# sfu-rsl/FastTrack

Hardware: AMD Instinct MI355X
Metric: frames/sec extract+match (higher is better)
Workload: dtype u8

## Files before the change

### fasttrack_amd/_capi.py

```python
from __future__ import annotations

import ctypes as C
import os
import re

import numpy as np

_PKG = os.path.dirname(os.path.abspath(__file__))
LIB_PATH = os.environ.get("FT_LIB") or os.path.join(_PKG, "libfasttrack_amd.so")
HEADER_PATH = os.path.join(os.path.dirname(_PKG), "include", "fasttrack_amd.h")

FT_OK, FT_ERR_INVALID, FT_ERR_NO_DEVICE, FT_ERR_HIP, FT_ERR_CAPACITY, FT_ERR_EMPTY = 0, -1, -2, -3, -4, -5

KP_DTYPE = np.dtype([("x", "<f4"), ("y", "<f4"), ("size", "<f4"), ("angle", "<f4"), ("response", "<f4"),
                     ("octave", "<i4"), ("class_id", "<i4")])
assert KP_DTYPE.itemsize == 28


class FastTrackError(RuntimeError):
    def __init__(self, status: int, message: str):
        super().__init__(f"fasttrack_amd status {status}: {message}")
        self.status = status


# ... 75 lines not shown
    _fields_ = [("M", C.c_int), ("skip", C.c_void_p), ("world_pos", C.c_void_p), ("normal", C.c_void_p),
                ("max_distance", C.c_void_p), ("min_distance", C.c_void_p), ("descriptors", C.c_void_p),
                ("observations", C.c_void_p)]


class FrustumResult(C.Structure):
    _fields_ = [(k, C.c_void_p) for k in ("in_view", "in_view_r", "level", "level_r", "view_cos", "view_cos_r",
                                          "proj_x", "proj_y", "proj_xr", "proj_yr", "depth", "depth_r")]


def declared_symbols() -> list[str]:
    text = open(HEADER_PATH).read()
    return sorted(set(re.findall(r"FT_API[^;(]*?\b(ft_[a-z0-9_]+)\s*\(", text)))


_lib = None


def _hip_runtime_mapped() -> bool:
    try:
        with open("/proc/self/maps") as f:
            mapped = {ln.split()[-1] for ln in f if "libamdhip64" in ln}
    except OSError:
        return False
    ours = {os.path.realpath(os.path.join(os.environ.get("ROCM_PATH", "/opt/rocm"), "lib", n))
            for n in ("libamdhip64.so", "libamdhip64.so.7")}
    return any(os.path.realpath(m) in ours for m in mapped)


def lib() -> C.CDLL:
    global _lib
    if _lib is not None:
        return _lib
    if not os.path.exists(LIB_PATH):
        raise ImportError(
            f"{LIB_PATH} is missing: build it with `python -c 'import __graft_entry__ as g; g.build()'` "
            f"(or `make -C fasttrack_amd/csrc`).  fasttrack_amd has no CPU fallback.")
    if "GPU_MAX_HW_QUEUES" not in os.environ:
        if _hip_runtime_mapped():
            import warnings
            warnings.warn("fasttrack_amd: a HIP runtime was loaded before the library and GPU_MAX_HW_QUEUES is unset - contexts "
                          "will use private streams (about 10 % below the lane table on wide batches); export "
                          "GPU_MAX_HW_QUEUES=10 before the first HIP call of the process", RuntimeWarning, stacklevel=2)
        else:
            os.environ["GPU_MAX_HW_QUEUES"] = "10"
    mode = os.RTLD_LOCAL | os.RTLD_NOW | getattr(os, "RTLD_DEEPBIND", 0)
    L = C.CDLL(LIB_PATH, mode=mode)
    vp, i, f = C.c_void_p, C.c_int, C.c_float
    ip = C.POINTER(C.c_int)
    L.ft_version.restype = C.c_char_p
    L.ft_last_error.restype = C.c_char_p
    L.ft_device_count.restype = i
    L.ft_device_pci_bus_id.argtypes = [i, C.c_char_p, i]
    L.ft_context_create.argtypes = [i, i, C.POINTER(vp)]
    L.ft_context_destroy.argtypes = [vp]
    L.ft_context_synchronize.argtypes = [vp]
    L.ft_context_device_name.argtypes = [vp, C.c_char_p, i]
    L.ft_context_host_threads.argtypes = [vp]
    L.ft_context_hw_queues.argtypes = [vp]
    L.ft_context_set_lane_map.argtypes = [vp, vp, i]
    L.ft_context_set_option.argtypes = [vp, C.c_char_p, i]
    L.ft_context_get_option.argtypes = [vp, C.c_char_p, ip]
    L.ft_option_describe.argtypes = [i, C.POINTER(C.c_char_p), C.POINTER(C.c_char_p), ip, C.POINTER(C.c_char_p)]
    L.ft_option_range.argtypes = [C.c_char_p, ip, ip]
    L.ft_context_save_stats.argtypes = [vp, C.c_char_p]
    L.ft_context_set_kernel_timing.argtypes = [vp, i]
    L.ft_context_get_stat.argtypes = [vp, C.c_char_p, C.POINTER(C.c_double), C.POINTER(C.c_long)]
    L.ft_context_reset_stats.argtypes = [vp]
    L.ft_device_malloc.argtypes = [vp, C.c_size_t, C.POINTER(vp)]
    L.ft_device_free.argtypes = [vp, vp]
    L.ft_host_malloc.argtypes = [vp, C.c_size_t, C.POINTER(vp)]
    L.ft_host_free.argtypes = [vp, vp]
    L.ft_memcpy_h2d.argtypes = [vp, vp, vp, C.c_size_t]
    L.ft_memcpy_d2h.argtypes = [vp, vp, vp, C.c_size_t]
    L.ft_extractor_create.argtypes = [vp, i, f, i, i, i, i, i, i, C.POINTER(vp)]
    L.ft_extractor_destroy.argtypes = [vp]
    L.ft_extractor_levels.argtypes = [vp]
    L.ft_extractor_max_batch.argtypes = [vp]
    L.ft_extractor_max_keypoints.argtypes = [vp]
    L.ft_extractor_scale_factors.argtypes = [vp, vp, vp, vp, vp]
    L.ft_extractor_features_per_level.argtypes = [vp, vp]
    L.ft_extractor_level_size.argtypes = [vp, i, ip, ip]
    L.ft_extract.argtypes = [vp, vp, i, i, i, i, i, vp, vp, i, ip, ip]
    L.ft_extract_batch.argtypes = [vp, vp, i, i, i, i, i, i, i, vp, vp, i, vp, vp]
    L.ft_extractor_download_level.argtypes = [vp, i, i, vp, i]
    L.ft_extractor_device_level.argtypes = [vp, i, i, C.POINTER(vp), ip]
    L.ft_extractor_download_candidates.argtypes = [vp, i, i, vp, i, ip]
    L.ft_extractor_octree_on_device.argtypes = [vp, i, vp, i, i, vp, i, ip, ip]
    L.ft_stereo_match.argtypes = [vp, vp, i, vp, i, vp, i, vp, vp, f, f, i, vp, vp, vp, ip]
    L.ft_stereo_frontend_create.argtypes = [vp, i, f, i, i, i, i, i, i, f, f, C.POINTER(vp)]
    L.ft_stereo_frontend_destroy.argtypes = [vp]
    L.ft_stereo_frontend_left.argtypes = [vp]
    L.ft_stereo_frontend_left.restype = vp
    L.ft_stereo_frontend_right.argtypes = [vp]
    L.ft_stereo_frontend_right.restype = vp
    L.ft_stereo_frontend_process.argtypes = [vp, vp, vp, i, i, i, i, i, vp, vp, vp, vp, vp, vp, i, vp, vp, vp]
    L.ft_stereo_frontend_submit.argtypes = [vp, vp, vp, i, i, i, i, i, vp, vp, vp, vp, vp, vp, i, vp, vp, vp]
    L.ft_stereo_frontend_wait.argtypes = [vp]
    L.ft_fisheye_match.argtypes = [vp, vp, i, vp, i, vp, vp, vp]
    L.ft_search_local_points.argtypes = [vp, C.POINTER(FrameView), C.POINTER(LocalPoints), f, f, vp, ip] + [vp] * 10
    L.ft_search_last_frame.argtypes = [vp, C.POINTER(FrameView), C.POINTER(LastPoints), vp, f, i, i, i, vp, ip] + [vp] * 4
    L.ft_features_in_area.argtypes = [vp, C.POINTER(FrameView), i, vp, vp, vp, vp, vp, vp, vp, i, vp]
    L.ft_fisheye_stereo.argtypes = [vp, C.POINTER(FisheyeRig), vp, vp, i, vp, vp, i, vp, i, vp, vp, vp, ip]
    L.ft_is_in_frustum.argtypes = [vp, C.POINTER(FrameView), C.POINTER(FramePose), C.POINTER(MapPoints), f, f,
                                   C.POINTER(FrustumResult), ip]
    L.ft_tracked_frame_create.argtypes = [vp, i, i, C.POINTER(vp)]
    L.ft_tracked_frame_destroy.argtypes = [vp]
    L.ft_tracked_frame_upload.argtypes = [vp, C.POINTER(FrameView)]
    L.ft_tracked_frame_bind_stereo.argtypes = [vp, vp, i, C.POINTER(FrameView)]
    L.ft_tracked_frame_search_last_frame.argtypes = [vp, C.POINTER(LastPoints), vp, f, i, i, i, vp, ip]
    L.ft_tracked_frame_search_last_frame_se3.argtypes = [vp, C.POINTER(LastPoints), C.POINTER(SE3), C.POINTER(SE3), f, i, i, i, vp, ip]
    L.ft_search_last_frame_se3.argtypes = [vp, C.POINTER(FrameView), C.POINTER(LastPoints), C.POINTER(SE3), C.POINTER(SE3), f, i, i,
                                           i, vp, ip] + [vp] * 4
    L.ft_tracked_frame_track_local_map.argtypes = [vp, C.POINTER(FramePose), C.POINTER(MapPoints), f, f, f, f, i, f,
                                                   C.POINTER(FrustumResult), ip, vp, ip]
    L.ft_tracked_frame_holder_obs.argtypes = [vp, vp]
    L.ft_search_for_initialization.argtypes = [vp, C.POINTER(FrameView), C.POINTER(FrameView), vp, i, f, i, vp, ip, vp]
    L.ft_tracked_frame_search_for_initialization.argtypes = [vp, vp, vp, i, f, i, vp, ip]
    L.ft_search_keyframe_projection.argtypes = [vp, C.POINTER(FrameView), C.POINTER(KeyFramePoints), C.POINTER(SE3), f, f, i, i, vp, ip, vp, vp]
    L.ft_tracked_frame_search_keyframe_projection.argtypes = [vp, C.POINTER(KeyFramePoints), C.POINTER(SE3), f, f, i, i, vp, ip]
    L.ft_tracked_batch_create.argtypes = [vp, i, i, i, C.POINTER(vp)]
    L.ft_tracked_batch_destroy.argtypes = [vp]
    L.ft_tracked_batch_upload.argtypes = [vp, i, C.POINTER(FrameView)]
    L.ft_tracked_batch_search_last_frame.argtypes = [vp, i, C.POINTER(LastPoints), vp, f, vp, vp, i, C.POINTER(vp), vp]
    L.ft_tracked_batch_search_last_frame_se3.argtypes = [vp, i, C.POINTER(LastPoints), C.POINTER(SE3), C.POINTER(SE3), f, vp, vp, i,
                                                         C.POINTER(vp), vp]
    L.ft_tracked_batch_track_local_map.argtypes = [vp, i, C.POINTER(FramePose), C.POINTER(MapPoints), f, f, f, f, i, f,
                                                   C.POINTER(FrustumResult), vp, C.POINTER(vp), vp]
    L.ft_tracked_batch_submit_search_last_frame.argtypes = L.ft_tracked_batch_search_last_frame.argtypes
    L.ft_tracked_batch_submit_search_last_frame_se3.argtypes = L.ft_tracked_batch_search_last_frame_se3.argtypes
    L.ft_tracked_batch_submit_track_local_map.argtypes = L.ft_tracked_batch_track_local_map.argtypes
    L.ft_tracked_batch_wait.argtypes = [vp]
    L.ft_tracked_batch_holder_obs.argtypes = [vp, i, vp]
    L.ft_tracked_batch_bind_fisheye.argtypes = [vp, vp, vp, i, i, i, i, i, i, C.POINTER(FrameView), C.POINTER(FisheyeRig), vp, C.POINTER(vp),
                                                C.POINTER(vp), C.POINTER(vp), C.POINTER(vp), vp]
    L.ft_tracked_batch_bind_fisheye_slots.argtypes = [vp, vp, vp, i, i, i, i, i, i, i, C.POINTER(FrameView), C.POINTER(FisheyeRig), vp,
                                                      C.POINTER(vp), C.POINTER(vp), C.POINTER(vp), C.POINTER(vp), vp]
    L.ft_descriptor_distance.argtypes = [vp, vp, vp, i, vp]
    L.ft_stereo_frontend_device_descriptors.argtypes = [vp, i, i, C.POINTER(vp), ip]
    L.ft_vocabulary_create.argtypes = [vp, i, i, i, i, i, vp, vp, vp, vp, C.POINTER(vp)]
    L.ft_vocabulary_load_text.argtypes = [vp, C.c_char_p, C.POINTER(vp)]
    L.ft_vocabulary_destroy.argtypes = [vp]
    L.ft_vocabulary_info.argtypes = [vp, ip, ip, ip, ip]
    L.ft_bow_transform.argtypes = [vp, vp, i, i, i, vp, vp, vp, vp, vp, i, ip, vp, vp, vp, i, ip]
    L.ft_search_by_bow.argtypes = [vp, C.POINTER(BowSide), vp, C.POINTER(BowSide), i, f, i, vp, ip]
    L.ft_search_for_triangulation.argtypes = [vp, C.POINTER(TriangKeyFrame), i, C.POINTER(TriangKeyFrame), C.POINTER(TriangPair), i, i, i, vp, vp, vp]
    L.ft_fuse_search.argtypes = [vp, C.POINTER(FusePoints), i, C.POINTER(FuseTarget), vp, vp, vp, vp]
    L.ft_search_keyframe_sim3.argtypes = [vp, C.POINTER(FrameView), i, C.POINTER(Sim3Job)]
    L.ft_selftest_libm.argtypes = [vp, i, C.c_uint32, C.c_uint32, C.c_uint32, C.POINTER(C.c_ulonglong),
                                   C.POINTER(C.c_ulonglong), C.POINTER(C.c_uint32)]
    L.ft_octree_distribute.argtypes = [vp, i, i, i, i, i, i, vp, i, ip]
    L.ft_level_geometry.argtypes = [i, i, i, f, i, vp, vp, vp, vp, vp, vp, vp]
    L.ft_pyramid_band_plan.argtypes = [i, i, f, i, i, vp, vp]
    _lib = L
    return L


def check(status: int) -> None:
    if status != FT_OK:
        raise FastTrackError(status, lib().ft_last_error().decode(errors="replace"))


def ptr(a):
    return None if a is None else a.ctypes.data_as(C.c_void_p)
```

### fasttrack_amd/csrc/extractor.cpp

```cpp
#include <algorithm>
#include <map>
#include <memory>
#include <cmath>
#include <cstdio>
#include <cstdlib>
#include <cstring>

#include "ft_host.h"

namespace {

inline int cvRoundF(float v) { return (int)lrintf(v); }
inline short satShort(int v) { return (short)(v < -32768 ? -32768 : (v > 32767 ? 32767 : v)); }

void buildTaps(int ssize, int dsize, bool clampIndex, FtTap *out) {
    const double inv_scale = (double)dsize / ssize;
    const double scale = 1. / inv_scale;
    for (int d = 0; d < dsize; d++) {
        float f = (float)((d + 0.5) * scale - 0.5);
        int s = (int)std::floor(f);
        f -= s;
        if (clampIndex) {
            if (s < 0) { f = 0; s = 0; }
            if (s >= ssize - 1) { f = 0; s = ssize - 1; }
// ... 162 lines not shown
int ft_pipeline_depth(const ft_tuning &t, int batch, bool deviceOctree) {
    const int envDepth = t.pipeline_depth > 0 ? std::min(FT_PIPE_MAX, t.pipeline_depth) : 0;
    if (envDepth) return std::max(1, std::min(envDepth, batch));
    if (deviceOctree) return batch >= 256 ? 2 : 1;
    return std::max(1, std::min(FT_PIPE_MAX, batch / 16));
}

int ft_extract_foreign_wait(ft_extractor *ex) {
    if (!ex->foreignReader) return FT_OK;
    hipEvent_t ev = ex->foreignReader;
    ex->foreignReader = nullptr;
    FT_HIP(hipStreamWaitEvent(ex->stream, ev, 0));
    return FT_OK;
}

int ft_extract_prepare(ft_extractor *ex, const uint8_t *const *images, int batch, int on_device, int width,
                       int height, int stride) {
    FT_REQUIRE(ex && images, "extract: null handle or image list");
    FT_REQUIRE(batch >= 1 && batch <= ex->maxBatch, "extract: batch outside [1, max_batch]");
    FT_REQUIRE(width == ex->width && height == ex->height, "extract: image size differs from the extractor's");
    FT_REQUIRE(stride >= width, "extract: stride smaller than width");
    int rc = ft_set_device(ex->ctx);
    if (rc != FT_OK) return rc;
    const FtGeom &g = ex->geom;
    const bool uploadKernel = ex->tune.upload_kernel != 0;
    if (!on_device && ex->stageHost && uploadKernel) {
        for (int b = 0; b < batch; b++) {
            if (!images[b]) {
                ft_set_error("extract: empty image");
                return FT_ERR_EMPTY;
            }
            ex->h_l0[b] = ex->d_pyr + (size_t)b * g.pyrPerSlot + g.lv[0].off;
        }
        ft_extract_restage(ex, images, batch, width, height, stride);
        ex->l0Aligned = true;
        ex->l0pitch = g.lv[0].pitch;
        ex->lastBatch = batch;
        return ft_launch_upload(ex->stream, batch, ex->h_srcTab, width, height, ex->d_pyr + g.lv[0].off, g.lv[0].pitch,
                                g.pyrPerSlot, ex->d_l0);
    }
    hipStream_t us = ex->stream;
    if (!on_device && !ex->stageHost) {
        rc = ft_context_upload_stream(ex->ctx, &us);
        if (rc != FT_OK) return rc;
    }
    bool oneCopy = false;
    if (!on_device && !ex->stageHost && batch >= 4 && stride == width && g.lv[0].pitch == width) {
        oneCopy = images[0] != nullptr;
        const ptrdiff_t delta = oneCopy && images[1] ? images[1] - images[0] : 0;
        if (delta < (ptrdiff_t)width * height) oneCopy = false;
        for (int b = 1; b < batch && oneCopy; b++)
            if (!images[b] || images[b] - images[b - 1] != delta) oneCopy = false;
        if (oneCopy && ex->ctx->maxPitch > 0 && (size_t)delta > ex->ctx->maxPitch) oneCopy = false;
        if (oneCopy) {
            const hipError_t ce = hipMemcpy2DAsync(ex->d_pyr + g.lv[0].off, g.pyrPerSlot, images[0], (size_t)delta, (size_t)width * height,
                                                   batch, hipMemcpyHostToDevice, us);
            if (ce != hipSuccess) {
                (void)hipGetLastError();
                oneCopy = false;
            }
        }
    }
    for (int b = 0; b < batch; b++) {
        if (!images[b]) {
            ft_set_error("extract: empty image");
            return FT_ERR_EMPTY;
        }
        uint8_t *slot0 = ex->d_pyr + (size_t)b * g.pyrPerSlot + g.lv[0].off;
        if (oneCopy) {
            ex->h_l0[b] = slot0;
        } else if (on_device) {
            ex->h_l0[b] = images[b];
        } else if (ex->stageHost) {
            ex->h_l0[b] = slot0;
            uint8_t *stg = ex->h_stage + (size_t)b * width * height;
            for (int y = 0; y < height; y++) memcpy(stg + (size_t)y * width, images[b] + (size_t)y * stride, width);
            FT_HIP(hipMemcpy2DAsync(slot0, g.lv[0].pitch, stg, width, width, height, hipMemcpyHostToDevice, ex->stream));
        } else {
            ex->h_l0[b] = slot0;
            FT_HIP(hipMemcpy2DAsync(slot0, g.lv[0].pitch, images[b], stride, width, height, hipMemcpyHostToDevice, us));
        }
    }
    if (us != ex->stream) {
        FT_HIP(hipEventRecord(ex->evUp, us));
        FT_HIP(hipStreamWaitEvent(ex->stream, ex->evUp, 0));
    }
    ex->l0Aligned = !on_device || ft_frames_aligned(images, batch, stride);
    ex->l0pitch = on_device ? stride : g.lv[0].pitch;
    ex->lastBatch = batch;
    FT_HIP(hipMemcpyAsync((void *)ex->d_l0, (const void *)ex->h_l0, sizeof(uint8_t *) * batch, hipMemcpyHostToDevice,
                          ex->stream));
    return FT_OK;
}

int ft_extract_ensure_stage(ft_extractor *ex) {
    if (!ex->h_srcTab) FT_CHECK(ex->own.pinAlloc(&ex->h_srcTab, 16));
    if (!ex->h_stage) FT_CHECK(ex->own.pinAlloc(&ex->h_stage, (size_t)std::min(ex->maxBatch, 16) * ex->width * ex->height));
    return FT_OK;
}
bool ft_frames_aligned(const uint8_t *const *images, int batch, int stride) {
    bool aligned = (stride & 3) == 0;
    for (int b = 0; b < batch; b++)
        if ((uintptr_t)images[b] & 3) aligned = false;
    return aligned;
}
void ft_extract_rebind(ft_extractor *ex, const uint8_t *const *images, int batch, int on_device, int width, int height, int stride) {
    if (on_device)
        for (int b = 0; b < batch; b++) ex->h_l0[b] = images[b];
    else
        ft_extract_restage(ex, images, batch, width, height, stride);
    ex->lastBatch = batch;
}
bool ft_graph_capture(hipStream_t st, hipGraphExec_t *exec, const std::function<int()> &enqueue) {
    if (*exec) hipGraphExecDestroy(*exec);
    *exec = nullptr;
    hipGraph_t graph = nullptr;
    int rc = FT_OK;
    hipError_t ce = hipStreamBeginCapture(st, hipStreamCaptureModeThreadLocal);
    if (ce == hipSuccess) {
        rc = enqueue();
        ce = hipStreamEndCapture(st, &graph);
        if (rc == FT_OK && ce == hipSuccess && graph) ce = hipGraphInstantiate(exec, graph, nullptr, nullptr, 0);
        if (graph) hipGraphDestroy(graph);
    }
    if (rc == FT_OK && ce == hipSuccess && *exec) return true;
    (void)hipGetLastError();
    *exec = nullptr;
    return false;
}
void ft_extract_restage(ft_extractor *ex, const uint8_t *const *images, int batch, int width, int height, int stride) {
    const bool uploadKernel = ex->tune.upload_kernel != 0;
    for (int b = 0; b < batch; b++) {
        if (uploadKernel && ft_is_pinned_host_range(images[b], (size_t)(height - 1) * stride + width)) {
            ex->h_srcTab[b].ptr = images[b];
            ex->h_srcTab[b].stride = stride;
            continue;
        }
        uint8_t *stg = ex->h_stage + (size_t)b * width * height;
        for (int y = 0; y < height; y++) memcpy(stg + (size_t)y * width, images[b] + (size_t)y * stride, width);
        ex->h_srcTab[b].ptr = stg;
        ex->h_srcTab[b].stride = width;
    }
}

int ft_extract_ensure_host_cand(ft_extractor *ex) {
    if (ex->h_cand) return FT_OK;
    FT_CHECK(ex->own.pinAlloc(&ex->h_cand, (size_t)ex->maxBatch * ex->geom.candPerSlot, hipHostMallocMapped | hipHostMallocCoherent));
    void *dp = nullptr;
    FT_HIP(hipHostGetDevicePointer(&dp, ex->h_cand, 0));
    ex->d_cand = (uint32_t *)dp;
    return FT_OK;
}

int ft_extract_launch_a(ft_extractor *ex, int b0, int nb, hipEvent_t done) {
    const FtGeom &g = ex->geom;
    if (!ex->deviceOctree) {
        const int rce = ft_extract_ensure_host_cand(ex);
        if (rce != FT_OK) return rce;
    }
    const bool tm = ex->ctx->kernelTiming;
    const int al = ex->l0Aligned ? 1 : 0;
    const uint8_t *const *l0 = ex->d_l0 + b0;
    uint8_t *pyr = ex->d_pyr + (size_t)b0 * g.pyrPerSlot;
    int *cellCount = ex->d_cellCount + (size_t)b0 * g.totalCells;
    uint32_t *stage = ex->d_stage + (size_t)b0 * g.stagePerSlot;
    hipStreamCaptureStatus cap = hipStreamCaptureStatusNone;
    FT_HIP(hipStreamIsCapturing(ex->stream, &cap));
    ex->evt.begin(tm, "kernel.pyr_down(all levels)", ex->stream);
    int rc = ft_launch_pyramid(ex->stream, g, nb, l0, ex->l0pitch, pyr, ex->d_taps, al, ex->tune.pyr_rows,
                               cap == hipStreamCaptureStatusNone ? &ex->pyrBands : nullptr);
    ex->evt.end(tm, ex->stream);
    if (rc != FT_OK) return rc;
    ex->evt.begin(tm, "kernel.fast_cells", ex->stream);
    rc = ft_launch_fast_cells(ex->stream, g, nb, l0, ex->l0pitch, pyr, ex->iniTh, ex->minTh, al, cellCount, stage,
                              ex->deviceOctree ? 0 : 1, ex->d_cellTab);
    ex->evt.end(tm, ex->stream);
    if (rc != FT_OK) return rc;
    ex->evt.begin(tm, "kernel.compact", ex->stream);
    uint32_t *candDst = ex->deviceOctree ? ex->d_candDev : ex->d_cand;
    int *cntDst = ex->deviceOctree ? ex->d_candCountDev : ex->d_candCount;
    rc = ft_launch_compact(ex->stream, g, nb, cellCount, stage, candDst + (size_t)b0 * g.candPerSlot,
                           cntDst + (size_t)b0 * g.nlevels);
    ex->evt.end(tm, ex->stream);
    if (rc != FT_OK) return rc;
    if (done) FT_HIP(hipEventRecord(done, ex->stream));
    return FT_OK;
}

int ft_extract_launch_octree(ft_extractor *ex, int sub, int b0, int nb, hipEvent_t done) {
    const FtGeom &g = ex->geom;
    hipStream_t so = ex->streamO[sub % FT_OCT_STREAMS];
    FT_HIP(hipEventRecord(ex->evO[sub], ex->stream));
    FT_HIP(hipStreamWaitEvent(so, ex->evO[sub], 0));
    FtOctArgs a = ex->octLayout;
    a.cand = ex->d_candDev + (size_t)b0 * g.candPerSlot;
    a.candCount = ex->d_candCountDev + (size_t)b0 * g.nlevels;
    a.sel = ex->d_sel + (size_t)b0 * g.maxKp;
    a.selCount = ex->d_selCount + (size_t)b0 * g.nlevels;
    a.overflow = ex->d_overflow;
    a.ovSlot = ex->d_ovSlot + b0;
    a.low = ex->d_octLow ? ex->d_octLow + (size_t)b0 * g.nlevels * FT_OCT_MAXN : nullptr;
    const bool large = nb > 16 || ex->lastBatch > 16;
    const bool histNow = ex->histEnabled && (large ? ex->histGrid > 0 : ex->histOn);
    a.histCap = histNow ? nb * g.nlevels : 0;
    a.histGrid = large ? std::min(ex->histGrid, nb * g.nlevels) : nb * g.nlevels;
    a.histWanted = ex->histEnabled && !histNow ? 1 : 0;
    a.histFirst = ex->histEnabled && (ex->histFirstMode == 2 || (ex->histFirstMode == 1 && !large)) ? 1 : 0;
    if (a.histFirst) a.histCap = a.histGrid = a.histWanted = 0;
    a.sortCap = a.bigN ? std::min(ex->bigGrid, nb * g.nlevels) : 0;
    a.bigCount = ex->d_bigCount + 4 * (sub % FT_OCT_STREAMS);
    a.bigList = ex->d_bigList + (size_t)(sub % FT_OCT_STREAMS) * ex->maxBatch * g.nlevels;
    a.sortList = ex->d_sortList + (size_t)(sub % FT_OCT_STREAMS) * ex->maxBatch * g.nlevels;
    const bool tm = ex->ctx->kernelTiming;
    ex->evt.begin(tm, "kernel.octree", so);
    int rc = ft_launch_octree(so, g, nb, a);
    ex->evt.end(tm, so);
    if (rc != FT_OK) return rc;
    if (done) FT_HIP(hipEventRecord(done, so));
    return FT_OK;
}

static void hostOctreeLevel(ft_extractor *ex, int slot, int level, const uint32_t *cand, int n) {
    static thread_local ft::OctreeWorkspace ws;
    static thread_local std::vector<int> keep;
    const FtLevelGeom &v = ex->geom.lv[level];
    keep.clear();
    const int minB = FT_EDGE_THRESHOLD - 3;
    int k = ft::distribute_octree(cand, n, minB, v.maxBX, minB, v.maxBY, ex->quota[level], ws, keep);
    k = std::min(k, ex->levelMax[level]);
    FtSelKp *dst = ex->h_sel + (size_t)slot * ex->geom.maxKp + ex->levelOff[level];
    for (int i = 0; i < k; i++) {
        const uint32_t c = cand[keep[i]];
        dst[i].x = (short)((c & 0xfffu) + minB);
        dst[i].y = (short)(((c >> 12) & 0xfffu) + minB);
        dst[i].level = (short)level;
        dst[i].response = (short)(c >> 24);
    }
    ex->h_selCount[(size_t)slot * ex->nlevels + level] = k;
}
static void sumSelCounts(ft_extractor *ex, int slot) {
    int n = 0;
    for (int l = 0; l < ex->nlevels; l++) n += ex->h_selCount[(size_t)slot * ex->nlevels + l];
    ex->h_nSel[slot] = n;
}
static void sortEmissionOrder(const FtLevelGeom &v, uint32_t *cand, int n) {
    auto rank = [&](uint32_t q) -> uint64_t {
        const int x = (int)(q & 0xfffu) - 3, y = (int)((q >> 12) & 0xfffu) - 3;
        const int cj = std::min(x / std::max(v.wCell, 1), std::max(v.nCols - 1, 0));
        const int ci = std::min(y / std::max(v.hCell, 1), std::max(v.nRows - 1, 0));
        return ((uint64_t)ci << 48) | ((uint64_t)cj << 32) | ((uint64_t)y << 16) | (uint64_t)x;
    };
    std::sort(cand, cand + n, [&](uint32_t a, uint32_t b) { return rank(a) < rank(b); });
}

int ft_extract_octree_multi(ft_extractor *const *exs, int nex, int b0, int nb) {
    ft_extractor *e0 = exs[0];
    const FtGeom &g = e0->geom;
    const int L = g.nlevels;
    const int perEx = nb * L;
    auto task = [&](int t, int) {
        ft_extractor *ex = exs[t / perEx];
        const int r = t % perEx;
        const int level = r / nb, rel = r - level * nb, slot = b0 + rel;
        hostOctreeLevel(ex, slot, level, ex->h_cand + (size_t)slot * g.candPerSlot + g.lv[level].candBase,
                        ex->h_candCount[slot * L + level]);
    };
    e0->ctx->pool->parallel_for(nex * perEx, task);
    for (int e = 0; e < nex; e++)
        for (int slot = b0; slot < b0 + nb; slot++) sumSelCounts(exs[e], slot);
    return FT_OK;
}

int ft_extract_octree(ft_extractor *ex, int b0, int nb) { return ft_extract_octree_multi(&ex, 1, b0, nb); }

void ft_extract_update_big_grid(ft_extractor *ex) {
    if (!ex->octLayout.bigN && !ex->histEnabled) return;
    if (ex->lastBatch <= 16) {
        if (ex->h_overflow[0]) {
            if (ex->histEnabled && ex->histFirstMode == 0 && !ex->histOn) ex->histOn = true;
            else if (ex->octLayout.bigN && ex->bigGrid == 0) ex->bigGrid = ex->maxBatch * ex->nlevels;
        }
        return;
    }
    int want = 0, wantHist = 0;
    for (int k = 0; k < FT_OCT_STREAMS; k++) {
        want = std::max(want, ex->h_bigStat[k]);
        wantHist = std::max(wantHist, ex->h_histStat[k]);
        ex->h_bigStat[k] = ex->h_histStat[k] = 0;
    }
    if (wantHist > 0) {
        ex->histIdle = 0;
        ex->histGrid = std::max(std::max(ex->histGrid, FT_OCT_HISTMIN), std::min(FT_OCT_HISTMAX, ((wantHist + 63) / 64) * 64));
    } else if (ex->histGrid > 0 && ++ex->histIdle >= FT_OCT_HIST_RETIRE) {
        ex->histGrid = 0;
    }
    if (!ex->octLayout.bigN) return;
    if (want > 0) {
        ex->bigIdle = 0;
        const int need = std::max(FT_OCT_BIGMIN, ((want + want / 4 + 63) / 64) * 64);
        if (need > ex->bigGrid) ex->bigGrid = std::min(need, ex->maxBatch * ex->nlevels);
    } else if (ex->bigGrid > 0 && ++ex->bigIdle >= 16) {
        ex->bigGrid = 0;
    }
}

int ft_extract_overflow_slots(ft_extractor *ex, int batch, std::vector<int> &slots) {
    std::vector<int> f(batch, 0);
    FT_HIP(hipMemcpy(f.data(), ex->d_ovSlot, sizeof(int) * batch, hipMemcpyDeviceToHost));
    for (int b = 0; b < batch; b++)
        if (f[b]) slots.push_back(b);
    FT_HIP(hipMemset(ex->d_ovSlot, 0, sizeof(int) * batch));
    FT_HIP(hipMemset(ex->d_overflow, 0, sizeof(int)));
    ex->h_overflow[0] = 0;
    return FT_OK;
}

int ft_extract_repair_prepare(const std::vector<std::pair<ft_extractor *, int>> &jobs) {
    if (jobs.empty()) return FT_OK;
    ft_extractor *e0 = jobs[0].first;
    const FtGeom &g = e0->geom;
    const int L = g.nlevels;
    std::vector<int> jobIdx(jobs.size());
    {
        std::map<ft_extractor *, int> perEx;
        for (size_t j = 0; j < jobs.size(); j++) jobIdx[j] = perEx[jobs[j].first]++;
        for (auto &kv : perEx) {
            ft_extractor *ex = kv.first;
            if (kv.second > ex->repCap) {
                ex->own.giveBack(ex->h_repCand);
                ex->repCap = 0;
                const int want = std::min(ex->maxBatch, std::max(kv.second + kv.second / 2, 4));
                FT_CHECK(ex->own.pinAlloc(&ex->h_repCand, (size_t)want * g.candPerSlot));
                ex->repCap = want;
            }
        }
    }
    std::vector<int> counts(jobs.size() * L, 0);
    for (size_t j = 0; j < jobs.size(); j++) {
        ft_extractor *ex = jobs[j].first;
        const int slot = jobs[j].second;
        FT_HIP(hipMemcpy(counts.data() + j * L, ex->d_candCountDev + (size_t)slot * L, sizeof(int) * L, hipMemcpyDeviceToHost));
        for (int l = 0; l < L; l++) {
            const FtLevelGeom &v = g.lv[l];
            int &n = counts[j * L + l];
            n = std::max(0, std::min(n, v.candCap));
            if (n > 0)
                FT_HIP(hipMemcpyAsync(ex->h_repCand + (size_t)jobIdx[j] * g.candPerSlot + v.candBase,
                                      ex->d_candDev + (size_t)slot * g.candPerSlot + v.candBase, sizeof(uint32_t) * n,
                                      hipMemcpyDeviceToHost, ex->streamB));
        }
    }
    for (auto &j : jobs) FT_HIP(hipStreamSynchronize(j.first->streamB));
    auto task = [&](int t, int) {
        const int j = t / L, level = t % L;
        ft_extractor *ex = jobs[j].first;
        const int n = counts[(size_t)j * L + level];
        uint32_t *cand = ex->h_repCand + (size_t)jobIdx[j] * g.candPerSlot + g.lv[level].candBase;
        sortEmissionOrder(g.lv[level], cand, n);
        hostOctreeLevel(ex, jobs[j].second, level, cand, n);
    };
    e0->ctx->pool->parallel_for((int)jobs.size() * L, task);
    for (auto &j : jobs) {
        sumSelCounts(j.first, j.second);
        j.first->ctx->addStat("extract.host_octree_repairs", 0);
    }
    return FT_OK;
}

int ft_extract_repair_launch(ft_extractor *ex, int slot, hipStream_t st) {
    const bool dev = ex->deviceOctree;
    ex->deviceOctree = false;
    const int rc = ft_extract_launch_b(ex, slot, 1, st);
    ex->deviceOctree = dev;
    return rc;
}

static int rangeMaxN(const ft_extractor *ex, int b0, int nb) {
    if (ex->deviceOctree) return ex->geom.maxKp;
    int maxN = 0;
    for (int b = b0; b < b0 + nb; b++) maxN = std::max(maxN, ex->h_nSel[b]);
    return maxN;
}

int ft_extract_launch_b(ft_extractor *ex, int b0, int nb, hipStream_t st) {
    const FtGeom &g = ex->geom;
    if (!ex->deviceOctree) {
        FT_HIP(hipMemcpyAsync(ex->d_selCount + (size_t)b0 * g.nlevels, ex->h_selCount + (size_t)b0 * g.nlevels,
                              sizeof(int) * nb * g.nlevels, hipMemcpyHostToDevice, st));
        FT_HIP(hipMemcpyAsync(ex->d_sel + (size_t)b0 * g.maxKp, ex->h_sel + (size_t)b0 * g.maxKp,
                              sizeof(FtSelKp) * (size_t)nb * g.maxKp, hipMemcpyHostToDevice, st));
    }
    const bool tm = ex->ctx->kernelTiming;
    ex->evt.begin(tm, "kernel.orient_desc", st);
    int rc = ft_launch_orient_desc(st, g, nb, ex->d_l0 + b0, ex->l0pitch, ex->d_pyr + (size_t)b0 * g.pyrPerSlot,
                                   ex->l0Aligned ? 1 : 0, ex->d_sel + (size_t)b0 * g.maxKp,
                                   ex->d_selCount + (size_t)b0 * g.nlevels, ex->octLayout, ex->d_nSel + b0,
                                   ex->d_keys + (size_t)b0 * g.maxKp, ex->d_desc + (size_t)b0 * g.maxKp * 32);
    ex->evt.end(tm, st);
    return rc;
}

int ft_extract_finish_counts(ft_extractor *ex, int batch, hipStream_t st) {
    if (!ex->deviceOctree) return FT_OK;
    FtCountsArgs a;
    a.nSel = ex->d_nSel;
    a.oNSel = ex->h_nSel;
    a.overflow = ex->d_overflow;
    a.oOverflow = ex->h_overflow;
    a.bigCount = (ex->octLayout.bigN || ex->histEnabled) ? ex->d_bigCount : nullptr;
    a.oHist = ex->h_histStat;
    a.oBig = ex->h_bigStat;
    a.batch = batch;
    a.nStreams = FT_OCT_STREAMS;
    return ft_launch_finish_counts(st, a);
}

FtDeliverArgs ft_deliver_args(const ft_extractor *ex) {
    FtDeliverArgs d{};
    d.keysL = ex->d_keys;
    d.descL = ex->d_desc;
    d.nL = ex->d_nSel;
    d.overflowL = ex->d_overflow;
    d.oKeysL = ex->h_keys;
    d.oDescL = ex->h_desc;
    d.oNL = ex->h_nSel;
    d.oOverflowL = ex->h_overflow;
    d.srcStride = d.dstStride = ex->geom.maxKp;
    return d;
}

int ft_extract_download(ft_extractor *ex, int b0, int nb, hipStream_t st) {
    const FtGeom &g = ex->geom;
    const int maxN = rangeMaxN(ex, b0, nb);
    if (maxN == 0) return FT_OK;
    const size_t o = (size_t)b0 * g.maxKp;
    FT_HIP(hipMemcpy2DAsync(ex->h_keys + o, sizeof(ft_keypoint) * g.maxKp, ex->d_keys + o, sizeof(ft_keypoint) * g.maxKp,
                            sizeof(ft_keypoint) * maxN, nb, hipMemcpyDeviceToHost, st));
    FT_HIP(hipMemcpy2DAsync(ex->h_desc + o * 32, (size_t)32 * g.maxKp, ex->d_desc + o * 32, (size_t)32 * g.maxKp,
                            (size_t)32 * maxN, nb, hipMemcpyDeviceToHost, st));
    return FT_OK;
}

static int assembleOutputs(ft_extractor *ex, int batch, int lap0, int lap1, ft_keypoint *keypoints,
                           uint8_t *descriptors, int capacity, int *n_keypoints, int *n_mono) {
    const FtGeom &g = ex->geom;
    for (int b = 0; b < batch; b++)
        if (ex->h_nSel[b] > capacity) {
            ft_set_error("extract: output capacity too small (use ft_extractor_max_keypoints)");
            return FT_ERR_CAPACITY;
        }
    const std::function<void(int, int)> one = [&](int b, int) {
        const int n = ex->h_nSel[b];
        const ft_keypoint *src = ex->h_keys + (size_t)b * g.maxKp;
        const uint8_t *sd = ex->h_desc + (size_t)b * g.maxKp * 32;
        ft_keypoint *dk = keypoints ? keypoints + (size_t)b * capacity : nullptr;
        uint8_t *dd = descriptors ? descriptors + (size_t)b * capacity * 32 : nullptr;
        int monoIndex = 0, stereoIndex = n - 1;
        for (int i = 0; i < n; i++) {
            const ft_keypoint &kp = src[i];
            int dst;
            if (kp.x >= lap0 && kp.x <= lap1) dst = stereoIndex--;
            else dst = monoIndex++;
            if (dk) dk[dst] = kp;
            if (dd) memcpy(dd + (size_t)dst * 32, sd + (size_t)i * 32, 32);
        }
        if (n_keypoints) n_keypoints[b] = n;
        if (n_mono) n_mono[b] = monoIndex;
    };
    if (batch >= 16) ex->ctx->pool->parallel_for(batch, one);
    else
        for (int b = 0; b < batch; b++) one(b, 0);
    return FT_OK;
}

extern "C" {

int ft_extractor_create(ft_context *ctx, int nfeatures, float scale_factor, int nlevels, int ini_th_fast,
                        int min_th_fast, int image_width, int image_height, int max_batch, ft_extractor **out) {
    FT_REQUIRE(ctx && out, "ft_extractor_create: null argument");
    *out = nullptr;
    FT_REQUIRE(nfeatures > 0, "nfeatures must be positive");
    FT_REQUIRE(nlevels >= 1 && nlevels <= FT_MAX_LEVELS, "nlevels outside [1, 12]");
    FT_REQUIRE(scale_factor > 1.0f, "scaleFactor must exceed 1");
    FT_REQUIRE(min_th_fast >= 1 && ini_th_fast >= min_th_fast && ini_th_fast < 255,
               "FAST thresholds must satisfy 1 <= minThFAST <= iniThFAST < 255");
    FT_REQUIRE(image_width >= 2 * FT_EDGE_THRESHOLD + 8 && image_height >= 2 * FT_EDGE_THRESHOLD + 8,
               "image smaller than the 19-px border allows");
    FT_REQUIRE(max_batch >= 1 && max_batch <= 4096, "max_batch outside [1, 4096]");
    FT_CHECK(ft_set_device(ctx));
    ft_extractor *ex = new ft_extractor();
    std::unique_ptr<ft_extractor, void (*)(ft_extractor *)> guard(ex, destroyExtractor);
    ex->ctx = ctx;
    ex->nfeatures = nfeatures;
    ex->scaleFactor = scale_factor;
    ex->nlevels = nlevels;
    ex->iniTh = ini_th_fast;
    ex->minTh = min_th_fast;
    ex->width = image_width;
    ex->height = image_height;
    ex->maxBatch = max_batch;
    ex->tune = ctx->tuning;
    std::vector<FtTap> taps;
    FT_CHECK(buildGeometry(ex, taps));
    const FtGeom &g = ex->geom;
    const size_t B = max_batch;
    {
        int first[FT_MAX_LEVELS * PC_BANDS], end[FT_MAX_LEVELS * PC_BANDS];
        ft_pyr_bands_of(g, PC_BANDS, first, end);
        ex->pyrBands.K = PC_BANDS;
        for (int l = 1; l < g.nlevels; l++)
            for (int k = 0; k < PC_BANDS; k++) ex->pyrBands.rows[l][k] = (unsigned)first[l * PC_BANDS + k] | ((unsigned)end[l * PC_BANDS + k] << 16);
    }
    {
        hipStream_t lanes[FT_LANE_STREAMS];
        FT_CHECK(ft_context_take_lanes(ctx, max_batch <= 16, image_width, image_height, lanes, &ex->ownStreams));
        ex->stream = lanes[0];
        ex->streamB = lanes[1];
        for (int i = 0; i < FT_OCT_STREAMS; i++) ex->streamO[i] = lanes[2 + i];
    }
    FtOwned &own = ex->own;
    for (int i = 0; i < FT_PIPE_MAX; i++) {
        FT_CHECK(own.event(&ex->evA[i]));
        FT_CHECK(own.event(&ex->evB[i]));
        FT_CHECK(own.event(&ex->evO[i]));
    }
    FT_CHECK(own.event(&ex->evJoin));
    FT_CHECK(own.event(&ex->evUp));
    FT_CHECK(own.devAlloc(&ex->d_pyr, B * g.pyrPerSlot));
    FT_CHECK(own.devAlloc(&ex->d_taps, taps.size()));
    FT_CHECK(own.devAlloc(&ex->d_cellTab, (size_t)std::max(g.totalCells, 1)));
    FT_CHECK(own.devAlloc(&ex->d_cellCount, B * g.totalCells));
    FT_CHECK(own.devAlloc(&ex->d_stage, B * g.stagePerSlot));
    FT_CHECK(own.devAlloc(&ex->d_l0, B));
    FT_CHECK(own.devAlloc(&ex->d_sel, B * g.maxKp));
    FT_CHECK(own.devAlloc(&ex->d_nSel, B));
    FT_CHECK(own.devAlloc(&ex->d_selCount, B * g.nlevels + FT_MAX_LEVELS));
    FT_CHECK(own.devAlloc(&ex->d_overflow, 1));
    FT_CHECK(own.devAlloc(&ex->d_ovSlot, B));
    FT_CHECK(own.devAlloc(&ex->d_bigCount, 4 * FT_OCT_STREAMS));
    FT_CHECK(own.pinAlloc(&ex->h_bigStat, FT_OCT_STREAMS));
    FT_CHECK(own.pinAlloc(&ex->h_histStat, FT_OCT_STREAMS));
    for (int k = 0; k < FT_OCT_STREAMS; k++) ex->h_bigStat[k] = ex->h_histStat[k] = 0;
    FT_CHECK(own.devAlloc(&ex->d_bigList, (size_t)FT_OCT_STREAMS * B * g.nlevels));
    FT_CHECK(own.devAlloc(&ex->d_sortList, (size_t)FT_OCT_STREAMS * B * g.nlevels));
    FT_CHECK(own.pinAlloc(&ex->h_selCount, B * g.nlevels));
    FT_CHECK(own.pinAlloc(&ex->h_overflow, 1));
    FT_CHECK(own.devAlloc(&ex->d_keys, B * g.maxKp));
    FT_CHECK(own.devAlloc(&ex->d_desc, B * g.maxKp * 32));
    FT_CHECK(own.pinAlloc(&ex->h_l0, B));
    FT_CHECK(own.pinAlloc(&ex->h_candCount, B * g.nlevels, hipHostMallocMapped | hipHostMallocCoherent));
    FT_CHECK(own.pinAlloc(&ex->h_sel, B * g.maxKp));
    FT_CHECK(own.pinAlloc(&ex->h_nSel, B));
    FT_CHECK(own.pinAlloc(&ex->h_nMono, B));
    FT_CHECK(own.pinAlloc(&ex->h_keys, B * g.maxKp));
    FT_CHECK(own.pinAlloc(&ex->h_desc, B * g.maxKp * 32));
    FT_HIP(hipHostGetDevicePointer((void **)&ex->d_candCount, ex->h_candCount, 0));
    {
        std::vector<FtCellRec> cellTab(std::max(g.totalCells, 1), FtCellRec{0, 0, 0, 0});
        for (int l = 0; l < nlevels; l++) {
            const FtLevelGeom &v = g.lv[l];
            for (int ci = 0; ci < v.nRows; ci++)
                for (int cj = 0; cj < v.nCols; cj++) {
                    const int iniX = 16 + cj * v.wCell, iniY = 16 + ci * v.hCell;
                    const int maxX = std::min(iniX + v.wCell + 6, v.maxBX), maxY = std::min(iniY + v.hCell + 6, v.maxBY);
                    int tw = maxX - iniX, th = maxY - iniY;
                    if (iniX >= v.maxBX - 6 || iniY >= v.maxBY - 3 || tw < 7 || th < 7) tw = th = 0;
                    const int c = ci * v.nCols + cj;
                    FtCellRec &r = cellTab[v.cellBase + c];
                    r.origin = (uint32_t)iniX | ((uint32_t)iniY << 16);
                    r.shape = (uint32_t)tw | ((uint32_t)th << 8) | ((uint32_t)l << 16);
                    r.srcOff = (uint32_t)(v.off + iniY * v.pitch + iniX);
                    r.outOff = (uint32_t)(v.stageBase + c * v.cellCap);
                }
        }
        FT_HIP(hipMemcpy(ex->d_cellTab, cellTab.data(), cellTab.size() * sizeof(FtCellRec), hipMemcpyHostToDevice));
        FT_HIP(hipMemcpy(ex->d_taps, taps.data(), taps.size() * sizeof(FtTap), hipMemcpyHostToDevice));
        FT_HIP(hipMemset(ex->d_nSel, 0, sizeof(int) * B));
    }
    memset(ex->h_nSel, 0, sizeof(int) * B);
    ex->levelOff.assign(nlevels + 1, 0);
    for (int l = 0; l < nlevels; l++) ex->levelOff[l + 1] = ex->levelOff[l] + ex->levelMax[l];
    memset(ex->h_selCount, 0, sizeof(int) * B * nlevels);
    ex->h_overflow[0] = 0;
    {
        FtOctArgs &o = ex->octLayout;
        memset(&o, 0, sizeof o);
        int maxQ = 0, need = 0;
        for (int l = 0; l < nlevels; l++) {
            o.quota[l] = ex->quota[l];
            o.levelMax[l] = ex->levelMax[l];
            o.selOff[l] = ex->levelOff[l];
            maxQ = std::max(maxQ, ex->quota[l]);
            const int minB = FT_EDGE_THRESHOLD - 3;
            int nIni = (int)std::round(static_cast<float>(g.lv[l].maxBX - minB) / (g.lv[l].maxBY - minB));
            if (nIni < 1) nIni = 1;
            need = std::max(need, ex->quota[l] + 4 * nIni);
        }
        o.poolCap = need + 16;
        (void)maxQ;
        ex->deviceOctree = ex->tune.device_octree != 0 && o.poolCap < 30000 && ft_octree_smem_bytes(o.poolCap) <= 160 * 1024;
        o.histCap = o.sortCap = o.histGrid = o.histWanted = o.histFirst = 0;
        ex->histEnabled = ex->deviceOctree && ex->tune.oct_hist != 0 &&
                          ft_octree_hist_smem_bytes(o.poolCap) <= 160 * 1024;
        ex->histFirstMode = ex->tune.oct_hist_first;
        o.bigN = ex->deviceOctree && ex->tune.oct_big != 0 ? ft_octree_big_keys(o.poolCap) : 0;
        o.bigCount = ex->d_bigCount;
        o.bigList = ex->d_bigList;
        o.sortList = ex->d_sortList;
        o.low = nullptr;
        if (ex->deviceOctree) {
            if (ft_debug_env("FT_DEBUG_OCT_PROFILE")) {
                FT_CHECK(own.devAlloc(&o.prof, (size_t)FT_MAX_LEVELS * 8));
                hipMemset(o.prof, 0, sizeof(unsigned long long) * FT_MAX_LEVELS * 8);
            }
            FT_CHECK(own.devAlloc(&ex->d_candDev, B * g.candPerSlot));
            FT_CHECK(own.devAlloc(&ex->d_candCountDev, B * g.nlevels));
            if (ft_octree_smem_bytes(o.poolCap, true) < ft_octree_smem_bytes(o.poolCap, false))
                FT_CHECK(own.devAlloc(&ex->d_octLow, B * g.nlevels * (size_t)FT_OCT_MAXN));
            FT_HIP(hipMemset(ex->d_overflow, 0, sizeof(int)));
            FT_HIP(hipMemset(ex->d_ovSlot, 0, sizeof(int) * B));
            FT_HIP(hipMemset(ex->d_bigCount, 0, 4 * FT_OCT_STREAMS * sizeof(int)));
        }
    }
    ctx->liveObjects++;
    *out = guard.release();
    return FT_OK;
}

int ft_octree_distribute(const int *xys, int n, int minX, int maxX, int minY, int maxY, int N, int *out_idx,
                         int capacity, int *n_out) {
    FT_REQUIRE(n >= 0 && (n == 0 || xys) && n_out, "ft_octree_distribute: bad argument");
    FT_REQUIRE(maxX > minX && maxY > minY && N >= 0, "ft_octree_distribute: empty region");
    std::vector<uint32_t> packed(n);
    for (int i = 0; i < n; i++) {
        FT_REQUIRE(xys[3 * i] >= 0 && xys[3 * i] < 4096 && xys[3 * i + 1] >= 0 && xys[3 * i + 1] < 4096 &&
                       xys[3 * i + 2] >= 0 && xys[3 * i + 2] < 256,
                   "ft_octree_distribute: candidate out of range");
        packed[i] = ft_pack_cand(xys[3 * i], xys[3 * i + 1], xys[3 * i + 2]);
    }
    ft::OctreeWorkspace ws;
    std::vector<int> keep;
    auto dbgInt = [](const char *name, int def) {
        const char *e = ft_debug_env(name);
        return e && *e ? atoi(e) : def;
    };
    const int usePaths = dbgInt("FT_DEBUG_OCTREE_PATHS", 0);
    int k;
    if (usePaths == 3 && n < 65535) {
        const int bins = dbgInt("FT_DEBUG_OCTREE_HIST_BINS", FT_OCT_HIST_BINS);
        k = ft::distribute_octree_hist(packed.data(), n, minX, maxX, minY, maxY, N, bins, keep);
        if (k == -2 && !dbgInt("FT_DEBUG_OCTREE_HIST_STRICT", 0)) {
            keep.clear();
            k = ft::distribute_octree_rounds(packed.data(), n, minX, maxX, minY, maxY, N, keep);
        }
    } else if (usePaths == 2 && n < 65535) k = ft::distribute_octree_rounds(packed.data(), n, minX, maxX, minY, maxY, N, keep);
    else if (usePaths == 1 && n < 65535) k = ft::distribute_octree_paths(packed.data(), n, minX, maxX, minY, maxY, N, keep);
    else k = ft::distribute_octree(packed.data(), n, minX, maxX, minY, maxY, N, ws, keep);
    if (k < 0) {
        ft_set_error("ft_octree_distribute: path-code workspace overflow");
        return FT_ERR_CAPACITY;
    }
    *n_out = k;
    if (k > capacity) {
        ft_set_error("ft_octree_distribute: capacity too small");
        return FT_ERR_CAPACITY;
    }
    for (int i = 0; i < k; i++) out_idx[i] = keep[i];
    return FT_OK;
}

int ft_level_geometry(int width, int height, int nfeatures, float scale_factor, int nlevels, int *level_w,
                      int *level_h, int *quota, int *n_cols, int *n_rows, int *w_cell, int *h_cell) {
    FT_REQUIRE(nlevels >= 1 && nlevels <= FT_MAX_LEVELS && scale_factor > 1.0f && nfeatures > 0, "bad parameters");
    ft_extractor ex;
    ex.nfeatures = nfeatures;
    ex.scaleFactor = scale_factor;
    ex.nlevels = nlevels;
    ex.width = width;
    ex.height = height;
    std::vector<FtTap> taps;
    int rc = buildGeometry(&ex, taps);
    if (rc != FT_OK) return rc;
    for (int l = 0; l < nlevels; l++) {
        const FtLevelGeom &v = ex.geom.lv[l];
        if (level_w) level_w[l] = v.w;
        if (level_h) level_h[l] = v.h;
        if (quota) quota[l] = ex.quota[l];
        if (n_cols) n_cols[l] = v.nCols;
        if (n_rows) n_rows[l] = v.nRows;
        if (w_cell) w_cell[l] = v.wCell;
        if (h_cell) h_cell[l] = v.hCell;
    }
    return FT_OK;
}

int ft_pyramid_band_plan(int width, int height, float scale_factor, int nlevels, int bands, int *first_row, int *end_row) {
    FT_REQUIRE(nlevels >= 1 && nlevels <= FT_MAX_LEVELS && scale_factor > 1.0f && bands >= 1 && first_row && end_row, "bad parameters");
    ft_extractor ex;
    ex.nfeatures = 1000;
    ex.scaleFactor = scale_factor;
    ex.nlevels = nlevels;
    ex.width = width;
    ex.height = height;
    std::vector<FtTap> taps;
    int rc = buildGeometry(&ex, taps);
    if (rc != FT_OK) return rc;
    ft_pyr_bands_of(ex.geom, bands, first_row, end_row);
    return FT_OK;
}

int ft_extractor_destroy(ft_extractor *ex) {
    if (!ex) return FT_OK;
    freeAll(ex);
    ex->ctx->liveObjects--;
    delete ex;
    return FT_OK;
}

int ft_extractor_levels(const ft_extractor *ex) { return ex ? ex->nlevels : 0; }
int ft_extractor_max_batch(const ft_extractor *ex) { return ex ? ex->maxBatch : 0; }
int ft_extractor_max_keypoints(const ft_extractor *ex) { return ex ? ex->geom.maxKp : 0; }

int ft_extractor_scale_factors(const ft_extractor *ex, float *scale, float *inv_scale, float *sigma2,
                               float *inv_sigma2) {
    FT_REQUIRE(ex, "null extractor");
    for (int i = 0; i < ex->nlevels; i++) {
        if (scale) scale[i] = ex->sf[i];
        if (inv_scale) inv_scale[i] = ex->invsf[i];
        if (sigma2) sigma2[i] = ex->sigma2[i];
        if (inv_sigma2) inv_sigma2[i] = ex->invsigma2[i];
    }
    return FT_OK;
}

int ft_extractor_features_per_level(const ft_extractor *ex, int *quota) {
    FT_REQUIRE(ex && quota, "null argument");
    for (int i = 0; i < ex->nlevels; i++) quota[i] = ex->quota[i];
    return FT_OK;
}

int ft_extractor_level_size(const ft_extractor *ex, int level, int *width, int *height) {
    FT_REQUIRE(ex && level >= 0 && level < ex->nlevels, "level out of range");
    if (width) *width = ex->geom.lv[level].w;
    if (height) *height = ex->geom.lv[level].h;
    return FT_OK;
}

int ft_extract_batch(ft_extractor *ex, const uint8_t *const *images, int batch, int on_device, int width,
                     int height, int stride, int lap0, int lap1, ft_keypoint *keypoints, uint8_t *descriptors,
                     int capacity, int *n_keypoints, int *n_mono) {
    FT_REQUIRE(ex, "null extractor");
    if (!images || width <= 0 || height <= 0) {
        ft_set_error("extract: empty image");
        return FT_ERR_EMPTY;
    }
    FtTimer tAll;
    int rc = ft_set_device(ex->ctx);
    if (rc != FT_OK) return rc;
    rc = ft_extract_foreign_wait(ex);
    if (rc != FT_OK) return rc;
    const int S = ft_pipeline_depth(ex->tune, batch, ex->deviceOctree);
    const int sb = (batch + S - 1) / S;
    const bool deliver = batch <= 8;
    static const bool stagedOnly = ft_debug_env("FT_DEBUG_STAGED_OUTPUTS") != nullptr;
    const bool direct = !stagedOnly && !deliver && ex->deviceOctree && capacity > 0 && (keypoints || descriptors) &&
                        (!keypoints || ft_host_block_contains(ex->ctx, keypoints, sizeof(ft_keypoint) * (size_t)batch * capacity)) &&
                        (!descriptors || ft_host_block_contains(ex->ctx, descriptors, (size_t)32 * batch * capacity));
    bool deliveredDirect = false;
    auto deliverOrdered = [&](int b0, int nb) -> int {
        deliveredDirect = true;
        FtOrderedArgs a;
        a.keys = ex->d_keys;
        a.desc = ex->d_desc;
        a.nSel = ex->d_nSel;
        a.oKeys = keypoints;
        a.oDesc = descriptors;
        a.oMono = ex->h_nMono;
        a.srcStride = ex->geom.maxKp;
        a.capacity = capacity;
        a.b0 = b0;
        a.lap0 = (float)lap0;
        a.lap1 = (float)lap1;
        return ft_launch_deliver_ordered(ex->streamB, nb, a);
    };
    auto repairOverflow = [&]() -> int {
        std::vector<int> slots;
        FT_CHECK(ft_extract_overflow_slots(ex, batch, slots));
        std::vector<std::pair<ft_extractor *, int>> jobs;
        for (int b : slots) jobs.emplace_back(ex, b);
        FT_CHECK(ft_extract_repair_prepare(jobs));
        for (int b : slots) {
            ex->ctx->addStat("extract.device_octree_fallbacks", 1);
            FT_CHECK(ft_extract_repair_launch(ex, b, ex->streamB));
            FT_CHECK(deliveredDirect ? deliverOrdered(b, 1) : ft_extract_download(ex, b, 1, ex->streamB));
        }
        FT_HIP(hipStreamSynchronize(ex->streamB));
        return FT_OK;
    };
    const bool dev = ex->deviceOctree;
    double tOct = 0;
    auto enqueue = [&](bool capture) -> int {
        FT_CHECK(ft_extract_prepare(ex, images, batch, on_device, width, height, stride));
        for (int s = 0, b0 = 0; b0 < batch; s++, b0 += sb) {
            const int nb = std::min(sb, batch - b0);
            FT_CHECK(ft_extract_launch_a(ex, b0, nb, dev ? nullptr : ex->evA[s]));
            if (dev) FT_CHECK(ft_extract_launch_octree(ex, s, b0, nb, ex->evA[s]));
        }
        for (int s = 0, b0 = 0; b0 < batch; s++, b0 += sb) {
            const int nb = std::min(sb, batch - b0);
            if (dev) {
                FT_HIP(hipStreamWaitEvent(ex->streamB, ex->evA[s], 0));
            } else {
                FT_HIP(hipEventSynchronize(ex->evA[s]));
                FtTimer tO;
                FT_CHECK(ft_extract_octree(ex, b0, nb));
                tOct += tO.ms();
            }
            FT_CHECK(ft_extract_launch_b(ex, b0, nb, ex->streamB));
            if (!capture) FT_CHECK((direct && dev) ? deliverOrdered(b0, nb) : ft_extract_download(ex, b0, nb, ex->streamB));
        }
        if (!capture) return ft_extract_finish_counts(ex, batch, ex->streamB);
        FT_CHECK(ft_launch_deliver(ex->streamB, batch, ft_deliver_args(ex)));
        FT_HIP(hipEventRecord(ex->evJoin, ex->streamB));
        FT_HIP(hipStreamWaitEvent(ex->stream, ex->evJoin, 0));
        return FT_OK;
    };
    bool launched = false, graphable = ex->tune.graph != 0 && !ex->graphDisabled && ex->ownStreams && dev && !ex->ctx->kernelTiming &&
                                       deliver && batch >= 1 && batch <= ex->maxBatch && width == ex->width && height == ex->height && stride >= width;
    for (int b = 0; b < batch && graphable; b++)
        if (!images[b]) graphable = false;
    if (graphable && !on_device && ft_extract_ensure_stage(ex) != FT_OK) {
        (void)hipGetLastError();
        graphable = false;
    }
    if (graphable) {
        ft_extractor::GraphKey key;
        key.batch = batch; key.onDevice = on_device; key.width = width; key.height = height; key.stride = stride;
        key.aligned = !on_device || ft_frames_aligned(images, batch, stride);
        key.bigGrid = ex->bigGrid + (ex->histOn ? (1 << 24) : 0);
        if (ex->graphExec && key == ex->graphKey) {
            ft_extract_rebind(ex, images, batch, on_device, width, height, stride);
            launched = true;
        } else {
            ex->stageHost = !on_device;
            launched = ft_graph_capture(ex->stream, &ex->graphExec, [&] { return enqueue(true); });
            ex->stageHost = false;
            ex->graphDisabled = !launched;
            if (launched) ex->graphKey = key;
            ex->ctx->addStat(launched ? "extract.graph_captures" : "extract.graph_capture_failed", 0);
        }
    }
    if (launched) FT_HIP(hipGraphLaunch(ex->graphExec, ex->stream));
    else FT_CHECK(enqueue(false));
    if (dev) ex->ctx->addStat("extract.device_octree_batches", 0);
    if (launched) {
        FT_HIP(hipStreamSynchronize(ex->stream));
    } else {
        FT_HIP(hipStreamSynchronize(ex->streamB));
        FT_HIP(hipStreamSynchronize(ex->stream));
        ex->evt.resolve(ex->ctx);
        if (!dev) ex->ctx->addStat("extract.octree(host)", tOct);
    }
    if (dev) {
        ft_extract_update_big_grid(ex);
        if (ex->h_overflow[0]) FT_CHECK(repairOverflow());
    }
    if (deliveredDirect) {
        for (int b = 0; b < batch; b++)
            if (ex->h_nSel[b] > capacity) {
                ft_set_error("extract: output capacity too small (use ft_extractor_max_keypoints)");
                return FT_ERR_CAPACITY;
            }
        for (int b = 0; b < batch; b++) {
            if (n_keypoints) n_keypoints[b] = ex->h_nSel[b];
            if (n_mono) n_mono[b] = ex->h_nMono[b];
        }
        ex->ctx->addStat("extract.delivered_in_order_on_device", batch);
        rc = FT_OK;
    } else {
        rc = assembleOutputs(ex, batch, lap0, lap1, keypoints, descriptors, capacity, n_keypoints, n_mono);
    }
    ex->ctx->addStat("extract.total", tAll.ms());
    return rc;
}

int ft_extract(ft_extractor *ex, const uint8_t *image, int width, int height, int stride, int lap0, int lap1,
               ft_keypoint *keypoints, uint8_t *descriptors, int capacity, int *n_keypoints, int *n_mono) {
    if (!image || width <= 0 || height <= 0) {
        ft_set_error("extract: empty image");
        return FT_ERR_EMPTY;
    }
    const uint8_t *imgs[1] = {image};
    return ft_extract_batch(ex, imgs, 1, 0, width, height, stride, lap0, lap1, keypoints, descriptors, capacity,
                            n_keypoints, n_mono);
}

int ft_extractor_device_level(ft_extractor *ex, int slot, int level, const uint8_t **dptr, int *pitch) {
    FT_REQUIRE(ex && dptr && pitch, "null argument");
    FT_REQUIRE(slot >= 0 && slot < ex->lastBatch, "slot holds no image");
    FT_REQUIRE(level >= 0 && level < ex->nlevels, "level out of range");
    const FtGeom &g = ex->geom;
    if (level == 0) {
        *dptr = ex->h_l0[slot];
        *pitch = ex->l0pitch;
    } else {
        *dptr = ex->d_pyr + (size_t)slot * g.pyrPerSlot + g.lv[level].off;
        *pitch = g.lv[level].pitch;
    }
    return FT_OK;
}

int ft_extractor_download_level(ft_extractor *ex, int slot, int level, uint8_t *dst, int dst_stride) {
    FT_REQUIRE(dst, "null destination");
    const uint8_t *src = nullptr;
    int pitch = 0;
    int rc = ft_extractor_device_level(ex, slot, level, &src, &pitch);
    if (rc != FT_OK) return rc;
    rc = ft_set_device(ex->ctx);
    if (rc != FT_OK) return rc;
    const FtLevelGeom &v = ex->geom.lv[level];
    FT_REQUIRE(dst_stride >= v.w, "destination stride smaller than the level width");
    FT_HIP(hipStreamSynchronize(ex->stream));
    FT_HIP(hipStreamSynchronize(ex->streamB));
    FT_HIP(hipMemcpy2D(dst, dst_stride, src, pitch, v.w, v.h, hipMemcpyDeviceToHost));
    return FT_OK;
}

int ft_extractor_download_blurred_level(ft_extractor *ex, int slot, int level, uint8_t *dst, int dst_stride) {
    FT_REQUIRE(dst, "null destination");
    const uint8_t *src = nullptr;
    int pitch = 0;
    int rc = ft_extractor_device_level(ex, slot, level, &src, &pitch);
    if (rc != FT_OK) return rc;
    rc = ft_set_device(ex->ctx);
    if (rc != FT_OK) return rc;
    const FtLevelGeom &v = ex->geom.lv[level];
    FT_REQUIRE(dst_stride >= v.w, "destination stride smaller than the level width");
    FT_HIP(hipStreamSynchronize(ex->stream));
    FT_HIP(hipStreamSynchronize(ex->streamB));
    uint8_t *tmp = nullptr;
    FT_HIP(hipMalloc((void **)&tmp, (size_t)v.w * v.h));
    rc = ft_launch_blur_level(ex->stream, src, pitch, v.w, v.h, tmp, v.w);
    hipError_t e = rc == FT_OK ? hipStreamSynchronize(ex->stream) : hipSuccess;
    if (rc == FT_OK && e == hipSuccess) e = hipMemcpy2D(dst, dst_stride, tmp, v.w, v.w, v.h, hipMemcpyDeviceToHost);
    hipFree(tmp);
    if (rc != FT_OK) return rc;
    FT_HIP(e);
    return FT_OK;
}

int ft_extractor_download_candidates(ft_extractor *ex, int slot, int level, int *xys, int capacity, int *n) {
    FT_REQUIRE(ex && n, "null argument");
    FT_REQUIRE(slot >= 0 && slot < ex->lastBatch, "slot holds no image");
    FT_REQUIRE(level >= 0 && level < ex->nlevels, "level out of range");
    int rc = ft_set_device(ex->ctx);
    if (rc != FT_OK) return rc;
    FT_HIP(hipStreamSynchronize(ex->stream));
    const FtGeom &g = ex->geom;
// ... 94 lines not shown
```

### fasttrack_amd/csrc/ft_host.h

```cpp
#pragma once

#include <algorithm>
#include <atomic>
#include <chrono>
#include <functional>
#include <map>
#include <mutex>
#include <string>
#include <vector>

#include "ft_internal.h"
#include "octree.h"
#include "thread_pool.h"

#define FT_REQUIRE(cond, msg)               \
    do {                                    \
        if (!(cond)) {                      \
            ft_set_error(std::string(msg)); \
            return FT_ERR_INVALID;          \
        }                                   \
    } while (0)
#define FT_CHECK(call)                \
    do {                              \
        const int _rc = (call);       \
// ... 20 lines not shown
    X(search_cache, "FT_SEARCH_CACHE", 2, 0, 3, "projection searches: 1 = later claim passes walk the cached candidate keys, 2 = and a batch of 24+ frames resolves its claims in one launch, 3 = every batch does") \
    X(search_grid, "FT_SEARCH_GRID", 1, 0, 1, "projection searches: CSR grid of the frame built on the device") \
    X(blocking_sync, "FT_BLOCKING_SYNC", 2, 0, 2, "host waits for the device: 0 = the runtime's default (it spins), 1 = sleeping (hipDeviceScheduleBlockingSync), 2 = sleeping when the process may use fewer than 8 CPUs")

struct ft_tuning {
#define FT_X(field, env, def, lo, hi, doc) int field = def;
    FT_TUNING_OPTIONS(FT_X)
#undef FT_X
};
bool ft_tuning_from_env(ft_tuning &t, std::string &err);
int *ft_tuning_field(ft_tuning &t, const char *name);
const char *ft_debug_env(const char *name);
const char *ft_read_env(const char *name);

struct ft_context {
    int device = 0;
    std::string deviceName;
    ft::ThreadPool *pool = nullptr;
    hipStream_t stream = nullptr;
    std::mutex laneMutex;
    std::vector<hipStream_t> lanes;
    hipStream_t uploadStream = nullptr;
    std::vector<int> laneMap;
    std::vector<int> laneMapSmall;
    bool userLaneMap = false;
    int nextLaneSet = 0;
    size_t maxPitch = 0;
    int hwQueues = 4;
    std::atomic<int> liveObjects{0};
    std::mutex matchMutex;
    void *scratchDev = nullptr, *scratchPin = nullptr;
    size_t scratchDevBytes = 0, scratchPinBytes = 0;
    std::mutex hostAllocMutex;
    std::vector<hipEvent_t> retiredEvents;
    std::map<uintptr_t, size_t> hostBlocks;
    std::vector<void *> hostAllocs;
    bool kernelTiming = false;
    ft_tuning tuning;
    std::mutex statsMutex;
    std::map<std::string, std::pair<double, long>> stats;
    void addStat(const char *name, double ms) {
        std::lock_guard<std::mutex> lk(statsMutex);
        auto &s = stats[name];
        s.first += ms;
        s.second += 1;
    }
};

struct FtEventTimer {
    struct Rec {
        const char *name;
        hipEvent_t a, b;
    };
    std::vector<hipEvent_t> pool;
    size_t used = 0;
    std::vector<Rec> recs;
    hipEvent_t get() {
        if (used == pool.size()) {
            hipEvent_t e = nullptr;
            if (hipEventCreate(&e) != hipSuccess) return nullptr;
            pool.push_back(e);
        }
        return pool[used++];
    }
    void begin(bool enabled, const char *name, hipStream_t st) {
        if (!enabled) return;
        Rec r{name, get(), get()};
        if (!r.a || !r.b) return;
        hipEventRecord(r.a, st);
        recs.push_back(r);
    }
    void end(bool enabled, hipStream_t st) {
        if (!enabled || recs.empty()) return;
        hipEventRecord(recs.back().b, st);
    }
    void resolve(ft_context *ctx) {
        for (auto &r : recs) {
            float ms = 0;
            if (hipEventElapsedTime(&ms, r.a, r.b) == hipSuccess) ctx->addStat(r.name, ms);
        }
        recs.clear();
        used = 0;
    }
    void destroy() {
        for (auto e : pool) hipEventDestroy(e);
        pool.clear();
    }
};

struct FtOwned {
    std::vector<void *> dev, pin;
    std::vector<hipEvent_t> events;
    FtOwned() = default;
    FtOwned(const FtOwned &) = delete;
    FtOwned &operator=(const FtOwned &) = delete;
    ~FtOwned() { release(); }
    template <typename T>
    int devAlloc(T **p, size_t n) {
        FT_HIP(hipMalloc((void **)p, std::max<size_t>(n, 1) * sizeof(T)));
        dev.push_back((void *)*p);
        return FT_OK;
    }
    template <typename T>
    int pinAlloc(T **p, size_t n, unsigned flags = hipHostMallocDefault) {
        FT_HIP(hipHostMalloc((void **)p, std::max<size_t>(n, 1) * sizeof(T), flags));
        pin.push_back((void *)*p);
        return FT_OK;
    }
    int event(hipEvent_t *e) {
        FT_HIP(hipEventCreateWithFlags(e, hipEventDisableTiming));
        events.push_back(*e);
        return FT_OK;
    }
    template <typename T>
    void giveBack(T *&p) {
        auto drop = [&](std::vector<void *> &v) {
            auto it = std::find(v.begin(), v.end(), (void *)p);
            if (it == v.end()) return false;
            v.erase(it);
            return true;
        };
        if (p && drop(dev)) hipFree((void *)p);
        else if (p && drop(pin)) hipHostFree((void *)p);
        p = nullptr;
    }
    void release() {
        for (auto e : events) hipEventDestroy(e);
        for (auto p : dev) hipFree(p);
        for (auto p : pin) hipHostFree(p);
        events.clear();
        dev.clear();
        pin.clear();
    }
};

struct FtTimer {
    std::chrono::steady_clock::time_point t0 = std::chrono::steady_clock::now();
    double ms() const {
        return std::chrono::duration<double, std::milli>(std::chrono::steady_clock::now() - t0).count();
    }
};

struct ft_extractor {
    ft_context *ctx = nullptr;
    ft_tuning tune;
    int nfeatures = 0, nlevels = 0, iniTh = 0, minTh = 0, width = 0, height = 0, maxBatch = 0;
    float scaleFactor = 1.2f;
    std::vector<float> sf, invsf, sigma2, invsigma2;
    std::vector<int> quota;
    std::vector<int> levelMax;
    std::vector<int> levelOff;
    FtGeom geom{};
    FtPyrBands pyrBands{};
    hipStream_t stream = nullptr;
    hipStream_t streamB = nullptr;
    hipEvent_t evA[FT_PIPE_MAX] = {}, evB[FT_PIPE_MAX] = {};
    hipStream_t streamO[FT_OCT_STREAMS] = {};
    bool ownStreams = false;
    FtOwned own;
    hipEvent_t evO[FT_PIPE_MAX] = {};
    struct GraphKey {
        int batch = 0, onDevice = 0, width = 0, height = 0, stride = 0, aligned = 0, bigGrid = 0;
        bool operator==(const GraphKey &o) const {
            return batch == o.batch && onDevice == o.onDevice && width == o.width && height == o.height && stride == o.stride &&
                   aligned == o.aligned && bigGrid == o.bigGrid;
        }
    } graphKey;
    hipGraphExec_t graphExec = nullptr;
    bool graphDisabled = false;
    hipEvent_t evJoin = nullptr;
    hipEvent_t evUp = nullptr;
    hipEvent_t foreignReader = nullptr;
    uint8_t *d_pyr = nullptr;
    FtTap *d_taps = nullptr;
    FtCellRec *d_cellTab = nullptr;
    int *d_cellCount = nullptr;
    uint32_t *d_stage = nullptr;
    const uint8_t **d_l0 = nullptr;
    const uint8_t **h_l0 = nullptr;
    uint8_t *h_stage = nullptr;
    FtSrcEntry *h_srcTab = nullptr;
    bool stageHost = false;
    uint32_t *h_cand = nullptr, *d_cand = nullptr;
    int *h_candCount = nullptr, *d_candCount = nullptr;
    bool deviceOctree = false;
    uint32_t *d_candDev = nullptr;
    int *d_candCountDev = nullptr;
    int *d_selCount = nullptr, *h_selCount = nullptr;
    int *d_overflow = nullptr, *h_overflow = nullptr;
    int *d_ovSlot = nullptr;
    int *d_bigCount = nullptr;
    int *h_bigStat = nullptr;
    unsigned *d_bigList = nullptr;
    unsigned *d_sortList = nullptr;
    uint32_t *d_octLow = nullptr;
    uint32_t *h_repCand = nullptr;
    int repCap = 0;
    bool histEnabled = false;
    int histFirstMode = 1;
    bool histOn = false;
    int histGrid = FT_OCT_HISTMIN;
    int histIdle = 0;
    int *h_histStat = nullptr;
    int bigGrid = 0, bigIdle = 0;
    FtOctArgs octLayout{};
    FtSelKp *h_sel = nullptr, *d_sel = nullptr;
    int *h_nSel = nullptr, *d_nSel = nullptr;
    int *h_nMono = nullptr;
    ft_keypoint *d_keys = nullptr, *h_keys = nullptr;
    uint8_t *d_desc = nullptr, *h_desc = nullptr;
    uint8_t *d_stScratch = nullptr;
    int stCap = 0;
    FtEventTimer evt;
    int lastBatch = 0;
    int l0pitch = 0;
    bool l0Aligned = true;
};

struct ft_stereo_frontend {
    ft_context *ctx = nullptr;
    ft_extractor *exL = nullptr, *exR = nullptr;
    float mbf = 0, mb = 0;
    int capacity = 0;
    FtOwned own;
    float *d_uright = nullptr, *d_depth = nullptr, *h_uright = nullptr, *h_depth = nullptr;
    int *d_sad = nullptr, *d_nMatches = nullptr, *h_nMatches = nullptr;
    int maxBatch = 0;
    bool pairedCapable = false, lastPaired = false;
    FtSortedR *d_sorted = nullptr;
    int *d_rowStart = nullptr;
    int *d_leftOrder = nullptr;
    struct GraphKey {
        int batch = 0, onDevice = 0, width = 0, height = 0, stride = 0, capacity = 0, alignedL = 0, alignedR = 0, paired = 0;
        int bigGridL = 0, bigGridR = 0;
        const void *out[6] = {nullptr, nullptr, nullptr, nullptr, nullptr, nullptr};
        bool operator==(const GraphKey &o) const {
            if (batch != o.batch || onDevice != o.onDevice || width != o.width || height != o.height || stride != o.stride ||
                capacity != o.capacity || alignedL != o.alignedL || alignedR != o.alignedR || paired != o.paired ||
                bigGridL != o.bigGridL || bigGridR != o.bigGridR)
                return false;
            for (int i = 0; i < 6; i++)
                if (out[i] != o.out[i]) return false;
            return true;
        }
    } graphKey;
    hipGraphExec_t graphExec = nullptr;
    bool graphDisabled = false;
    hipEvent_t evFork = nullptr, evJoin = nullptr;
    hipEvent_t evDone[2] = {nullptr, nullptr};
    struct Pending {
        bool active = false, direct = false, graph = false;
        int batch = 0, capacity = 0;
        std::vector<const uint8_t *> imagesL, imagesR;
        int onDevice = 0, width = 0, height = 0, stride = 0;
        ft_keypoint *keysL = nullptr, *keysR = nullptr;
        uint8_t *descL = nullptr, *descR = nullptr;
        int *nL = nullptr, *nR = nullptr, *nMatches = nullptr;
        float *uright = nullptr, *depth = nullptr;
    } pending;
};

int ft_set_device(const ft_context *ctx);
int ft_context_take_lanes(ft_context *ctx, bool wantPrivate, int width, int height, hipStream_t *out, bool *owned);
int ft_context_upload_stream(ft_context *ctx, hipStream_t *out);
bool ft_is_pinned_host(const void *p);
bool ft_is_pinned_host_range(const void *p, size_t bytes);
bool ft_host_block_contains(ft_context *ctx, const void *p, size_t bytes);
int ft_extract_foreign_wait(ft_extractor *ex);
int ft_ensure_scratch(ft_context *ctx, size_t devBytes, size_t pinBytes);
int ft_usable_cpus();
int ft_hw_queues_hint();
bool ft_parse_lane_map(const char *text, std::vector<int> &map, std::string &err);
int ft_pipeline_depth(const ft_tuning &t, int batch, bool deviceOctree);
int ft_extract_prepare(ft_extractor *ex, const uint8_t *const *images, int batch, int on_device, int width, int height,
                       int stride);
int ft_extract_launch_a(ft_extractor *ex, int b0, int nb, hipEvent_t done);
int ft_extract_ensure_stage(ft_extractor *ex);
int ft_extract_ensure_host_cand(ft_extractor *ex);
void ft_extract_restage(ft_extractor *ex, const uint8_t *const *images, int batch, int width, int height, int stride);
bool ft_graph_capture(hipStream_t st, hipGraphExec_t *exec, const std::function<int()> &enqueue);
bool ft_frames_aligned(const uint8_t *const *images, int batch, int stride);
void ft_extract_rebind(ft_extractor *ex, const uint8_t *const *images, int batch, int on_device, int width, int height, int stride);
FtDeliverArgs ft_deliver_args(const ft_extractor *ex);
int ft_extract_octree(ft_extractor *ex, int b0, int nb);
int ft_extract_overflow_slots(ft_extractor *ex, int batch, std::vector<int> &slots);
void ft_extract_update_big_grid(ft_extractor *ex);
int ft_extract_repair_prepare(const std::vector<std::pair<ft_extractor *, int>> &jobs);
int ft_extract_repair_launch(ft_extractor *ex, int slot, hipStream_t st);
int ft_extract_octree_multi(ft_extractor *const *exs, int nex, int b0, int nb);
int ft_extract_launch_octree(ft_extractor *ex, int sub, int b0, int nb, hipEvent_t done);
int ft_extract_launch_b(ft_extractor *ex, int b0, int nb, hipStream_t st);
int ft_extract_finish_counts(ft_extractor *ex, int batch, hipStream_t st);
int ft_extract_download(ft_extractor *ex, int b0, int nb, hipStream_t st);
```

### fasttrack_amd/csrc/ft_internal.h

```cpp
#pragma once

#include <hip/hip_runtime.h>
#include <stdint.h>

#include <string>

#include "../../include/fasttrack_amd.h"

#define FT_MAX_LEVELS 12
#define FT_EDGE_THRESHOLD 19
#define FT_PATCH_SIZE 31
#define FT_HALF_PATCH 15
#define FT_TH_HIGH 100
#define FT_TH_LOW 50
#define FT_HISTO_LENGTH 30
#define FT_GRID_COLS 64
#define FT_GRID_ROWS 48

struct FtLevelGeom {
    int w, h, pitch;
    int off;
    int maxBX, maxBY;
    int nCols, nRows, wCell, hCell;
    int cellBase;
    int cellCap;
    int stageBase;
    int candBase;
    int candCap;
    int xtab, ytab;
    int area2x;
};

struct FtGeom {
    int nlevels;
    int totalCells;
    int stagePerSlot;
    int candPerSlot;
    int pyrPerSlot;
    int maxKp;
    float sf[FT_MAX_LEVELS];
    float invsf[FT_MAX_LEVELS];
    unsigned fastLv[FT_MAX_LEVELS];
    FtLevelGeom lv[FT_MAX_LEVELS];
};

struct FtCellRec {
    uint32_t origin;
    uint32_t shape;
    uint32_t srcOff;
    uint32_t outOff;
};

static inline __host__ __device__ uint32_t ft_pack_cand(int x, int y, int s) {
    return (uint32_t)x | ((uint32_t)y << 12) | ((uint32_t)s << 24);
}

struct FtSlotGrid {
    int blocksPerSlot, batch, xcdMap;
    unsigned magic;
};
static inline FtSlotGrid ft_slot_grid(int blocksPerSlot, int batch, dim3 &grid) {
    FtSlotGrid sg;
    sg.blocksPerSlot = blocksPerSlot;
    sg.batch = batch;
    sg.xcdMap = batch >= 8;
    sg.magic = blocksPerSlot > 1 ? 0xffffffffu / (unsigned)blocksPerSlot + 1u : 0u;
    grid = sg.xcdMap ? dim3((unsigned)blocksPerSlot * 8u * (unsigned)((batch + 7) / 8), 1, 1) : dim3(blocksPerSlot, batch, 1);
    return sg;
}
#if defined(__HIPCC__)
__device__ __forceinline__ bool ft_slot_block(const FtSlotGrid &sg, int &slot, int &blk) {
    if (!sg.xcdMap) {
        slot = blockIdx.y;
        blk = blockIdx.x;
        return true;
    }
    const int xcd = (int)(blockIdx.x & 7u), j = (int)(blockIdx.x >> 3);
    const int grp = sg.magic ? (int)__umulhi((unsigned)j, sg.magic) : j;
    blk = j - grp * sg.blocksPerSlot;
    slot = grp * 8 + xcd;
    return slot < sg.batch;
}
#endif

struct FtSelKp {
    short x, y;
    short level;
    short response;
};

struct FtTap {
    short s, a0, a1, pad;
};

#define FT_OCT_MAXN 4096
#define FT_OCT_HIST_BINS 8192
#define FT_OCT_HISTMIN 16
#define FT_OCT_HIST_RETIRE 2
#ifndef FT_OCT_HISTMAX
#define FT_OCT_HISTMAX 768
#endif
#define FT_OCT_BIGMIN 64
struct FtOctArgs {
    const uint32_t *cand;
    const int *candCount;
    FtSelKp *sel;
    int *selCount;
    int *overflow;
    int *ovSlot;
    int *bigCount;
    unsigned *bigList, *sortList;
    uint32_t *low;
    int histCap, histGrid, sortCap, bigN;
    int histWanted;
    int histFirst;
    int quota[FT_MAX_LEVELS], levelMax[FT_MAX_LEVELS], selOff[FT_MAX_LEVELS];
    int poolCap, keyBytes;
    unsigned long long *prof;
};

struct FtBowTree {
    const int *childStart;
    const unsigned *childList;
    const uint8_t *desc;
    const unsigned *wordId;
    const double *weight;
    int nNodes;
};
int ft_launch_bow_walk(hipStream_t st, const FtBowTree &t, const uint8_t *desc, int n, int nidLevel, unsigned *wordOut,
                       unsigned *nodeOut, double *weightOut);
struct FtBowSide {
    int n, nNodes;
    const unsigned *nodes;
    const int *offsets;
    const unsigned *features;
    const uint8_t *desc;
};
int ft_launch_search_by_bow(hipStream_t st, const FtBowSide &K, const uint8_t *kfHasPoint, const FtBowSide &F, int nleft,
                            float nnRatio, int *matches);

void ft_set_error(const std::string &msg);
int ft_debug_repeat(const char *name);
int ft_hip_fail(hipError_t e, const char *what, const char *file, int line);
const char *ft_debug_env(const char *name);

#define FT_HIP(call)                                                              \
    do {                                                                          \
        hipError_t _e = (call);                                                   \
        if (_e != hipSuccess) return ft_hip_fail(_e, #call, __FILE__, __LINE__);  \
    } while (0)

#ifndef PC_BANDS
#define PC_BANDS 2
#endif
#ifndef PC_WAVES
#define PC_WAVES 16
#endif
#define FT_PYR_BANDS_MAX 8
struct FtPyrBands {
    int K;
    unsigned rows[FT_MAX_LEVELS][FT_PYR_BANDS_MAX];
};
void ft_pyr_bands_of(const FtGeom &g, int K, int *first, int *end);
int ft_launch_pyramid(hipStream_t st, const FtGeom &g, int batch, const uint8_t *const *l0, int l0pitch,
                      uint8_t *pyr, const FtTap *taps, int alignedLoads, int rowsKernel, const FtPyrBands *bands);
struct FtCellRanges {
    int lo0, n0, lo1, n1;
};
int ft_launch_fast_cells(hipStream_t st, const FtGeom &g, int batch, const uint8_t *const *l0, int l0pitch,
                         const uint8_t *pyr, int iniTh, int minTh, int alignedLoads, int *cellCount,
                         uint32_t *stage, int ordered, const FtCellRec *cellTab);
int ft_launch_compact(hipStream_t st, const FtGeom &g, int batch, const int *cellCount, const uint32_t *stage,
                      uint32_t *cand, int *candCount);
int ft_launch_orient_desc(hipStream_t st, const FtGeom &g, int batch, const uint8_t *const *l0, int l0pitch,
                          const uint8_t *pyr, int alignedLoads, const FtSelKp *sel, const int *selCount,
                          const FtOctArgs &layout, int *nSel, ft_keypoint *keys, uint8_t *desc);
int ft_launch_octree(hipStream_t st, const FtGeom &g, int batch, const FtOctArgs &a);
int ft_launch_blur_level(hipStream_t st, const uint8_t *img, int pitch, int w, int h, uint8_t *dst, int dstPitch);
size_t ft_octree_smem_bytes(int poolCap, bool compact = false);
size_t ft_octree_hist_smem_bytes(int poolCap);
int ft_octree_big_keys(int poolCap);
size_t ft_fast_smem_bytes(const FtGeom &g);

struct __attribute__((aligned(16))) FtSortedR {
    float x, y;
    int octave, idx;
    unsigned long long desc[4];
};
struct FtStereoArgs {
    const ft_keypoint *keysL, *keysR;
    const uint8_t *descL, *descR;
    const int *nL, *nR;
    int capacity;
    float mbf, mb;
    float *uright, *depth;
    int *sad;
    int *hamIdx;
    int *nMatches;
    int applyMedianCut;
    int *rowStart;
    FtSortedR *sorted;
    int rowStride;
    int *leftOrder;
    int alignedLoads;
};
struct FtDeliverArgs {
    const ft_keypoint *keysL, *keysR;
    const uint8_t *descL, *descR;
    const float *uright, *depth;
    const int *nL, *nR, *nMatches;
    const int *overflowL, *overflowR;
    ft_keypoint *oKeysL, *oKeysR;
    uint8_t *oDescL, *oDescR;
    float *oUright, *oDepth;
    int *oNL, *oNR, *oNMatches, *oOverflowL, *oOverflowR;
    int srcStride, dstStride;
};
int ft_launch_deliver(hipStream_t st, int batch, const FtDeliverArgs &a);
struct FtOrderedArgs {
    const ft_keypoint *keys;
    const uint8_t *desc;
    const int *nSel;
    ft_keypoint *oKeys;
    uint8_t *oDesc;
    int *oMono;
    int srcStride, capacity, b0;
    float lap0, lap1;
};
int ft_launch_deliver_ordered(hipStream_t st, int nb, const FtOrderedArgs &a);
struct FtCountsArgs {
    const int *nSel;
    int *oNSel;
    const int *overflow;
    int *oOverflow;
    int *bigCount;
    int *oHist, *oBig;
    int batch, nStreams;
};
int ft_launch_finish_counts(hipStream_t st, const FtCountsArgs &a);
struct FtSrcEntry {
    const uint8_t *ptr;
    long long stride;
};
int ft_launch_upload(hipStream_t st, int batch, const FtSrcEntry *srcTab, int width, int height, uint8_t *slot0, int pitch,
                     size_t slotBytes, const uint8_t **l0Table);
struct FtFisheyeRig {
    float cam1[8], cam2[8], precision, Rlr[9], tlr[3];
    float sigma2[FT_MAX_LEVELS];
};
int ft_launch_fisheye_triangulate(hipStream_t st, const FtFisheyeRig &rig, const ft_keypoint *keysL, int nL,
                                  const ft_keypoint *keysR, int *matches, float *depth, float *p3d, int *nMatches);
int ft_launch_stereo_match(hipStream_t st, const FtGeom &g, int batch, const uint8_t *const *l0L,
                           const uint8_t *const *l0R, int l0pitchL, int l0pitchR, const uint8_t *pyrL,
                           const uint8_t *pyrR, const FtStereoArgs &a);
int ft_launch_stereo_median(hipStream_t st, int batch, const FtStereoArgs &a);
int ft_launch_stereo_rowsort(hipStream_t st, const FtGeom &g, int batch, const FtStereoArgs &a);
int ft_launch_fisheye(hipStream_t st, const uint8_t *descL, int nL, const uint8_t *descR, int nR, int *matches,
                      int *best, int *second);
int ft_launch_hamming_pairs(hipStream_t st, const uint8_t *a, const uint8_t *b, int n, int *dist);
```

### fasttrack_amd/csrc/kernels_extract.hip

```cpp
#include "ft_internal.h"
#include "libm_f32.h"
#include "wave_ops.h"

namespace {


struct FtMomentTab {
    unsigned W[17 * 8], M[17 * 8];
};
constexpr FtMomentTab ft_make_moment_tab() {
    constexpr int umax[16] = {15, 15, 15, 15, 14, 14, 14, 13, 13, 12, 11, 10, 9, 8, 6, 3};
    FtMomentTab t{};
    for (int av = 0; av < 16; av++)
        for (int j = 0; j < 8; j++)
            for (int k = 0; k < 4; k++) {
                const int u = -15 + 4 * j + k;
                const int au = u < 0 ? -u : u;
                if (u <= 15 && au <= umax[av]) {
                    t.W[av * 8 + j] |= (unsigned)(u + 16) << (8 * k);
                    t.M[av * 8 + j] |= 1u << (8 * k);
                }
            }
    return t;
}
// ... 718 lines not shown
        }
        flushB();
    } else if constexpr (TP > 0) {
        const bool act = lane < pw;
        const uint8_t *col = t0 + min(lane, pw - 1) + 3;
        unsigned pA = col[3 * TP], pB = col[4 * TP], pC = col[5 * TP];
        unsigned dA = __builtin_amdgcn_sad_u8(pA, (unsigned)col[0], 0u);
        unsigned dB = __builtin_amdgcn_sad_u8(pB, (unsigned)col[TP], 0u);
        unsigned dC = __builtin_amdgcn_sad_u8(pC, (unsigned)col[2 * TP], 0u);
        for (int y = 0; y < ph; y += FC_ROWS) {
            const uint8_t *r = col + y * TP;
            unsigned pv[FC_ROWS + 3], m01[FC_ROWS], dSv[FC_ROWS], mAny = 0;
            pv[0] = pA; pv[1] = pB; pv[2] = pC;
#pragma unroll
            for (int k = 0; k < FC_ROWS; k++) pv[k + 3] = r[(k + 6) * TP];
#pragma unroll
            for (int k = 0; k < FC_ROWS; k++) {
                const unsigned v = pv[k];
                const uint8_t *cpx = r + (k + 3) * TP;
                const unsigned dS = dSv[k] = __builtin_amdgcn_sad_u8(v, pv[k + 3], 0u);
                const unsigned dN = k == 0 ? dA : k == 1 ? dB : k == 2 ? dC : dSv[k >= 3 ? k - 3 : 0];
                const unsigned m1 = max(FT_AD(3, 0), FT_AD(-3, 0));
                m01[k] = (act && y + k < ph) ? min(max(dN, dS), m1) : 0u;
                mAny = max(mAny, m01[k]);
            }
            dA = dSv[FC_ROWS - 3]; dB = dSv[FC_ROWS - 2]; dC = dSv[FC_ROWS - 1];
            pA = pv[FC_ROWS]; pB = pv[FC_ROWS + 1]; pC = pv[FC_ROWS + 2];
            if (__any(mAny > (unsigned)minTh)) {
#pragma unroll
                for (int k = 0; k < FC_ROWS; k++) nc = pushRow(m01[k] > (unsigned)minTh, pixCode(y + k, lane), nc);
            }
            if (nc > FC_CAND - FC_ROWS * 64 || y + FC_ROWS >= ph) flushB();
        }
    } else {
        for (int base = 0; base < npx; base += 64 * FC_UNROLL) {
            unsigned m01[FC_UNROLL];
            const uint8_t *cp[FC_UNROLL];
            unsigned mAny = 0;
#pragma unroll
            for (int u = 0; u < FC_UNROLL; u++) {
                const int i = base + 64 * u + lane;
                const int ii = min(i, npx - 1);
                const int y = div_by(ii, pwMagic), x = ii - y * pw;
                const uint8_t *cpx = t0 + (y + 3) * tp + (x + 3);
                cp[u] = cpx;
                const unsigned v = cpx[0];
                const unsigned m0 = max(FT_AD(0, 3), FT_AD(0, -3));
                const unsigned m1 = max(FT_AD(3, 0), FT_AD(-3, 0));
                m01[u] = i < npx ? min(m0, m1) : 0u;
                mAny = max(mAny, m01[u]);
            }
            if (__any(mAny > (unsigned)minTh)) {
#pragma unroll
                for (int u = 0; u < FC_UNROLL; u++) {
                    const int i = base + 64 * u + lane;
                    const uint8_t *cpx = cp[u];
                    const unsigned v = cpx[0];
                    const unsigned m2 = max(FT_AD(2, 2), FT_AD(-2, -2));
                    const unsigned m3 = max(FT_AD(2, -2), FT_AD(-2, 2));
                    const bool pass = min(m01[u], min(m2, m3)) > (unsigned)minTh;
                    const unsigned long long b = __ballot(pass);
                    if (pass) cand[nc + __popcll(b & ((1ull << lane) - 1ull))] = (unsigned short)i;
                    nc += __popcll(b);
                }
            }
            if (nc > FC_CAND - 64 * FC_UNROLL || base + 64 * FC_UNROLL >= npx) flushB();
        }
    }
#undef FT_AD
    wave_lds_sync();
    if (dbg & 2) {
        if (lane == 0) *cnt = 0;
        return;
    }
    const bool useList = ncorn <= FC_CORN;
    const int nItems = useList ? ncorn : npx;
    auto nms = [&](int item, int &pix) -> int {
        int y, x;
        if (useList) {
            pix = (int)corn[item];
            y = pixY(pix), x = pixX(pix, y);
        } else {
            const unsigned mg = TP ? div_magic_of((unsigned)pw) : pwMagic;
            y = div_by(item, mg), x = item - y * pw;
            pix = pixCode(y, x);
        }
        const uint8_t *s = score + y * tp + x;
        const unsigned v = s[tp + 1];
        const unsigned m = max(max(max(max((unsigned)s[0], (unsigned)s[1]), (unsigned)s[2]),
                                   max(max((unsigned)s[tp], (unsigned)s[tp + 2]), (unsigned)s[2 * tp])),
                               max((unsigned)s[2 * tp + 1], (unsigned)s[2 * tp + 2]));
        return v > m ? (v >= (unsigned)iniTh ? 2 : 1) : 0;
    };
    uint32_t *out = stage + ((size_t)slot * g.stagePerSlot + rec.outOff);
    int run = 0;
    auto emit = [&](int fl, int pix, int need) {
        const bool f = fl >= need;
        const unsigned long long b = __builtin_amdgcn_ballot_w64(f);
        const int y = pixY(pix), x = pixX(pix, y);
        const int pos = (int)__builtin_amdgcn_mbcnt_hi((unsigned)(b >> 32), __builtin_amdgcn_mbcnt_lo((unsigned)b, (unsigned)run));
        const uint32_t packed = ft_pack_cand(x + (iniX - 13), y + (iniY - 13), score[(y + 1) * tp + (x + 1)]);
        if (f && pos < cellCap) out[pos] = packed;
        run += __popcll(b);
    };
    if (nItems <= 64 * FC_NMS_REG) {
        int fl[FC_NMS_REG], px[FC_NMS_REG], anyHi = 0;
#pragma unroll
        for (int q = 0; q < FC_NMS_REG; q++) {
            fl[q] = 0;
            px[q] = 0;
            if (q * 64 < nItems) {
                const int f = nms(min(q * 64 + lane, nItems - 1), px[q]);
                fl[q] = q * 64 + lane < nItems ? f : 0;
                anyHi |= __any(fl[q] == 2);
            }
        }
        const int need = anyHi ? 2 : 1;
#pragma unroll
        for (int q = 0; q < FC_NMS_REG; q++)
            if (q * 64 < nItems) emit(fl[q], px[q], need);
    } else {
        auto itemPix = [&](int it) -> int {
            if (useList) return (int)corn[it];
            const unsigned mg = TP ? div_magic_of((unsigned)pw) : pwMagic;
            const int y = div_by(it, mg);
            return pixCode(y, it - y * pw);
        };
        unsigned mx = 0;
        for (int base = 0; base < nItems; base += 64) {
            const int pix = itemPix(min(base + lane, nItems - 1));
            const int y = pixY(pix), x = pixX(pix, y);
            mx = max(mx, (unsigned)score[(y + 1) * tp + (x + 1)]);
        }
        int need = __any(mx >= (unsigned)iniTh) ? 2 : 1;
        for (;;) {
            int anyHi = 0;
            run = 0;
            for (int base = 0; base < nItems; base += 64) {
                const int it = base + lane;
                int pix = 0;
                const int f = nms(min(it, nItems - 1), pix);
                const int fl = it < nItems ? f : 0;
                anyHi |= __any(fl == 2);
                emit(fl, pix, need);
            }
            if (need == 1 || anyHi) break;
            need = 1;
        }
    }
    if (lane == 0) *cnt = min(run, cellCap);
}

__global__ __launch_bounds__(256) void k_compact(FtGeom g, const int *cellCount, const uint32_t *stage,
                                                 uint32_t *cand, int *candCount) {
    extern __shared__ __attribute__((aligned(16))) uint8_t smem[];
    int *offs = (int *)smem;
    __shared__ int wsum[4];
    const int tid = threadIdx.x, lane = tid & 63, wave = tid >> 6;
    const int level = blockIdx.x, slot = blockIdx.y;
    const FtLevelGeom &L = g.lv[level];
    const int nCells = L.nCols * L.nRows;
    const int *cnt = cellCount + (size_t)slot * g.totalCells + L.cellBase;
    const int per = (nCells + 255) / 256;
    const int c0 = tid * per, c1 = min(c0 + per, nCells);
    int local = 0;
    for (int c = c0; c < c1; c++) local += cnt[c];
    int incl = local;
#pragma unroll
    for (int o = 1; o < 64; o <<= 1) {
        int t = __shfl_up(incl, o);
        if (lane >= o) incl += t;
    }
    if (lane == 63) wsum[wave] = incl;
    __syncthreads();
    int wbase = 0, total = 0;
#pragma unroll
    for (int w = 0; w < 4; w++) {
        if (w < wave) wbase += wsum[w];
        total += wsum[w];
    }
    int run = wbase + incl - local;
    for (int c = c0; c < c1; c++) {
        offs[c] = run;
        run += cnt[c];
    }
    if (tid == 0) offs[nCells] = total;
    __syncthreads();
    total = min(total, L.candCap);
    const uint32_t *st = stage + (size_t)slot * g.stagePerSlot + L.stageBase;
    uint32_t *dst = cand + (size_t)slot * g.candPerSlot + L.candBase;
    for (int o = tid; o < total; o += 256) {
        int lo = 0, hi = nCells;
        while (hi - lo > 1) {
            int mid = (lo + hi) >> 1;
            if (offs[mid] <= o) lo = mid;
            else hi = mid;
        }
        dst[o] = st[(size_t)lo * L.cellCap + (o - offs[lo])];
    }
    if (tid == 0) candCount[slot * g.nlevels + level] = total;
}

#define OD_R 21
#define OD_P (2 * OD_R + 1)
#define OD_PP 48
#define OD_HP 40
#ifndef OD_LAYOUT
#define OD_LAYOUT 1
#endif
#ifndef OD_RP
#define OD_RP 44
#endif
#define OD_RAW_BYTES (OD_P * OD_PP)
#define OD_HB_BYTES (OD_LAYOUT ? OD_HP * OD_RP * 2 + 16 : OD_P * OD_HP * 2)
#define OD_WAVE_BYTES ((OD_RAW_BYTES + OD_HB_BYTES + 15) & ~15)
#define OD_WAVES 4
#ifndef OD_MFMA
#define OD_MFMA 0
#endif
#if OD_MFMA && !OD_LAYOUT
#error "OD_MFMA writes the column-major layout"
#endif
#define OD_BIAS (OD_MFMA ? 0x80808080u : 0u)
#ifndef OD_KPW_WIDE
#define OD_KPW_WIDE 2
#endif

__device__ __forceinline__ int reflect101(int i, int n) {
    if (i < 0) i = -i;
    if (i >= n) i = 2 * (n - 1) - i;
    return i;
}

__device__ __forceinline__ void od_hblur4(unsigned d0, unsigned d1, unsigned d2, unsigned &h0, unsigned &h1, unsigned &h2, unsigned &h3) {
#define FT_W4(a, b, c, d) ((unsigned)(a) | ((unsigned)(b) << 8) | ((unsigned)(c) << 16) | ((unsigned)(d) << 24))
    const unsigned W0a = FT_W4(18, 34, 48, 56), W0b = FT_W4(48, 34, 18, 0);
    const unsigned W1a = FT_W4(0, 18, 34, 48), W1b = FT_W4(56, 48, 34, 18);
    const unsigned W2a = FT_W4(0, 0, 18, 34), W2b = FT_W4(48, 56, 48, 34), W2c = FT_W4(18, 0, 0, 0);
    const unsigned W3a = FT_W4(0, 0, 0, 18), W3b = FT_W4(34, 48, 56, 48), W3c = FT_W4(34, 18, 0, 0);
#undef FT_W4
    h0 = __builtin_amdgcn_udot4(d1, W0b, __builtin_amdgcn_udot4(d0, W0a, 0u, false), false);
    h1 = __builtin_amdgcn_udot4(d1, W1b, __builtin_amdgcn_udot4(d0, W1a, 0u, false), false);
    h2 = __builtin_amdgcn_udot4(d2, W2c, __builtin_amdgcn_udot4(d1, W2b, __builtin_amdgcn_udot4(d0, W2a, 0u, false), false), false);
    h3 = __builtin_amdgcn_udot4(d2, W3c, __builtin_amdgcn_udot4(d1, W3b, __builtin_amdgcn_udot4(d0, W3a, 0u, false), false), false);
}
__device__ __forceinline__ unsigned od_vblur7(unsigned p0, unsigned p1, unsigned p2, unsigned p3, unsigned p4, unsigned p5, unsigned p6) {
    unsigned v;
    asm("v_mad_u32_u24 %0, %1, 18, %2" : "=v"(v) : "v"(p0 + p6), "s"(32768u));
    asm("v_mad_u32_u24 %0, %1, 34, %2" : "=v"(v) : "v"(p1 + p5), "v"(v));
    asm("v_mad_u32_u24 %0, %1, 48, %2" : "=v"(v) : "v"(p2 + p4), "v"(v));
    asm("v_mad_u32_u24 %0, %1, 56, %2" : "=v"(v) : "v"(p3), "v"(v));
    return v >> 16;
}

typedef unsigned short od_us2 __attribute__((ext_vector_type(2)));
typedef int od_v4i __attribute__((ext_vector_type(4)));
__device__ __forceinline__ unsigned od_dot2(unsigned a, unsigned w, unsigned acc) {
    return __builtin_amdgcn_udot2(__builtin_bit_cast(od_us2, a), __builtin_bit_cast(od_us2, w), acc, false);
}
__device__ __forceinline__ unsigned od_vblur7_pairs(unsigned e0, unsigned e1, unsigned e2, unsigned e3) {
    const unsigned W01 = 18u | (34u << 16), W23 = 48u | (56u << 16), W45 = 48u | (34u << 16), W6 = 18u;
    return od_dot2(e3, W6, od_dot2(e2, W45, od_dot2(e1, W23, od_dot2(e0, W01, 32768u)))) >> 16;
}
__device__ __forceinline__ unsigned od_vblur7_dwords(unsigned d0, unsigned d1, unsigned d2, unsigned d3, unsigned sh) {
    return od_vblur7_pairs(__builtin_amdgcn_alignbit(d1, d0, sh), __builtin_amdgcn_alignbit(d2, d1, sh),
                           __builtin_amdgcn_alignbit(d3, d2, sh), d3 >> (sh & 31u));
}

typedef short od_s2 __attribute__((ext_vector_type(2)));
__device__ __forceinline__ int od_sdot2(unsigned a, unsigned w, int acc) {
    return __builtin_amdgcn_sdot2(__builtin_bit_cast(od_s2, a), __builtin_bit_cast(od_s2, w), acc, false);
}
__device__ __forceinline__ unsigned od_vblur7_dwords_s(unsigned d0, unsigned d1, unsigned d2, unsigned d3, unsigned sh) {
    const unsigned W01 = 18u | (34u << 16), W23 = 48u | (56u << 16), W45 = 48u | (34u << 16), W6 = 18u;
    const unsigned e0 = __builtin_amdgcn_alignbit(d1, d0, sh), e1 = __builtin_amdgcn_alignbit(d2, d1, sh),
                   e2 = __builtin_amdgcn_alignbit(d3, d2, sh), e3 = d3 >> (sh & 31u);
    return (unsigned)od_sdot2(e3, W6, od_sdot2(e2, W45, od_sdot2(e1, W23, od_sdot2(e0, W01, 32768 + 256 * 32768)))) >> 16;
}

__global__ void k_blur_level(const uint8_t *img, int pitch, int w, int h, uint8_t *dst, int dstPitch) {
    const int gx = (blockIdx.x * blockDim.x + threadIdx.x) * 4, y = blockIdx.y;
    if (gx >= w || y >= h) return;
    unsigned hb[7][4];
    for (int s = 0; s < 7; s++) {
        const uint8_t *row = img + (size_t)reflect101(y + s - 3, h) * pitch;
        unsigned d[3] = {0u, 0u, 0u};
        for (int b = 0; b < 12; b++) d[b >> 2] |= (unsigned)row[reflect101(gx - 3 + b, w)] << (8 * (b & 3));
        od_hblur4(d[0], d[1], d[2], hb[s][0], hb[s][1], hb[s][2], hb[s][3]);
    }
    for (int j = 0; j < 4 && gx + j < w; j++) {
#if OD_LAYOUT
        const unsigned t[8] = {hb[0][j], hb[1][j], hb[2][j], hb[3][j], hb[4][j], hb[5][j], hb[6][j], 0u};
        unsigned v;
        if ((gx + j + y) & 1) v = od_vblur7_dwords(t[0] << 16, t[1] | (t[2] << 16), t[3] | (t[4] << 16), t[5] | (t[6] << 16), 16u);
        else v = od_vblur7_dwords(t[0] | (t[1] << 16), t[2] | (t[3] << 16), t[4] | (t[5] << 16), t[6], 0u);
        dst[(size_t)y * dstPitch + gx + j] = (uint8_t)v;
#else
        dst[(size_t)y * dstPitch + gx + j] = (uint8_t)od_vblur7(hb[0][j], hb[1][j], hb[2][j], hb[3][j], hb[4][j], hb[5][j], hb[6][j]);
#endif
    }
}

__device__ __forceinline__ float fast_atan2_deg(float y, float x) {
    const float p1 = 0.9997878412794807f * (float)(180 / 3.14159265358979323846);
    const float p3 = -0.3258083974640975f * (float)(180 / 3.14159265358979323846);
    const float p5 = 0.1555786518463281f * (float)(180 / 3.14159265358979323846);
    const float p7 = -0.04432655554792128f * (float)(180 / 3.14159265358979323846);
    const float eps = (float)2.2204460492503131e-16;
    const float ax = fabsf(x), ay = fabsf(y);
    float a, c, c2;
    if (ax >= ay) {
        c = __fdiv_rn(ay, __fadd_rn(ax, eps));
// ... 328 lines not shown
        mxSum = std::max(mxSum, t + sc);
    }
    return (TP ? mxTile + mxScore : mxSum) + fc_list_bytes();
}

static bool pyr_rows_fits(const FtGeom &g, int level) {
    const FtLevelGeom &D = g.lv[level], &P = g.lv[level - 1];
    return (double)P.w / (double)D.w < 2.5 && P.w >= 8;
}

int ft_launch_pyramid(hipStream_t st, const FtGeom &g, int batch, const uint8_t *const *l0, int l0pitch,
                      uint8_t *pyr, const FtTap *taps, int alignedLoads, int rowsKernel, const FtPyrBands *bands) {
    const bool rowsOn = rowsKernel != 0;
    bool cascade = rowsKernel == 2 && batch >= 8 && alignedLoads && bands && bands->K >= 1 && g.nlevels >= 2;
    for (int level = 1; cascade && level < g.nlevels; level++) cascade = pyr_rows_fits(g, level);
    if (cascade) {
        dim3 grid, block(64 * PC_WAVES, 1, 1);
        const FtSlotGrid sg = ft_slot_grid(bands->K, batch, grid);
        const int readableEnd = std::min((g.lv[0].w + 3) & ~3, l0pitch);
        for (int rep = ft_debug_repeat("pyr"); rep > 0; rep--)
            hipLaunchKernelGGL(k_pyr_cascade, grid, block, 0, st, g, l0, l0pitch, pyr, taps, sg, *bands, readableEnd);
        FT_HIP(hipGetLastError());
        return FT_OK;
    }
    for (int rep = ft_debug_repeat("pyr"); rep > 0; rep--)
    for (int level = 1; level < g.nlevels; level++) {
        const FtLevelGeom &D = g.lv[level], &P = g.lv[level - 1];
        if (rowsOn && batch >= 8 && alignedLoads && pyr_rows_fits(g, level)) {
            const int stripsX = (D.w + PR_COLS - 1) / PR_COLS, stripsY = (D.h + PR_RB - 1) / PR_RB;
            dim3 grid, block(64, 1, 1);
            const FtSlotGrid sg = ft_slot_grid(stripsX * stripsY, batch, grid);
            const int readableEnd = level == 1 ? std::min((P.w + 3) & ~3, l0pitch) : P.pitch;
            if (D.area2x)
                hipLaunchKernelGGL(k_pyr_rows<true>, grid, block, 0, st, g, level, l0, l0pitch, pyr, taps, sg, stripsX,
                                   div_magic_of((unsigned)stripsX), readableEnd);
            else
                hipLaunchKernelGGL(k_pyr_rows<false>, grid, block, 0, st, g, level, l0, l0pitch, pyr, taps, sg, stripsX,
                                   div_magic_of((unsigned)stripsX), readableEnd);
            continue;
        }
        const int cols = (int)((long long)PD_TW * P.w / D.w) + 8, rowsN = (int)((long long)PD_TH * P.h / D.h) + 8;
        const int ldsPitch = (cols + 3 + 3) & ~3;
        const unsigned sxQ16 = (unsigned)(((unsigned long long)P.w << 16) / (unsigned)D.w) + 1u;
        const unsigned syQ16 = (unsigned)(((unsigned long long)P.h << 16) / (unsigned)D.h) + 1u;
        const int tilesX = (D.w + PD_TW - 1) / PD_TW, tilesY = (D.h + PD_TH - 1) / PD_TH;
        dim3 grid, block(64, 1, 1);
        const FtSlotGrid sg = ft_slot_grid(tilesX * tilesY, batch, grid);
        hipLaunchKernelGGL(k_pyr_down, grid, block, (size_t)ldsPitch * rowsN + 4, st, g, level, l0, l0pitch, pyr, taps,
                           alignedLoads, ldsPitch, rowsN, sxQ16, syQ16, sg, tilesX, div_magic_of((unsigned)tilesX));
    }
    FT_HIP(hipGetLastError());
    return FT_OK;
}

static size_t fast_smem_of(const FtGeom &g, unsigned mask, int TP, int *tileBytes, int *scoreBytes) {
    size_t mxTile = 0, mxScore = 0, mxSum = 0;
    for (int l = 0; l < g.nlevels; l++) {
        const FtLevelGeom &L = g.lv[l];
        if (!((mask >> l) & 1u) || L.nCols * L.nRows <= 0) continue;
        const size_t t = (size_t)fc_tile_bytes(L.wCell, L.hCell, TP), sc = (size_t)fc_score_bytes(L.wCell, L.hCell, TP);
        mxTile = std::max(mxTile, t);
        mxScore = std::max(mxScore, sc);
        mxSum = std::max(mxSum, t + sc);
    }
    if (tileBytes) *tileBytes = (int)mxTile;
    if (scoreBytes) *scoreBytes = (int)mxScore;
    return (TP ? mxTile + mxScore : mxSum) + fc_list_bytes();
}

static bool fast_cell_ranges(const FtGeom &g, unsigned mask, FtCellRanges &cr) {
    int runs = 0, lo[2] = {0, 0}, n[2] = {0, 0};
    bool open = false;
    for (int l = 0; l < g.nlevels; l++) {
        const int cells = g.lv[l].nCols * g.lv[l].nRows;
        if (cells <= 0) continue;
        if ((mask >> l) & 1u) {
            if (!open) {
                if (runs == 2) return false;
                lo[runs] = g.lv[l].cellBase;
                n[runs] = 0;
                runs++;
                open = true;
            }
            n[runs - 1] += cells;
        } else {
            open = false;
        }
    }
    cr.lo0 = lo[0]; cr.n0 = n[0]; cr.lo1 = lo[1]; cr.n1 = n[1];
    return runs > 0;
}

int ft_launch_fast_cells(hipStream_t st, const FtGeom &g, int batch, const uint8_t *const *l0, int l0pitch,
                         const uint8_t *pyr, int iniTh, int minTh, int alignedLoads, int *cellCount,
                         uint32_t *stage, int ordered, const FtCellRec *cellTab) {
    if (g.totalCells == 0) return FT_OK;
    typedef void (*FastFn)(FtGeom, const uint8_t *const *, int, const uint8_t *, int, int, int, int *, uint32_t *, const FtCellRec *,
                           FtSlotGrid, int, int, int, FtCellRanges);
    static const int dbg = ft_debug_env("FT_DEBUG_FAST") ? atoi(ft_debug_env("FT_DEBUG_FAST")) : 0;
    static const bool occDbg = ft_debug_env("FT_DEBUG_OCC") != nullptr;
    static const bool noSplit = ft_debug_env("FT_DEBUG_FAST_NOSPLIT") != nullptr;
    const unsigned all = (1u << g.nlevels) - 1u;
    unsigned mask48 = 0, mask64 = 0, maskAny = 0;
    for (int l = 0; l < g.nlevels; l++) {
        if (g.lv[l].nCols * g.lv[l].nRows <= 0) continue;
        const int need = g.lv[l].wCell + 9;
        (need <= 48 ? mask48 : need <= 64 ? mask64 : maskAny) |= 1u << l;
    }
    struct Part { unsigned mask; int TP; };
    Part parts[3];
    int nParts = 0;
    FtCellRanges probe;
    const bool splittable = !noSplit && !maskAny && mask48 && mask64 && fast_cell_ranges(g, mask48, probe) && fast_cell_ranges(g, mask64, probe);
    if (splittable) {
        parts[nParts++] = {mask48, 48};
        parts[nParts++] = {mask64, 64};
    } else {
        parts[nParts++] = {all, fast_tile_pitch(g)};
    }
    const int runBlock = 8 * FC_XCD_RUN;
    for (int pi = 0; pi < nParts; pi++) {
        const int TP = parts[pi].TP;
        FtCellRanges cr;
        if (!fast_cell_ranges(g, parts[pi].mask, cr)) {
            cr.lo0 = 0; cr.n0 = g.totalCells; cr.lo1 = 0; cr.n1 = 0;
        }
        if (nParts == 1) { cr.lo0 = 0; cr.n0 = g.totalCells; cr.lo1 = 0; cr.n1 = 0; }
        const int nCells = cr.n0 + cr.n1;
        int tileBytes = 0, scoreBytes = 0;
        const size_t smem = fast_smem_of(g, parts[pi].mask, TP, &tileBytes, &scoreBytes);
        dim3 grid(((nCells + runBlock - 1) / runBlock) * runBlock, batch, 1), block(64, 1, 1);
        FtSlotGrid sg;
        sg.blocksPerSlot = 0; sg.batch = batch; sg.xcdMap = 0; sg.magic = 0;
        if (batch >= 8) sg = ft_slot_grid(nCells, batch, grid);
        const FastFn fn = TP == 48 ? (ordered ? k_fast_cells<48, true> : k_fast_cells<48, false>)
                          : TP == 64 ? (ordered ? k_fast_cells<64, true> : k_fast_cells<64, false>)
                                     : k_fast_cells<0, true>;
        if (smem > 64 * 1024)
            FT_HIP(hipFuncSetAttribute((const void *)fn, hipFuncAttributeMaxDynamicSharedMemorySize, (int)smem));
        if (occDbg) {
            int nb = 0;
            hipOccupancyMaxActiveBlocksPerMultiprocessor(&nb, (const void *)fn, 64, smem);
            fprintf(stderr, "[ft] k_fast_cells<%d,%d>: %d cells per image, %zu B of LDS per wave, %d waves per CU\n", TP, ordered, nCells, smem, nb);
        }
        for (int rep = ft_debug_repeat("fast"); rep > 0; rep--)
            hipLaunchKernelGGL(fn, grid, block, smem, st, g, l0, l0pitch, pyr, iniTh, minTh, alignedLoads, cellCount, stage, cellTab, sg, dbg,
                               tileBytes, scoreBytes, cr);
    }
    FT_HIP(hipGetLastError());
    return FT_OK;
}

int ft_launch_compact(hipStream_t st, const FtGeom &g, int batch, const int *cellCount, const uint32_t *stage,
                      uint32_t *cand, int *candCount) {
    int maxCells = 0;
    for (int l = 0; l < g.nlevels; l++) maxCells = std::max(maxCells, g.lv[l].nCols * g.lv[l].nRows);
    dim3 grid2(g.nlevels, batch, 1), block(256, 1, 1);
    for (int rep = ft_debug_repeat("compact"); rep > 0; rep--)
    hipLaunchKernelGGL(k_compact, grid2, block, (size_t)(maxCells + 1) * sizeof(int), st, g, cellCount, stage, cand,
                       candCount);
    FT_HIP(hipGetLastError());
    return FT_OK;
}

int ft_launch_blur_level(hipStream_t st, const uint8_t *img, int pitch, int w, int h, uint8_t *dst, int dstPitch) {
    dim3 grid(((w + 3) / 4 + 63) / 64, h, 1), block(64, 1, 1);
    hipLaunchKernelGGL(k_blur_level, grid, block, 0, st, img, pitch, w, h, dst, dstPitch);
    FT_HIP(hipGetLastError());
    return FT_OK;
}

int ft_launch_orient_desc(hipStream_t st, const FtGeom &g, int batch, const uint8_t *const *l0, int l0pitch,
                          const uint8_t *pyr, int alignedLoads, const FtSelKp *sel, const int *selCount,
                          const FtOctArgs &layout, int *nSel, ft_keypoint *keys, uint8_t *desc) {
    dim3 grid, block(64 * OD_WAVES, 1, 1);
    const int kpw = batch >= 8 ? OD_KPW_WIDE : 1;
    const FtSlotGrid sg = ft_slot_grid((g.maxKp + OD_WAVES * kpw - 1) / (OD_WAVES * kpw), batch, grid);
    const size_t smem = OD_WAVES * (size_t)OD_WAVE_BYTES;
    static const bool occDbg = ft_debug_env("FT_DEBUG_OCC") != nullptr;
    if (occDbg) {
        int nb = 0;
        hipOccupancyMaxActiveBlocksPerMultiprocessor(&nb, kpw == 1 ? (const void *)k_orient_desc<1> : (const void *)k_orient_desc<OD_KPW_WIDE>,
                                                     64 * OD_WAVES, smem);
        fprintf(stderr, "[ft] k_orient_desc<%d>: %zu B of LDS per workgroup, %d workgroups per CU\n", kpw, smem, nb);
    }
    static const int prof = ft_debug_env("FT_DEBUG_OD_PROFILE") ? 1 : 0;
    for (int rep = ft_debug_repeat("orient"); rep > 0; rep--) {
        if (kpw == 1)
            hipLaunchKernelGGL(k_orient_desc<1>, grid, block, smem, st, g, l0, l0pitch, pyr, alignedLoads, sel, selCount, layout,
                               nSel, keys, desc, sg, 0);
        else
            hipLaunchKernelGGL(k_orient_desc<OD_KPW_WIDE>, grid, block, smem, st, g, l0, l0pitch, pyr, alignedLoads, sel, selCount,
                               layout, nSel, keys, desc, sg, prof);
    }
    if (prof && kpw > 1) {
        static int launches = 0;
        if (++launches % 64 == 0) {
            unsigned long long h[16];
            if (hipMemcpyFromSymbol(h, HIP_SYMBOL(g_odProf), sizeof h) == hipSuccess && h[0]) {
                static const char *names[9] = {"loads (level, selection, patches)", "stage 0", "moments 0", "hblur 0", "stage 1 + moments 1",
                                               "angles", "samples 0 + stores", "hblur 1", "samples 1 + stores"};
                double tot = 0;
                for (int k = 0; k < 9; k++) tot += (double)h[1 + k];
                fprintf(stderr, "[ft] k_orient_desc<2> wave life, %llu sampled waves, %.2f us per wave:\n", h[0], tot / h[0] / 100.0);
                for (int k = 0; k < 9; k++) fprintf(stderr, "[ft]   %-36s %6.2f us  %5.1f %%\n", names[k], h[1 + k] / (double)h[0] / 100.0, 100.0 * h[1 + k] / tot);
            }
        }
    }
    FT_HIP(hipGetLastError());
    return FT_OK;
}
```

### fasttrack_amd/csrc/kernels_octree.hip

```cpp
#include "ft_internal.h"
#include "octree_paths.h"

namespace {

using ft::op::kMaxDepth;
using ft::op::Roots;
using ft::op::SortElem;
using ft::op::SortFrame;

__device__ __forceinline__ void wave_lds_sync() {
    __builtin_amdgcn_fence(__ATOMIC_ACQ_REL, "wavefront");
    __builtin_amdgcn_wave_barrier();
}

__device__ __forceinline__ int wave_excl_scan(int v, int lane, int &total) {
    (void)lane;
    int x = v;
    x += __builtin_amdgcn_update_dpp(0, x, 0x111, 0xF, 0xF, true);
    x += __builtin_amdgcn_update_dpp(0, x, 0x112, 0xF, 0xF, true);
    x += __builtin_amdgcn_update_dpp(0, x, 0x114, 0xF, 0xF, true);
    x += __builtin_amdgcn_update_dpp(0, x, 0x118, 0xF, 0xF, true);
    x += __builtin_amdgcn_update_dpp(0, x, 0x142, 0xA, 0xF, true);
    x += __builtin_amdgcn_update_dpp(0, x, 0x143, 0xC, 0xF, true);
    total = __builtin_amdgcn_readlane(x, 63);
// ... 113 lines not shown
            key = (unsigned)__shfl((int)key, partner);
            val = (unsigned)__shfl((int)val, partner);
            wave_lds_sync();
            if (sp < 64) {
                if (lane == sp) frames = (unsigned)(cut | (hi << 8) | (depth << 16));
                sp++;
            }
            hi = cut;
        }
    }
    if (lane < len) a[f + lane] = SortElem{key, val};
    wave_lds_sync();
}

__device__ __forceinline__ void wave_std_sort(SortElem *a, int n, SortFrame *stack, uint16_t *posA, uint16_t *posB, SortElem *tmp, int lane) {
    if (n <= 1) return;
    int lg = 0;
    for (int t = n; t > 1; t >>= 1) lg++;
    int sp = 0;
    if (lane == 0) stack[0] = SortFrame{0, (uint16_t)n, (uint16_t)(2 * lg), 0};
    sp = 1;
    wave_lds_sync();
    const unsigned long long below = (1ull << lane) - 1;
    while (sp > 0) {
        const SortFrame fr = stack[--sp];
        int f = fr.f, l = fr.l, depth = fr.depth;
        wave_lds_sync();
        while (l - f > 16) {
            if (l - f <= 64) {
                wave_sort_window(a, f, l, depth, (uint8_t *)posA, (uint8_t *)posB, lane);
                break;
            }
            if (depth == 0) {
                if (lane == 0) ft::op::ss_heap_sort(a + f, a + l);
                wave_lds_sync();
                break;
            }
            --depth;
            const int ia = f + 1, ib = f + (l - f) / 2, ic = l - 1;
            const uint32_t ka = a[ia].key, kb = a[ib].key, kc = a[ic].key;
            int pick;
            if (ka < kb) pick = (kb < kc) ? ib : (ka < kc) ? ic : ia;
            else pick = (ka < kc) ? ia : (kb < kc) ? ic : ib;
            const uint32_t pv = (pick == ia) ? ka : (pick == ib) ? kb : kc;
            if (lane == 0) {
                const SortElem t0 = a[f], t1 = a[pick];
                a[f] = t1;
                a[pick] = t0;
            }
            wave_lds_sync();
            int nA = 0, nB = 0;
            for (int i0 = f + 1; i0 < l; i0 += 64) {
                const int i = i0 + lane;
                const bool valid = i < l;
                const uint32_t x = valid ? a[i].key : 0u;
                const bool isA = valid && !(x < pv), isB = valid && !(pv < x);
                const unsigned long long bA = __ballot(isA), bB = __ballot(isB);
                if (isA) posA[nA + __popcll(bA & below)] = (uint16_t)i;
                if (isB) posB[nB + __popcll(bB & below)] = (uint16_t)i;
                nA += __popcll(bA);
                nB += __popcll(bB);
            }
            wave_lds_sync();
            int K = 0;
            const int nPair = min(nA, nB);
            for (int k0 = 0; k0 < nPair; k0 += 64) {
                const int k = k0 + lane;
                bool sw = false;
                int pa = 0, pb = 0;
                if (k < nPair) {
                    pa = posA[k];
                    pb = posB[nB - 1 - k];
                    sw = pa < pb;
                }
                const unsigned long long bs = __ballot(sw);
                if (sw) {
                    const SortElem t0 = a[pa], t1 = a[pb];
                    a[pa] = t1;
                    a[pb] = t0;
                }
                K += __popcll(bs);
                if (bs != ~0ull) break;
            }
            const int bK = K ? (int)posB[nB - K] : l;
            const int aK = K < nA ? (int)posA[K] : 0x7fffffff;
            const int cut = aK < bK ? aK : bK;
            wave_lds_sync();
            if (sp < 64) {
                if (lane == 0) stack[sp] = SortFrame{(uint16_t)cut, (uint16_t)l, (uint16_t)depth, 0};
                sp++;
            }
            l = cut;
        }
        wave_lds_sync();
    }
    for (int i = lane; i < n; i += 64) {
        const SortElem e = a[i];
        uint32_t kl[16], kr[16];
#pragma unroll
        for (int d = 0; d < 16; d++) {
            kl[d] = a[max(i - 1 - d, 0)].key;
            kr[d] = a[min(i + 1 + d, n - 1)].key;
        }
        int pos = i;
#pragma unroll
        for (int d = 0; d < 16; d++) {
            pos -= (i - 1 - d >= 0) && kl[d] > e.key;
            pos += (i + 1 + d <= n - 1) && kr[d] < e.key;
        }
        tmp[pos] = e;
    }
    wave_lds_sync();
    for (int i = lane; i < n; i += 64) a[i] = tmp[i];
    wave_lds_sync();
}

constexpr int OCT_THREADS = 512;
#ifndef OCT_SORT_STAGES
#define OCT_SORT_STAGES 2
#endif
static_assert(OCT_SORT_STAGES >= 1 && OCT_SORT_STAGES <= 4, "bitonic_pass is instantiated for 1 .. 4 stages");

template <int S>
__device__ __forceinline__ void bitonic_pass(unsigned long long *keys, int nPad, int k, int p, int tid) {
    constexpr int E = 1 << S;
    const int q = p - S + 1;
    for (int t = tid; t < (nPad >> S); t += OCT_THREADS) {
        const int i = ((t >> q) << (p + 1)) + (t & ((1 << q) - 1));
        unsigned long long e[E];
#pragma unroll
        for (int r = 0; r < E; r++) e[r] = keys[i + (r << q)];
        const bool up = (i & k) == 0;
#pragma unroll
        for (int d = E >> 1; d > 0; d >>= 1) {
#pragma unroll
            for (int r = 0; r < E; r++) {
                if (r & d) continue;
                const unsigned long long x = e[r], y = e[r | d];
                const unsigned long long lo = x < y ? x : y, hi = x < y ? y : x;
                e[r] = up ? lo : hi;
                e[r | d] = up ? hi : lo;
            }
        }
#pragma unroll
        for (int r = 0; r < E; r++) keys[i + (r << q)] = e[r];
    }
    __syncthreads();
}

enum { OM_START = 0, OM_M = 1, OM_CURB = 2, OM_GAVEUP = 3, OM_WAVESUM = 4  };

template <bool HIST>
__device__ __forceinline__ bool oct_level(const FtGeom &g, const FtOctArgs &a, const int slot, const int level, const int maxN,
                                          uint8_t *smem, uint32_t *lowG = nullptr) {
    const int tid = threadIdx.x;
    const int lane = tid & 63;
    const FtLevelGeom &L = g.lv[level];
    const int n = a.candCount[slot * g.nlevels + level];
    const int N = a.quota[level];
    int *cntOut = a.selCount + slot * g.nlevels + level;
    if (n <= 0) {
        if (tid == 0) *cntOut = 0;
        return true;
    }
    const unsigned wMagic = L.wCell > 1 ? 0xffffffffu / (unsigned)L.wCell + 1u : 0u;
    const unsigned hMagic = L.hCell > 1 ? 0xffffffffu / (unsigned)L.hCell + 1u : 0u;
    const int minB = FT_EDGE_THRESHOLD - 3;
    const Roots R = ft::op::make_roots(minB, L.maxBX, minB, L.maxBY);
    const bool keyFits = L.nCols <= 128 && L.nRows <= 128 && L.wCell <= 128 && L.hCell <= 128 && R.nIni <= 15;
    auto fail = [&]() {
        if (tid == 0) {
            *cntOut = 0;
            atomicOr(a.overflow, 1);
            a.ovSlot[slot] = 1;
        }
    };
    auto hand_on = [&](int *cnt, unsigned *list, int cap) -> bool {
        const int idx = atomicAdd(cnt, 1);
        atomicMax(cnt + 2, idx + 1);
        if (idx >= cap) return false;
        list[idx] = (unsigned)slot | ((unsigned)level << 16);
        return true;
    };
    if constexpr (!HIST) {
        if (n > maxN && keyFits && (a.histCap > 0 || a.histWanted || maxN < a.bigN)) {
            if (tid == 0) {
                bool ok;
                if ((a.histCap > 0 || a.histWanted) && n <= 65535) ok = hand_on(a.bigCount, a.bigList, a.histCap);
                else if (n <= a.bigN) ok = hand_on(a.bigCount + 1, a.sortList, a.sortCap);
                else ok = false;
                if (!ok) {
                    *cntOut = 0;
                    atomicOr(a.overflow, 1);
                    a.ovSlot[slot] = 1;
                }
            }
            return true;
        }
        if (n > maxN || !keyFits) {
            fail();
            return true;
        }
    } else {
        if (n > 65535 || !keyFits) {
            fail();
            return true;
        }
    }
    const uint32_t *cand = a.cand + (size_t)slot * g.candPerSlot + L.candBase;
    const int cap = a.poolCap;
    const OctLds o = oct_lds_layout(cap, HIST ? oct_hist_key_bytes() : maxN * 8, HIST, lowG != nullptr);
    const bool compact = !HIST && o.low != 0;
    unsigned long long *keys = (unsigned long long *)(smem + o.keys);
    const uint32_t *codes = (const uint32_t *)keys + (compact ? 0 : 1);
    const int codeShift = compact ? 0 : 1;
    uint32_t *bins32 = (uint32_t *)(smem + o.keys);
    uint16_t *bins = (uint16_t *)(smem + o.keys);
    int *misc = (int *)(smem + o.misc);
    auto lohiOf = [&](int b) -> uint32_t * { return (uint32_t *)(smem + (b ? o.lohi[1] : o.lohi[0])); };
    auto x01Of = [&](int b) -> uint32_t * { return (uint32_t *)(smem + (b ? o.x01[1] : o.x01[0])); };
    auto depOf = [&](int b) -> uint8_t * { return smem + (b ? o.dep[1] : o.dep[0]); };
    auto preOf = [&](int b) -> uint32_t * { return (uint32_t *)(smem + (b ? o.pre[1] : o.pre[0])); };
    SortElem *vSize = (SortElem *)(smem + o.vSize);
    SortElem *vPrev = (SortElem *)(smem + o.vPrev);
    uint16_t *ord = (uint16_t *)(smem + o.ord);
    uint16_t *bq = (uint16_t *)(smem + o.bq);
    uint32_t *pq = (uint32_t *)(smem + o.pq);
    uint8_t *mark = smem + o.mark;
    SortFrame *stack = (SortFrame *)(smem + o.stack);
    const int D = HIST ? ft::op::hist_depth(R.nIni, FT_OCT_HIST_BINS) : 0;
    const int nBins = HIST ? R.nIni << (2 * D) : 0;
    const int perThread = HIST ? (nBins + OCT_THREADS - 1) / OCT_THREADS : 0;

    const bool prof = a.prof && slot == 0;
    unsigned long long tPrev = prof ? wall_clock64() : 0;
    int profIdx = 0;
    auto tick = [&]() {
        if (!prof) return;
        const unsigned long long t = wall_clock64();
        if (tid == 0 && profIdx < 8) a.prof[level * 8 + profIdx] += t - tPrev;
        profIdx++;
        tPrev = t;
    };
    auto emission_key = [&](int x, int y) -> unsigned {
        const int cj = min(wMagic ? (int)__umulhi((unsigned)(x - 3), wMagic) : x - 3, L.nCols - 1);
        const int ci = min(hMagic ? (int)__umulhi((unsigned)(y - 3), hMagic) : y - 3, L.nRows - 1);
        return ((unsigned)ci << 21) | ((unsigned)cj << 14) | ((unsigned)(y - 3 - ci * L.hCell) << 7) | (unsigned)(x - 3 - cj * L.wCell);
    };
    if constexpr (!HIST) {
        int nPad = 64;
        while (nPad < n) nPad <<= 1;
        for (int i = tid; i < nPad; i += OCT_THREADS) {
            unsigned long long k = ~0ull;
            if (i < n) {
                const uint32_t c = cand[i];
                const int x = (int)(c & 0xfffu), y = (int)((c >> 12) & 0xfffu);
                k = ((unsigned long long)ft::op::path_code(R, x, y) << 36) | ((unsigned long long)(c >> 24) << 28) | emission_key(x, y);
            }
            keys[i] = k;
        }
        __syncthreads();
        tick();
        {
            int m = 1;
            for (int k = 2; k <= nPad; k <<= 1, m++) {
                int p = m - 1;
                const int first = m % OCT_SORT_STAGES;
                if (first == 1) bitonic_pass<1>(keys, nPad, k, p, tid);
                else if (first == 2) bitonic_pass<2>(keys, nPad, k, p, tid);
                else if (first == 3) bitonic_pass<3>(keys, nPad, k, p, tid);
                p -= first;
                for (; p >= OCT_SORT_STAGES - 1; p -= OCT_SORT_STAGES) bitonic_pass<OCT_SORT_STAGES>(keys, nPad, k, p, tid);
            }
        }
        tick();
        if (compact) {
            uint32_t *packed = (uint32_t *)keys;
            for (int base = 0; base < n; base += 8 * OCT_THREADS) {
                unsigned long long kk[8];
#pragma unroll
                for (int j = 0; j < 8; j++) {
                    const int i = base + j * OCT_THREADS + tid;
                    kk[j] = i < n ? keys[i] : 0ull;
                }
                __syncthreads();
#pragma unroll
                for (int j = 0; j < 8; j++) {
                    const int i = base + j * OCT_THREADS + tid;
                    if (i < n) {
                        packed[i] = (uint32_t)(kk[j] >> 32);
                        lowG[i] = (uint32_t)kk[j];
                    }
                }
                __syncthreads();
            }
        }
        if (tid >= 64) return true;
    } else {
        for (int i = tid; i <= (nBins >> 1); i += OCT_THREADS) bins32[i] = 0;
        if (tid == 0) misc[OM_GAVEUP] = 0;
        __syncthreads();
        for (int i = tid; i < n; i += OCT_THREADS) {
            const uint32_t c = cand[i];
            const unsigned b = ft::op::path_prefix(R, (int)(c & 0xfffu), (int)((c >> 12) & 0xfffu), D);
            atomicAdd(&bins32[b >> 1], 1u << ((b & 1u) * 16u));
        }
        __syncthreads();
        tick();
        {
            const int b0 = min(tid * perThread, nBins), b1 = min(b0 + perThread, nBins);
            int sum = 0;
            for (int b = b0; b < b1; b++) sum += bins[b];
            int tot;
            int ex = wave_excl_scan(sum, lane, tot);
            if (lane == 63) misc[OM_WAVESUM + (tid >> 6)] = tot;
            __syncthreads();
            for (int w = 0; w < (tid >> 6); w++) ex += misc[OM_WAVESUM + w];
            for (int b = b0; b < b1; b++) {
                const int c = bins[b];
                bins[b] = (uint16_t)ex;
                ex += c;
            }
            if (tid == OCT_THREADS - 1) bins[nBins] = (uint16_t)n;
            __syncthreads();
        }
        tick();
    }
    int curB = 0, start = cap, m = 0;
    bool gaveUp = false;
    if (tid < 64) {
    auto lower_bound = [&](int lo, int hi, uint32_t target) {
        while (lo < hi) {
            const int mid = (lo + hi) >> 1;
            if (codes[mid << codeShift] < (target << 4)) lo = mid + 1;
            else hi = mid;
        }
        return lo;
    };
    for (int s0 = 0; s0 < R.nIni; s0 += 64) {
        const int s = s0 + lane;
        int lo = 0, hi = 0;
        if (s < R.nIni) {
            if constexpr (HIST) {
                lo = bins[s << (2 * D)];
                hi = bins[(s + 1) << (2 * D)];
            } else {
                lo = lower_bound(0, n, (uint32_t)s << (2 * kMaxDepth));
                hi = lower_bound(lo, n, (uint32_t)(s + 1) << (2 * kMaxDepth));
            }
        }
        const bool has = hi > lo;
        const unsigned long long bal = __ballot(has);
        if (has) {
            const int pos = start + m + __popcll(bal & ((1ull << lane) - 1));
            int x0, x1;
            ft::op::root_bounds(R, s, x0, x1);
            lohiOf(0)[pos] = (uint32_t)lo | ((uint32_t)hi << 16);
            x01Of(0)[pos] = (uint32_t)x0 | ((uint32_t)x1 << 16);
            depOf(0)[pos] = 0;
            if constexpr (HIST) preOf(0)[pos] = (uint32_t)s;
        }
        m += __popcll(bal);
    }
// ... 149 lines not shown
            }
            wave_lds_sync();
        }
        split_round(nOrd, false);
        if (gaveUp) break;
        if (m >= N || m == prevSize) {
            finish = true;
        } else if (m + 3 * nV > N) {
            while (!finish) {
                prevSize = m;
                const int nPrev = nV;
                for (int k = lane; k < nPrev; k += 64) vPrev[k] = vSize[k];
                wave_lds_sync();
                const unsigned long long ts = prof ? wall_clock64() : 0;
                wave_std_sort(vPrev, nPrev, stack, bq, bq + cap, vSize, lane);
                if (prof && lane == 0) {
                    a.prof[level * 8 + 4] += wall_clock64() - ts;
                    a.prof[level * 8 + 5] += (unsigned long long)nPrev;
                    a.prof[level * 8 + 6] += 1;
                }
                for (int r = lane; r < nPrev; r += 64) ord[r] = (uint16_t)vPrev[nPrev - 1 - r].val;
                wave_lds_sync();
                split_round(nPrev, true);
                if (gaveUp) break;
                if (m >= N || m == prevSize) finish = true;
            }
            if (gaveUp) break;
        }
    }
    if constexpr (HIST) {
        if (lane == 0) {
            misc[OM_START] = start;
            misc[OM_M] = m;
            misc[OM_CURB] = curB;
            misc[OM_GAVEUP] = gaveUp ? 1 : 0;
        }
    }
    }
    tick();
    FtSelKp *out = a.sel + (size_t)slot * g.maxKp + a.selOff[level];
    const unsigned long long low = (1ull << 36) - 1, inv = (1ull << 28) - 1;
    auto write_out = [&](int t, unsigned long long best) {
        const unsigned ek = (unsigned)(~best) & (unsigned)inv;
        const int bx = (int)((ek >> 14) & 127u) * L.wCell + (int)(ek & 127u) + 3;
        const int by = (int)((ek >> 21) & 127u) * L.hCell + (int)((ek >> 7) & 127u) + 3;
        FtSelKp s;
        s.x = (short)(bx + minB);
        s.y = (short)(by + minB);
        s.level = (short)level;
        s.response = (short)(best >> 28);
        out[t] = s;
    };
    if constexpr (!HIST) {
        const int kept = min(m, a.levelMax[level]);
        const uint32_t *cl = lohiOf(curB);
        if (compact) {
            uint32_t *lowL = (uint32_t *)(smem + o.low);
            wave_lds_sync();
            for (int base = 0; base < n; base += 8 * 64) {
                uint32_t v[8];
#pragma unroll
                for (int j = 0; j < 8; j++) {
                    const int i = base + j * 64 + lane;
                    v[j] = i < n ? __hip_atomic_load(lowG + i, __ATOMIC_RELAXED, __HIP_MEMORY_SCOPE_AGENT) : 0u;
                }
#pragma unroll
                for (int j = 0; j < 8; j++) {
                    const int i = base + j * 64 + lane;
                    if (i < n) lowL[i] = v[j];
                }
            }
            wave_lds_sync();
            for (int t = lane; t < kept; t += 64) {
                const unsigned lh = cl[start + t];
                const int lo = (int)(lh & 0xffffu), hi = (int)(lh >> 16);
                unsigned long long best = 0;
                for (int k = lo; k < hi; k++)
                    best = max(best, (((unsigned long long)(codes[k] & 0xfu) << 32) | lowL[k]) ^ inv);
                write_out(t, best);
            }
        } else {
            for (int t = lane; t < kept; t += 64) {
                const unsigned lh = cl[start + t];
                const int lo = (int)(lh & 0xffffu), hi = (int)(lh >> 16);
                unsigned long long best = (keys[lo] & low) ^ inv;
                for (int k = lo + 1; k < hi; k++) best = max(best, (keys[k] & low) ^ inv);
                write_out(t, best);
            }
        }
        tick();
        if (lane == 0) *cntOut = kept;
        return true;
    } else {
        __syncthreads();
        if (misc[OM_GAVEUP]) return false;
        start = misc[OM_START];
        m = misc[OM_M];
        curB = misc[OM_CURB];
        const int kept = min(m, a.levelMax[level]);
        unsigned long long *best = (unsigned long long *)(smem + o.best);
        __syncthreads();
        for (int b = tid; b < nBins; b += OCT_THREADS) bins[b] = 0;
        for (int t = tid; t < kept; t += OCT_THREADS) best[t] = 0;
        __syncthreads();
        {
            const uint32_t *cp = preOf(curB);
            const uint8_t *cd = depOf(curB);
            for (int t = tid; t < m; t += OCT_THREADS) bins[cp[start + t] << (2 * (D - (int)cd[start + t]))] = (uint16_t)(t + 1);
        }
        __syncthreads();
        {
            const int b0 = min(tid * perThread, nBins), b1 = min(b0 + perThread, nBins);
            int last = 0;
            for (int b = b0; b < b1; b++) {
                const int v = bins[b];
                last = v ? v : last;
            }
            const unsigned long long has = __ballot(last != 0);
            const unsigned long long below = has & ((1ull << lane) - 1ull);
            const int src = below ? 63 - __clzll((long long)below) : 0;
            const int fromWave = __shfl(last, src);
            const int waveLast = __shfl(last, has ? 63 - __clzll((long long)has) : 0);
            if (lane == 0) misc[OM_WAVESUM + (tid >> 6)] = has ? waveLast : 0;
            __syncthreads();
            int carry = 0;
            for (int w = 0; w < (tid >> 6); w++) {
                const int v = misc[OM_WAVESUM + w];
                carry = v ? v : carry;
            }
            if (below) carry = fromWave;
            for (int b = b0; b < b1; b++) {
                const int v = bins[b];
                carry = v ? v : carry;
                bins[b] = (uint16_t)carry;
            }
        }
        __syncthreads();
        tick();
        for (int i = tid; i < n; i += OCT_THREADS) {
            const uint32_t c = cand[i];
            const int x = (int)(c & 0xfffu), y = (int)((c >> 12) & 0xfffu);
            const int t1 = bins[ft::op::path_prefix(R, x, y, D)];
            if (t1 >= 1 && t1 <= kept)
                atomicMax(&best[t1 - 1], ((((unsigned long long)(c >> 24)) << 28) | (unsigned long long)emission_key(x, y)) ^ inv);
        }
        __syncthreads();
        for (int t = tid; t < kept; t += OCT_THREADS) write_out(t, best[t]);
        tick();
        if (tid == 0) *cntOut = kept;
        return true;
    }
}

__global__ __launch_bounds__(OCT_THREADS) void k_octree(FtGeom g, FtOctArgs a) {
    extern __shared__ __attribute__((aligned(16))) uint8_t smem[];
    __builtin_amdgcn_s_setprio(3);
    oct_level<false>(g, a, blockIdx.x, blockIdx.y, FT_OCT_MAXN, smem,
                     a.low ? a.low + ((size_t)blockIdx.x * g.nlevels + blockIdx.y) * FT_OCT_MAXN : nullptr);
}

__global__ __launch_bounds__(OCT_THREADS) void k_octree_hist(FtGeom g, FtOctArgs a) {
    extern __shared__ __attribute__((aligned(16))) uint8_t smem[];
    const int cnt = min(a.bigCount[0], a.histCap);
    if ((int)blockIdx.x >= cnt) return;
    __builtin_amdgcn_s_setprio(3);
    for (int ei = (int)blockIdx.x; ei < cnt; ei += (int)gridDim.x) {
        const unsigned e = a.bigList[ei];
        const int slot = (int)(e & 0xffffu), level = (int)(e >> 16);
        const bool done = oct_level<true>(g, a, slot, level, 0, smem);
        if (!done && threadIdx.x == 0) {
            const int n = a.candCount[slot * g.nlevels + level];
            bool ok = false;
            if (n <= a.bigN) {
                const int idx = atomicAdd(a.bigCount + 1, 1);
                atomicMax(a.bigCount + 3, idx + 1);
                if (idx < a.sortCap) {
                    a.sortList[idx] = e;
                    ok = true;
                }
            }
            if (!ok) {
                a.selCount[slot * g.nlevels + level] = 0;
                atomicOr(a.overflow, 1);
                a.ovSlot[slot] = 1;
            }
        }
        __syncthreads();
    }
}

__global__ __launch_bounds__(OCT_THREADS) void k_octree_auto(FtGeom g, FtOctArgs a) {
    extern __shared__ __attribute__((aligned(16))) uint8_t smem[];
    __builtin_amdgcn_s_setprio(3);
    const int slot = (int)blockIdx.x, level = (int)blockIdx.y;
    const int n = a.candCount[slot * g.nlevels + level];
    const int N = a.quota[level];
    bool done = false;
    if (2 * n >= 3 * N || n > FT_OCT_MAXN) done = oct_level<true>(g, a, slot, level, 0, smem);
    if (done) return;
    if (n <= FT_OCT_MAXN) {
        __syncthreads();
        oct_level<false>(g, a, slot, level, FT_OCT_MAXN, smem, a.low ? a.low + ((size_t)slot * g.nlevels + level) * FT_OCT_MAXN : nullptr);
        return;
    }
    if (threadIdx.x == 0) {
        bool ok = false;
        if (n <= a.bigN) {
            const int idx = atomicAdd(a.bigCount + 1, 1);
            atomicMax(a.bigCount + 3, idx + 1);
            if (idx < a.sortCap) {
                a.sortList[idx] = (unsigned)slot | ((unsigned)level << 16);
                ok = true;
            }
        }
        if (!ok) {
            a.selCount[slot * g.nlevels + level] = 0;
            atomicOr(a.overflow, 1);
            a.ovSlot[slot] = 1;
        }
    }
}

__global__ __launch_bounds__(OCT_THREADS) void k_octree_big(FtGeom g, FtOctArgs a) {
    extern __shared__ __attribute__((aligned(16))) uint8_t smem[];
    const int cnt = min(a.bigCount[1], a.sortCap);
    if ((int)blockIdx.x >= cnt) return;
    const unsigned e = a.sortList[blockIdx.x];
    oct_level<false>(g, a, (int)(e & 0xffffu), (int)(e >> 16), a.bigN, smem);
}

}

size_t ft_octree_smem_bytes(int poolCap, bool compact) { return (size_t)oct_lds_layout(poolCap, FT_OCT_MAXN * 8, false, compact).total; }
size_t ft_octree_hist_smem_bytes(int poolCap) { return (size_t)oct_lds_layout(poolCap, oct_hist_key_bytes(), true).total; }
int ft_octree_big_keys(int poolCap) {
    for (int n = 16384; n > FT_OCT_MAXN; n >>= 1)
        if ((size_t)oct_lds_layout(poolCap, n * 8, false).total <= 160 * 1024) return n;
    return 0;
}

int ft_launch_octree(hipStream_t st, const FtGeom &g, int batch, const FtOctArgs &a) {
    const size_t smem = ft_octree_smem_bytes(a.poolCap, a.low != nullptr);
    if (ft_debug_env("FT_DEBUG_OCC")) fprintf(stderr, "[ft] k_octree: %zu B of LDS per workgroup (pool %d)\n", smem, a.poolCap);
    if (smem > 64 * 1024)
        FT_HIP(hipFuncSetAttribute((const void *)k_octree, hipFuncAttributeMaxDynamicSharedMemorySize, (int)smem));
    const size_t smemHist = a.histCap > 0 ? ft_octree_hist_smem_bytes(a.poolCap) : 0;
    if (smemHist > 64 * 1024)
        FT_HIP(hipFuncSetAttribute((const void *)k_octree_hist, hipFuncAttributeMaxDynamicSharedMemorySize, (int)smemHist));
    const size_t smemBig = a.bigN ? (size_t)oct_lds_layout(a.poolCap, a.bigN * 8, false).total : 0;
    if (a.bigN && a.sortCap > 0)
        FT_HIP(hipFuncSetAttribute((const void *)k_octree_big, hipFuncAttributeMaxDynamicSharedMemorySize, (int)smemBig));
    if (a.histFirst) {
        const size_t smemAll = std::max(ft_octree_hist_smem_bytes(a.poolCap), smem);
        if (smemAll > 64 * 1024)
            FT_HIP(hipFuncSetAttribute((const void *)k_octree_auto, hipFuncAttributeMaxDynamicSharedMemorySize, (int)smemAll));
        for (int rep = ft_debug_repeat("octree"); rep > 0; rep--) {
            if (a.bigN) FT_HIP(hipMemsetAsync(a.bigCount, 0, 2 * sizeof(int), st));
            hipLaunchKernelGGL(k_octree_auto, dim3(batch, g.nlevels), dim3(OCT_THREADS), smemAll, st, g, a);
            if (a.bigN && a.sortCap > 0) hipLaunchKernelGGL(k_octree_big, dim3(a.sortCap), dim3(OCT_THREADS), smemBig, st, g, a);
        }
        FT_HIP(hipGetLastError());
        return FT_OK;
    }
    for (int rep = ft_debug_repeat("octree"); rep > 0; rep--) {
        if (a.bigN || a.histCap > 0 || a.histWanted) FT_HIP(hipMemsetAsync(a.bigCount, 0, 2 * sizeof(int), st));
        hipLaunchKernelGGL(k_octree, dim3(batch, g.nlevels), dim3(OCT_THREADS), smem, st, g, a);
        if (a.histCap > 0) hipLaunchKernelGGL(k_octree_hist, dim3(std::min(a.histCap, std::max(a.histGrid, 1))), dim3(OCT_THREADS), smemHist, st, g, a);
        if (a.bigN && a.sortCap > 0) hipLaunchKernelGGL(k_octree_big, dim3(a.sortCap), dim3(OCT_THREADS), smemBig, st, g, a);
    }
    FT_HIP(hipGetLastError());
    return FT_OK;
}
```

### fasttrack_amd/csrc/matcher.cpp

```cpp
#include <algorithm>
#include <cstring>
#include <memory>

#include "ft_host.h"

#define FT_GRAPH_MAX_BATCH 8

static bool sameGeometry(const ft_extractor *a, const ft_extractor *b) {
    return a->width == b->width && a->height == b->height && a->nlevels == b->nlevels &&
           a->scaleFactor == b->scaleFactor && a->ctx == b->ctx;
}

struct StereoSide {
    const ft_keypoint *keys;
    const uint8_t *desc;
    const int *n;
};
static FtStereoArgs stereoArgs(StereoSide l, StereoSide r, int capacity, float *uright, float *depth, int *sad, int *hamIdx, int *nMatches,
                               int medianCut, int *rowStart, int rowStride, FtSortedR *sorted, int *leftOrder, float mbf, float mb,
                               bool aligned) {
    FtStereoArgs a{};
    a.keysL = l.keys;
    a.keysR = r.keys;
    a.descL = l.desc;
// ... 104 lines not shown
    std::unique_ptr<ft_stereo_frontend, int (*)(ft_stereo_frontend *)> guard(fe, ft_stereo_frontend_destroy);
    fe->ctx = ctx;
    fe->mbf = mbf;
    fe->mb = mb;
    fe->maxBatch = max_batch;
    const bool pairedOn = ctx->tuning.paired != 0;
    fe->pairedCapable = pairedOn && max_batch >= 1 && max_batch <= FT_GRAPH_MAX_BATCH;
    FT_CHECK(ft_extractor_create(ctx, nfeatures, scale_factor, nlevels, ini_th_fast, min_th_fast, image_width, image_height,
                                 fe->pairedCapable ? 2 * max_batch : max_batch, &fe->exL));
    FT_CHECK(ft_extractor_create(ctx, nfeatures, scale_factor, nlevels, ini_th_fast, min_th_fast, image_width, image_height,
                                 max_batch, &fe->exR));
    fe->capacity = fe->exL->geom.maxKp;
    const size_t n = (size_t)max_batch * fe->capacity;
    FtOwned &own = fe->own;
    FT_CHECK(own.devAlloc(&fe->d_uright, n));
    FT_CHECK(own.devAlloc(&fe->d_depth, n));
    FT_CHECK(own.devAlloc(&fe->d_sad, n));
    FT_CHECK(own.devAlloc(&fe->d_nMatches, max_batch));
    FT_CHECK(own.devAlloc(&fe->d_sorted, n));
    FT_CHECK(own.devAlloc(&fe->d_rowStart, (size_t)max_batch * (image_height + 2)));
    FT_CHECK(own.devAlloc(&fe->d_leftOrder, n));
    FT_CHECK(own.pinAlloc(&fe->h_uright, n));
    FT_CHECK(own.pinAlloc(&fe->h_depth, n));
    FT_CHECK(own.pinAlloc(&fe->h_nMatches, max_batch));
    FT_CHECK(own.event(&fe->evFork));
    FT_CHECK(own.event(&fe->evJoin));
    for (int i = 0; i < 2; i++) FT_CHECK(own.event(&fe->evDone[i]));
    *out = guard.release();
    return FT_OK;
}

int ft_stereo_frontend_destroy(ft_stereo_frontend *fe) {
    if (!fe) return FT_OK;
    hipSetDevice(fe->ctx->device);
    ft_extractor_destroy(fe->exL);
    ft_extractor_destroy(fe->exR);
    if (fe->graphExec) hipGraphExecDestroy(fe->graphExec);
    fe->own.release();
    delete fe;
    return FT_OK;
}

ft_extractor *ft_stereo_frontend_left(ft_stereo_frontend *fe) { return fe ? fe->exL : nullptr; }
ft_extractor *ft_stereo_frontend_right(ft_stereo_frontend *fe) { return fe ? fe->exR : nullptr; }

static FtStereoArgs frontendStereoArgs(const ft_stereo_frontend *fe, int b0, StereoSide r, bool aligned) {
    const ft_extractor *L = fe->exL;
    const int maxKp = L->geom.maxKp, rowStride = L->height + 2;
    const size_t o = (size_t)b0 * maxKp;
    return stereoArgs({L->d_keys + o, L->d_desc + o * 32, L->d_nSel + b0}, r, maxKp, fe->d_uright + o, fe->d_depth + o, fe->d_sad + o,
                      nullptr, fe->d_nMatches + b0, 1, fe->d_rowStart + (size_t)b0 * rowStride, rowStride, fe->d_sorted + o,
                      fe->d_leftOrder + o, fe->mbf, fe->mb, aligned);
}
static FtDeliverArgs frontendDeliverArgs(const ft_stereo_frontend *fe, StereoSide r, const int *overflowR, bool direct, ft_keypoint *keysL,
                                         uint8_t *descL, ft_keypoint *keysR, uint8_t *descR, float *uright, float *depth, int capacity) {
    const ft_extractor *L = fe->exL, *R = fe->exR;
    FtDeliverArgs d = ft_deliver_args(L);
    d.keysR = r.keys;
    d.descR = r.desc;
    d.nR = r.n;
    d.overflowR = overflowR;
    d.uright = fe->d_uright;
    d.depth = fe->d_depth;
    d.nMatches = fe->d_nMatches;
    if (direct) {
        d.oKeysL = keysL;
        d.oDescL = descL;
        d.dstStride = capacity;
    }
    d.oKeysR = direct ? keysR : R->h_keys;
    d.oDescR = direct ? descR : R->h_desc;
    d.oUright = direct ? uright : fe->h_uright;
    d.oDepth = direct ? depth : fe->h_depth;
    d.oNR = R->h_nSel;
    d.oNMatches = fe->h_nMatches;
    d.oOverflowR = R->h_overflow;
    return d;
}

static int frontendMatchAndDeliver(ft_stereo_frontend *fe, int s, int b0, int nb, bool dev, bool deliver, bool direct,
                                   ft_keypoint *keysL, uint8_t *descL, ft_keypoint *keysR, uint8_t *descR, int capacity,
                                   float *uright, float *depth) {
    ft_extractor *L = fe->exL, *R = fe->exR;
    const FtGeom &g = L->geom;
    const bool tm = fe->ctx->kernelTiming;
    hipStream_t st = L->streamB;
    int rc;
    const size_t kp = sizeof(ft_keypoint);
    auto d2h = [&](void *user, void *staging, const void *dev, size_t elem, int b0, int nb, int maxN) -> hipError_t {
        const size_t o = (size_t)b0 * g.maxKp * elem;
        if (direct) {
            if (!user) return hipSuccess;
            return hipMemcpy2DAsync((uint8_t *)user + (size_t)b0 * capacity * elem, elem * capacity, (const uint8_t *)dev + o,
                                    elem * g.maxKp, elem * maxN, nb, hipMemcpyDeviceToHost, st);
        }
        return hipMemcpy2DAsync((uint8_t *)staging + o, elem * g.maxKp, (const uint8_t *)dev + o, elem * g.maxKp, elem * maxN,
                                nb, hipMemcpyDeviceToHost, st);
    };
    FT_HIP(hipEventRecord(R->evB[s], R->streamB));
    FT_HIP(hipStreamWaitEvent(st, R->evB[s], 0));
    const size_t o = (size_t)b0 * g.maxKp;
    const FtStereoArgs a = frontendStereoArgs(fe, b0, {R->d_keys + o, R->d_desc + o * 32, R->d_nSel + b0}, L->l0Aligned && R->l0Aligned);
    L->evt.begin(tm, "kernel.stereo_rowsort", st);
    rc = ft_launch_stereo_rowsort(st, g, nb, a);
    L->evt.end(tm, st);
    if (rc != FT_OK) return rc;
    L->evt.begin(tm, "kernel.stereo_match", st);
    rc = ft_launch_stereo_match(st, g, nb, L->d_l0 + b0, R->d_l0 + b0, L->l0pitch, R->l0pitch,
                                L->d_pyr + (size_t)b0 * g.pyrPerSlot, R->d_pyr + (size_t)b0 * g.pyrPerSlot, a);
    L->evt.end(tm, st);
    if (rc != FT_OK) return rc;
    L->evt.begin(tm, "kernel.stereo_median", st);
    rc = ft_launch_stereo_median(st, nb, a);
    L->evt.end(tm, st);
    if (rc != FT_OK) return rc;
    int maxNL = 0, maxNR = 0;
    for (int b = b0; b < b0 + nb; b++) {
        maxNL = std::max(maxNL, dev ? g.maxKp : L->h_nSel[b]);
        maxNR = std::max(maxNR, dev ? g.maxKp : R->h_nSel[b]);
    }
    if (!dev && (maxNL > capacity || maxNR > capacity)) {
        ft_set_error("stereo front end: output capacity too small (use ft_extractor_max_keypoints)");
        return FT_ERR_CAPACITY;
    }
    if (deliver) return FT_OK;
    if (maxNL > 0) {
        FT_HIP(d2h(keysL, L->h_keys, L->d_keys, kp, b0, nb, maxNL));
        FT_HIP(d2h(descL, L->h_desc, L->d_desc, 32, b0, nb, maxNL));
        FT_HIP(d2h(uright, fe->h_uright, fe->d_uright, 4, b0, nb, maxNL));
        FT_HIP(d2h(depth, fe->h_depth, fe->d_depth, 4, b0, nb, maxNL));
    }
    if (maxNR > 0) {
        FT_HIP(d2h(keysR, R->h_keys, R->d_keys, kp, b0, nb, maxNR));
        FT_HIP(d2h(descR, R->h_desc, R->d_desc, 32, b0, nb, maxNR));
    }
    FT_HIP(hipMemcpyAsync(fe->h_nMatches + b0, fe->d_nMatches + b0, sizeof(int) * nb, hipMemcpyDeviceToHost, st));
    return FT_OK;
}

static int frontendEnqueue(ft_stereo_frontend *fe, const uint8_t *const *imagesL, const uint8_t *const *imagesR, int batch,
                           int on_device, int width, int height, int stride, ft_keypoint *keysL, uint8_t *descL, int *nL,
                           ft_keypoint *keysR, uint8_t *descR, int *nR, int capacity, float *uright, float *depth,
                           int *n_matches, bool direct, int capture, bool paired) {
    ft_extractor *L = fe->exL, *R = fe->exR;
    const FtGeom &g = L->geom;
    FtTimer tAll;
    fe->lastPaired = paired;
    if (paired) {
        const int B = batch;
        std::vector<const uint8_t *> imgs(imagesL, imagesL + B);
        imgs.insert(imgs.end(), imagesR, imagesR + B);
        FT_CHECK(ft_extract_prepare(L, imgs.data(), 2 * B, on_device, width, height, stride));
        fe->ctx->addStat("stereo.device_octree_batches", 0);
        FT_CHECK(ft_extract_launch_a(L, 0, 2 * B, nullptr));
        FT_CHECK(ft_extract_launch_octree(L, 0, 0, 2 * B, L->evA[0]));
        hipStream_t st = L->streamB;
        FT_HIP(hipStreamWaitEvent(st, L->evA[0], 0));
        FT_CHECK(ft_extract_launch_b(L, 0, 2 * B, st));
        const size_t oR = (size_t)B * g.maxKp;
        const StereoSide right = {L->d_keys + oR, L->d_desc + oR * 32, L->d_nSel + B};
        const FtStereoArgs a = frontendStereoArgs(fe, 0, right, L->l0Aligned);
        FT_CHECK(ft_launch_stereo_rowsort(st, g, B, a));
        FT_CHECK(ft_launch_stereo_match(st, g, B, L->d_l0, L->d_l0 + B, L->l0pitch, L->l0pitch, L->d_pyr,
                                        L->d_pyr + (size_t)B * g.pyrPerSlot, a));
        FT_CHECK(ft_launch_stereo_median(st, B, a));
        FT_CHECK(ft_launch_deliver(st, B, frontendDeliverArgs(fe, right, L->d_overflow, direct, keysL, descL, keysR, descR, uright, depth, capacity)));
        R->lastBatch = B;
        if (capture) {
            FT_HIP(hipEventRecord(fe->evJoin, st));
            FT_HIP(hipStreamWaitEvent(L->stream, fe->evJoin, 0));
        }
        fe->ctx->addStat("stereo.submit.total", tAll.ms());
        return FT_OK;
    }
    if (capture) {
        FT_HIP(hipEventRecord(fe->evFork, L->stream));
        FT_HIP(hipStreamWaitEvent(R->stream, fe->evFork, 0));
    }
    int rc = ft_extract_prepare(L, imagesL, batch, on_device, width, height, stride);
    if (rc != FT_OK) return rc;
    rc = ft_extract_prepare(R, imagesR, batch, on_device, width, height, stride);
    if (rc != FT_OK) return rc;
    const int S = ft_pipeline_depth(L->tune, batch, L->deviceOctree && R->deviceOctree);
    const int sb = (batch + S - 1) / S;
    const bool dev = L->deviceOctree && R->deviceOctree;
    if (!dev) L->deviceOctree = R->deviceOctree = false;
    if (dev) fe->ctx->addStat("stereo.device_octree_batches", 0);
    for (int s = 0, b0 = 0; b0 < batch; s++, b0 += sb) {
        const int nb = std::min(sb, batch - b0);
        rc = ft_extract_launch_a(L, b0, nb, dev ? nullptr : L->evA[s]);
        if (rc == FT_OK && dev) rc = ft_extract_launch_octree(L, s, b0, nb, L->evA[s]);
        if (rc != FT_OK) return rc;
        rc = ft_extract_launch_a(R, b0, nb, dev ? nullptr : R->evA[s]);
        if (rc == FT_OK && dev) rc = ft_extract_launch_octree(R, s, b0, nb, R->evA[s]);
        if (rc != FT_OK) return rc;
    }
    hipStream_t st = L->streamB;
    const bool deliver = dev && batch <= FT_GRAPH_MAX_BATCH;
    double tOct = 0, tWait = 0, tLaunch = 0;
    for (int s = 0, b0 = 0; b0 < batch; s++, b0 += sb) {
        const int nb = std::min(sb, batch - b0);
        if (dev) {
            FT_HIP(hipStreamWaitEvent(L->streamB, L->evA[s], 0));
            FT_HIP(hipStreamWaitEvent(R->streamB, R->evA[s], 0));
        } else {
            FtTimer tW;
            FT_HIP(hipEventSynchronize(L->evA[s]));
            FT_HIP(hipEventSynchronize(R->evA[s]));
            tWait += tW.ms();
            FtTimer tO;
            ft_extractor *both[2] = {L, R};
            rc = ft_extract_octree_multi(both, 2, b0, nb);
            if (rc != FT_OK) return rc;
            tOct += tO.ms();
        }
        FtTimer tL;
        rc = ft_extract_launch_b(L, b0, nb, L->streamB);
        if (rc != FT_OK) return rc;
        rc = ft_extract_launch_b(R, b0, nb, R->streamB);
        if (rc != FT_OK) return rc;
        rc = frontendMatchAndDeliver(fe, s, b0, nb, dev, deliver, direct, keysL, descL, keysR, descR, capacity, uright, depth);
        if (rc != FT_OK) return rc;
        tLaunch += tL.ms();
    }
    if (deliver) {
        FT_CHECK(ft_launch_deliver(st, batch, frontendDeliverArgs(fe, {R->d_keys, R->d_desc, R->d_nSel}, R->d_overflow, direct, keysL, descL,
                                                                  keysR, descR, uright, depth, capacity)));
    } else {
        FT_CHECK(ft_extract_finish_counts(L, batch, st));
        FT_CHECK(ft_extract_finish_counts(R, batch, st));
    }
    if (capture) {
        FT_HIP(hipEventRecord(fe->evJoin, st));
        FT_HIP(hipStreamWaitEvent(L->stream, fe->evJoin, 0));
    }
    if (!dev) fe->ctx->addStat("stereo.octree(host,both)", tOct);
    fe->ctx->addStat("stereo.host_wait_stageA", tWait);
    fe->ctx->addStat("stereo.host_launch_stageB", tLaunch);
    fe->ctx->addStat("stereo.submit.total", tAll.ms());
    return FT_OK;
}

int ft_stereo_frontend_submit(ft_stereo_frontend *fe, const uint8_t *const *imagesL, const uint8_t *const *imagesR,
                              int batch, int on_device, int width, int height, int stride, ft_keypoint *keysL,
                              uint8_t *descL, int *nL, ft_keypoint *keysR, uint8_t *descR, int *nR, int capacity,
                              float *uright, float *depth, int *n_matches) {
    FT_REQUIRE(fe, "null front end");
    FT_REQUIRE(!fe->pending.active, "stereo front end: a submitted batch has not been waited for");
    if (!imagesL || !imagesR || width <= 0 || height <= 0) {
        ft_set_error("stereo front end: empty image");
        return FT_ERR_EMPTY;
    }
    ft_extractor *L = fe->exL, *R = fe->exR;
    const FtGeom &g = L->geom;
    int rc = ft_set_device(fe->ctx);
    if (rc != FT_OK) return rc;
    FT_REQUIRE(batch >= 1 && batch <= fe->maxBatch, "stereo front end: batch outside [1, max_batch]");
    rc = ft_extract_foreign_wait(L);
    if (rc == FT_OK) rc = ft_extract_foreign_wait(R);
    if (rc != FT_OK) return rc;
    const bool dev = L->deviceOctree && R->deviceOctree;
    const bool paired = fe->pairedCapable && dev && batch <= FT_GRAPH_MAX_BATCH && 2 * batch <= L->maxBatch;
    const bool direct = ft_is_pinned_host(keysL) && ft_is_pinned_host(descL) && ft_is_pinned_host(keysR) && ft_is_pinned_host(descR) &&
                        ft_is_pinned_host(uright) && ft_is_pinned_host(depth) && (!dev || capacity >= g.maxKp);
    bool launched = false, useGraph = L->tune.graph != 0 && !fe->graphDisabled && L->ownStreams && R->ownStreams && dev && direct &&
                                      !fe->ctx->kernelTiming && batch <= FT_GRAPH_MAX_BATCH && width == L->width && height == L->height &&
                                      stride >= width;
    for (int b = 0; b < batch && useGraph; b++)
        if (!imagesL[b] || !imagesR[b]) useGraph = false;
    if (useGraph && !on_device && (ft_extract_ensure_stage(L) != FT_OK || ft_extract_ensure_stage(R) != FT_OK)) {
        (void)hipGetLastError();
        useGraph = false;
    }
    if (useGraph) {
        ft_stereo_frontend::GraphKey key;
        key.batch = batch; key.onDevice = on_device; key.width = width; key.height = height; key.stride = stride;
        key.capacity = capacity;
        key.paired = paired ? 1 : 0;
        key.bigGridL = L->bigGrid + (L->histOn ? (1 << 24) : 0);
        key.bigGridR = R->bigGrid + (R->histOn ? (1 << 24) : 0);
        key.alignedL = !on_device || ft_frames_aligned(imagesL, batch, stride);
        key.alignedR = !on_device || ft_frames_aligned(imagesR, batch, stride);
        if (paired) key.alignedL = key.alignedR = key.alignedL & key.alignedR;
        const void *outs[6] = {keysL, descL, keysR, descR, uright, depth};
        for (int i = 0; i < 6; i++) key.out[i] = outs[i];
        if (fe->graphExec && key == fe->graphKey) {
            if (paired) {
                std::vector<const uint8_t *> imgs(imagesL, imagesL + batch);
                imgs.insert(imgs.end(), imagesR, imagesR + batch);
                ft_extract_rebind(L, imgs.data(), 2 * batch, on_device, width, height, stride);
                R->lastBatch = batch;
            } else {
                ft_extract_rebind(L, imagesL, batch, on_device, width, height, stride);
                ft_extract_rebind(R, imagesR, batch, on_device, width, height, stride);
            }
            fe->lastPaired = paired;
            fe->ctx->addStat("stereo.device_octree_batches", 0);
            FtTimer tG;
            FT_HIP(hipGraphLaunch(fe->graphExec, L->stream));
            fe->ctx->addStat("stereo.graph_launch", tG.ms());
            launched = true;
        } else {
            L->stageHost = R->stageHost = !on_device;
            launched = ft_graph_capture(L->stream, &fe->graphExec, [&] {
                return frontendEnqueue(fe, imagesL, imagesR, batch, on_device, width, height, stride, keysL, descL, nL, keysR, descR, nR,
                                       capacity, uright, depth, n_matches, direct, 1, paired);
            });
            L->stageHost = R->stageHost = false;
            fe->graphDisabled = !launched;
            if (launched) fe->graphKey = key;
            fe->ctx->addStat(launched ? "stereo.graph_captures" : "stereo.graph_capture_failed", 0);
            if (launched) FT_HIP(hipGraphLaunch(fe->graphExec, L->stream));
        }
    }
    if (!launched) {
        rc = frontendEnqueue(fe, imagesL, imagesR, batch, on_device, width, height, stride, keysL, descL, nL, keysR, descR,
                             nR, capacity, uright, depth, n_matches, direct, 0, paired);
        if (rc != FT_OK) return rc;
        FT_HIP(hipEventRecord(fe->evDone[0], L->streamB));
        FT_HIP(hipEventRecord(fe->evDone[1], R->streamB));
    }
    auto &P = fe->pending;
    P.imagesL.assign(imagesL, imagesL + batch);
    P.imagesR.assign(imagesR, imagesR + batch);
    P.onDevice = on_device;
    P.width = width;
    P.height = height;
    P.stride = stride;
    P.active = true;
    P.graph = launched;
    P.batch = batch;
    P.capacity = capacity;
    P.direct = direct;
    P.keysL = keysL; P.descL = descL; P.nL = nL;
    P.keysR = keysR; P.descR = descR; P.nR = nR;
    P.uright = uright; P.depth = depth; P.nMatches = n_matches;
    return FT_OK;
}

int ft_stereo_frontend_wait(ft_stereo_frontend *fe) {
    FT_REQUIRE(fe, "null front end");
    auto &P = fe->pending;
    if (!P.active) return FT_OK;
    int rc = ft_set_device(fe->ctx);
    if (rc != FT_OK) return rc;
    ft_extractor *L = fe->exL, *R = fe->exR;
// ... 228 lines not shown
```

### include/fasttrack_amd.h

```cpp
#ifndef FASTTRACK_AMD_H
#define FASTTRACK_AMD_H

#include <stddef.h>
#include <stdint.h>

#ifdef __cplusplus
extern "C" {
#endif

#define FT_API __attribute__((visibility("default")))

typedef enum ft_status {
    FT_OK = 0,
    FT_ERR_INVALID = -1,
    FT_ERR_NO_DEVICE = -2,
    FT_ERR_HIP = -3,
    FT_ERR_CAPACITY = -4,
    FT_ERR_EMPTY = -5
} ft_status;

typedef struct ft_keypoint {
    float x, y, size, angle, response;
    int octave, class_id;
} ft_keypoint;

typedef struct ft_context ft_context;

FT_API const char *ft_version(void);
FT_API const char *ft_last_error(void);
FT_API int ft_device_count(void);
FT_API int ft_device_pci_bus_id(int device, char *buf, int len);
FT_API int ft_context_create(int device, int host_threads, ft_context **out);
FT_API int ft_context_destroy(ft_context *ctx);
FT_API int ft_context_synchronize(ft_context *ctx);
FT_API int ft_context_device_name(ft_context *ctx, char *buf, int len);
FT_API int ft_context_hw_queues(const ft_context *ctx);
FT_API int ft_context_set_lane_map(ft_context *ctx, const int *map, int n);
FT_API int ft_context_set_option(ft_context *ctx, const char *name, int value);
FT_API int ft_context_get_option(const ft_context *ctx, const char *name, int *value);
FT_API int ft_option_describe(int index, const char **name, const char **env, int *default_value, const char **doc);
FT_API int ft_option_range(const char *name, int *min_value, int *max_value);
FT_API int ft_context_host_threads(const ft_context *ctx);
FT_API int ft_context_save_stats(ft_context *ctx, const char *path);
FT_API int ft_context_set_kernel_timing(ft_context *ctx, int enabled);
FT_API int ft_context_get_stat(ft_context *ctx, const char *name, double *total_ms, long *calls);
FT_API int ft_context_reset_stats(ft_context *ctx);
FT_API int ft_device_malloc(ft_context *ctx, size_t bytes, void **dptr);
FT_API int ft_device_free(ft_context *ctx, void *dptr);
FT_API int ft_host_malloc(ft_context *ctx, size_t bytes, void **ptr);
FT_API int ft_host_free(ft_context *ctx, void *ptr);
FT_API int ft_memcpy_h2d(ft_context *ctx, void *dst, const void *src, size_t bytes);
FT_API int ft_memcpy_d2h(ft_context *ctx, void *dst, const void *src, size_t bytes);

typedef struct ft_extractor ft_extractor;

FT_API int ft_extractor_create(ft_context *ctx, int nfeatures, float scale_factor, int nlevels, int ini_th_fast,
                               int min_th_fast, int image_width, int image_height, int max_batch,
                               ft_extractor **out);
FT_API int ft_extractor_destroy(ft_extractor *ex);
FT_API int ft_extractor_levels(const ft_extractor *ex);
FT_API int ft_extractor_max_batch(const ft_extractor *ex);
FT_API int ft_extractor_max_keypoints(const ft_extractor *ex);
FT_API int ft_extractor_scale_factors(const ft_extractor *ex, float *scale, float *inv_scale, float *sigma2,
                                      float *inv_sigma2);
FT_API int ft_extractor_features_per_level(const ft_extractor *ex, int *quota);
FT_API int ft_extractor_level_size(const ft_extractor *ex, int level, int *width, int *height);

FT_API int ft_extract(ft_extractor *ex, const uint8_t *image, int width, int height, int stride, int lap0,
                      int lap1, ft_keypoint *keypoints, uint8_t *descriptors, int capacity, int *n_keypoints,
                      int *n_mono);


FT_API int ft_extract_batch(ft_extractor *ex, const uint8_t *const *images, int batch, int on_device, int width,
                            int height, int stride, int lap0, int lap1, ft_keypoint *keypoints,
                            uint8_t *descriptors, int capacity, int *n_keypoints, int *n_mono);

FT_API int ft_extractor_download_level(ft_extractor *ex, int slot, int level, uint8_t *dst, int dst_stride);
FT_API int ft_extractor_download_blurred_level(ft_extractor *ex, int slot, int level, uint8_t *dst, int dst_stride);
FT_API int ft_extractor_device_level(ft_extractor *ex, int slot, int level, const uint8_t **dptr, int *pitch);
FT_API int ft_extractor_download_candidates(ft_extractor *ex, int slot, int level, int *xys, int capacity,
                                            int *n);

FT_API int ft_extractor_octree_on_device(ft_extractor *ex, int level, const int *xys, int n, int tiers, int *out_xys,
                                         int capacity, int *n_out, int *tier);

FT_API int ft_octree_distribute(const int *xys, int n, int minX, int maxX, int minY, int maxY, int N, int *out_idx,
                                int capacity, int *n_out);
FT_API int ft_level_geometry(int width, int height, int nfeatures, float scale_factor, int nlevels, int *level_w,
                             int *level_h, int *quota, int *n_cols, int *n_rows, int *w_cell, int *h_cell);
FT_API int ft_pyramid_band_plan(int width, int height, float scale_factor, int nlevels, int bands, int *first_row, int *end_row);

FT_API int ft_stereo_match(ft_extractor *exL, ft_extractor *exR, int slot, const ft_keypoint *keysL, int nL,
                           const ft_keypoint *keysR, int nR, const uint8_t *descL, const uint8_t *descR,
                           float mbf, float mb, int apply_median_cut, float *uright, float *depth, int *sad,
                           int *n_matches);

typedef struct ft_stereo_frontend ft_stereo_frontend;
FT_API int ft_stereo_frontend_create(ft_context *ctx, int nfeatures, float scale_factor, int nlevels,
                                     int ini_th_fast, int min_th_fast, int image_width, int image_height,
                                     int max_batch, float mbf, float mb, ft_stereo_frontend **out);
FT_API int ft_stereo_frontend_destroy(ft_stereo_frontend *fe);
FT_API ft_extractor *ft_stereo_frontend_left(ft_stereo_frontend *fe);
FT_API ft_extractor *ft_stereo_frontend_right(ft_stereo_frontend *fe);
FT_API int ft_stereo_frontend_submit(ft_stereo_frontend *fe, const uint8_t *const *imagesL,
                                     const uint8_t *const *imagesR, int batch, int on_device, int width, int height,
                                     int stride, ft_keypoint *keysL, uint8_t *descL, int *nL, ft_keypoint *keysR,
                                     uint8_t *descR, int *nR, int capacity, float *uright, float *depth,
                                     int *n_matches);
FT_API int ft_stereo_frontend_wait(ft_stereo_frontend *fe);
FT_API int ft_stereo_frontend_process(ft_stereo_frontend *fe, const uint8_t *const *imagesL,
                                      const uint8_t *const *imagesR, int batch, int on_device, int width,
                                      int height, int stride, ft_keypoint *keysL, uint8_t *descL, int *nL,
                                      ft_keypoint *keysR, uint8_t *descR, int *nR, int capacity, float *uright,
                                      float *depth, int *n_matches);
FT_API int ft_stereo_frontend_device_descriptors(ft_stereo_frontend *fe, int slot, int right, const uint8_t **dptr, int *n);

FT_API int ft_fisheye_match(ft_context *ctx, const uint8_t *descL, int nL, const uint8_t *descR, int nR,
                            int *matches, int *best, int *second);

typedef struct ft_fisheye_rig {
    float cam1[8], cam2[8];
    float precision;
    float Rlr[9], tlr[3];
} ft_fisheye_rig;
FT_API int ft_fisheye_stereo(ft_context *ctx, const ft_fisheye_rig *rig, const uint8_t *descL, const ft_keypoint *keysL,
                             int nL, const uint8_t *descR, const ft_keypoint *keysR, int nR, const float *level_sigma2,
                             int nlevels, int *matches, float *depth, float *p3d, int *n_matches);

typedef struct ft_frame_view {
    int N;
    int Nleft;
    float mnMinX, mnMinY, mnMaxX, mnMaxY;
    float grid_inv_w, grid_inv_h;
    float mbf, mb;
    const ft_keypoint *keys;
    const ft_keypoint *keys_right;
    const uint8_t *descriptors;
    const float *uright;
    int *holder_obs;
    const int *left_to_right;
    const int *right_to_left;
    int cam_model;
    float cam[8];
    float Trl[12];
    const float *scale_factors;
    int nlevels;
} ft_frame_view;

FT_API int ft_features_in_area(ft_context *ctx, const ft_frame_view *F, int nq, const float *x, const float *y,
                               const float *r, const int *min_level, const int *max_level, const uint8_t *right,
                               int *indices, int capacity, int *counts);

typedef struct ft_local_points {
    int M;
    const uint8_t *skip;
    const uint8_t *in_view, *in_view_r;
    const int *level, *level_r;
    const float *view_cos, *view_cos_r;
    const float *proj_x, *proj_y;
    const float *proj_xr, *proj_yr;
    const uint8_t *descriptors;
    const int *observations;
} ft_local_points;

FT_API int ft_search_local_points(ft_context *ctx, ft_frame_view *F, const ft_local_points *P, float th,
                                  float nn_ratio, int *assign, int *n_matches, int *best_dist, int *best_dist2,
                                  int *best_level, int *best_level2, int *best_idx, int *best_dist_r,
                                  int *best_dist2_r, int *best_level_r, int *best_level2_r, int *best_idx_r);

typedef struct ft_last_points {
    int N;
    const uint8_t *valid;
    const float *world_pos;
    const uint8_t *descriptors;
    const int *observations;
    const int *octave;
    const float *angle;
} ft_last_points;

FT_API int ft_search_last_frame(ft_context *ctx, ft_frame_view *Cur, const ft_last_points *L, const float *Tcw,
                                float th, int forward, int backward, int check_orientation, int *assign,
                                int *n_matches, int *best_dist, int *best_idx, int *best_dist_r,
                                int *best_idx_r);

typedef struct ft_se3 {
    float q[4];
    float t[3];
} ft_se3;
FT_API int ft_search_last_frame_se3(ft_context *ctx, ft_frame_view *Cur, const ft_last_points *L, const ft_se3 *Tcw,
                                    const ft_se3 *Trl, float th, int forward, int backward, int check_orientation, int *assign,
                                    int *n_matches, int *best_dist, int *best_idx, int *best_dist_r, int *best_idx_r);

FT_API int ft_search_for_initialization(ft_context *ctx, const ft_frame_view *F1, const ft_frame_view *F2, float *prev_matched,
                                        int window_size, float nn_ratio, int check_orientation, int *matches12, int *n_matches,
                                        int *matched_distance);

typedef struct ft_keyframe_points {
    int N;
    const uint8_t *valid;
    const float *world_pos;
    const float *max_distance;
    const float *min_distance;
    const uint8_t *descriptors;
    const int *observations;
    const float *angle;
} ft_keyframe_points;
FT_API int ft_search_keyframe_projection(ft_context *ctx, ft_frame_view *Cur, const ft_keyframe_points *K, const ft_se3 *Tcw,
                                         float log_scale_factor, float th, int orb_dist, int check_orientation, int *assign,
                                         int *n_matches, int *best_dist, int *best_idx);

typedef struct ft_frame_pose {
    float Rcw[9];
    float tcw[3];
    float Ow[3];
    float tlr[3];
} ft_frame_pose;

typedef struct ft_map_points {
    int M;
    const uint8_t *skip;
    const float *world_pos;
    const float *normal;
    const float *max_distance;
    const float *min_distance;
    const uint8_t *descriptors;
    const int *observations;
} ft_map_points;

typedef struct ft_frustum_result {
    uint8_t *in_view, *in_view_r;
    int *level, *level_r;
    float *view_cos, *view_cos_r;
    float *proj_x, *proj_y, *proj_xr, *proj_yr;
    float *depth, *depth_r;
} ft_frustum_result;

FT_API int ft_is_in_frustum(ft_context *ctx, const ft_frame_view *F, const ft_frame_pose *pose, const ft_map_points *P,
                            float viewing_cos_limit, float log_scale_factor, const ft_frustum_result *out,
                            int *n_to_match);

typedef struct ft_tracked_frame ft_tracked_frame;
FT_API int ft_tracked_frame_create(ft_context *ctx, int max_keypoints, int max_points, ft_tracked_frame **out);
FT_API int ft_tracked_frame_destroy(ft_tracked_frame *tf);
// ... 163 lines not shown
```

Baseline: 83290.

## Split octree launch into LDS size classes and zero counters in compact kernel

```diff
diff --git a/fasttrack_amd/_capi.py b/fasttrack_amd/_capi.py
--- a/fasttrack_amd/_capi.py
+++ b/fasttrack_amd/_capi.py
@@ -251,6 +251,8 @@
     L.ft_octree_distribute.argtypes = [vp, i, i, i, i, i, i, vp, i, ip]
     L.ft_level_geometry.argtypes = [i, i, i, f, i, vp, vp, vp, vp, vp, vp, vp]
     L.ft_pyramid_band_plan.argtypes = [i, i, f, i, i, vp, vp]
+    L.ft_octree_class_plan.argtypes = [i, i, i, f, i, i, vp, vp, vp, vp, vp]
+    L.ft_octree_lds_bytes.argtypes = [i, i, i]
     _lib = L
     return L
 
diff --git a/fasttrack_amd/csrc/extractor.cpp b/fasttrack_amd/csrc/extractor.cpp
--- a/fasttrack_amd/csrc/extractor.cpp
+++ b/fasttrack_amd/csrc/extractor.cpp
@@ -338,7 +338,12 @@
     return FT_OK;
 }
 
-int ft_extract_launch_a(ft_extractor *ex, int b0, int nb, hipEvent_t done) {
+static int *octCountersOf(ft_extractor *ex, int sub) {
+    if (!ex->deviceOctree || !(ex->octLayout.bigN || ex->histEnabled)) return nullptr;
+    return ex->d_bigCount + 4 * (sub % FT_PIPE_MAX);
+}
+
+int ft_extract_launch_a(ft_extractor *ex, int sub, int b0, int nb, hipEvent_t done) {
     const FtGeom &g = ex->geom;
     if (!ex->deviceOctree) {
         const int rce = ft_extract_ensure_host_cand(ex);
@@ -366,7 +371,7 @@
     uint32_t *candDst = ex->deviceOctree ? ex->d_candDev : ex->d_cand;
     int *cntDst = ex->deviceOctree ? ex->d_candCountDev : ex->d_candCount;
     rc = ft_launch_compact(ex->stream, g, nb, cellCount, stage, candDst + (size_t)b0 * g.candPerSlot,
-                           cntDst + (size_t)b0 * g.nlevels);
+                           cntDst + (size_t)b0 * g.nlevels, octCountersOf(ex, sub));
     ex->evt.end(tm, ex->stream);
     if (rc != FT_OK) return rc;
     if (done) FT_HIP(hipEventRecord(done, ex->stream));
@@ -394,12 +399,13 @@
     a.histFirst = ex->histEnabled && (ex->histFirstMode == 2 || (ex->histFirstMode == 1 && !large)) ? 1 : 0;
     if (a.histFirst) a.histCap = a.histGrid = a.histWanted = 0;
     a.sortCap = a.bigN ? std::min(ex->bigGrid, nb * g.nlevels) : 0;
-    a.bigCount = ex->d_bigCount + 4 * (sub % FT_OCT_STREAMS);
+    int *counters = octCountersOf(ex, sub);
+    a.bigCount = counters ? counters : ex->d_bigCount;
     a.bigList = ex->d_bigList + (size_t)(sub % FT_OCT_STREAMS) * ex->maxBatch * g.nlevels;
     a.sortList = ex->d_sortList + (size_t)(sub % FT_OCT_STREAMS) * ex->maxBatch * g.nlevels;
     const bool tm = ex->ctx->kernelTiming;
     ex->evt.begin(tm, "kernel.octree", so);
-    int rc = ft_launch_octree(so, g, nb, a);
+    int rc = ft_launch_octree(so, g, nb, a, large && !a.histFirst ? &ex->octClasses : nullptr, counters != nullptr);
     ex->evt.end(tm, so);
     if (rc != FT_OK) return rc;
     if (done) FT_HIP(hipEventRecord(done, so));
@@ -469,12 +475,13 @@
         return;
     }
     int want = 0, wantHist = 0;
-    for (int k = 0; k < FT_OCT_STREAMS; k++) {
+    for (int k = 0; k < FT_PIPE_MAX; k++) {
         want = std::max(want, ex->h_bigStat[k]);
         wantHist = std::max(wantHist, ex->h_histStat[k]);
         ex->h_bigStat[k] = ex->h_histStat[k] = 0;
     }
     if (wantHist > 0) {
+        ex->ctx->addStat("extract.octree_listed_levels", wantHist);
         ex->histIdle = 0;
         ex->histGrid = std::max(std::max(ex->histGrid, FT_OCT_HISTMIN), std::min(FT_OCT_HISTMAX, ((wantHist + 63) / 64) * 64));
     } else if (ex->histGrid > 0 && ++ex->histIdle >= FT_OCT_HIST_RETIRE) {
@@ -597,7 +604,7 @@
     a.oHist = ex->h_histStat;
     a.oBig = ex->h_bigStat;
     a.batch = batch;
-    a.nStreams = FT_OCT_STREAMS;
+    a.nStreams = FT_PIPE_MAX;
     return ft_launch_finish_counts(st, a);
 }
 
@@ -657,6 +664,23 @@
     else
         for (int b = 0; b < batch; b++) one(b, 0);
     return FT_OK;
+}
+
+static int octPoolNeeds(const ft_extractor *ex, int *need) {
+    int cap = 0;
+    for (int l = 0; l < ex->nlevels; l++) {
+        const int minB = FT_EDGE_THRESHOLD - 3;
+        int nIni = (int)std::round(static_cast<float>(ex->geom.lv[l].maxBX - minB) / (ex->geom.lv[l].maxBY - minB));
+        if (nIni < 1) nIni = 1;
+        need[l] = ex->quota[l] + 4 * nIni + 16;
+        cap = std::max(cap, need[l]);
+    }
+    return cap;
+}
+static int octClassesWanted() {
+    const char *e = ft_debug_env("FT_DEBUG_OCT_CLASSES");
+    if (e && (e[0] == '0' || e[0] == '1') && !e[1]) return e[0] - '0';
+    return FT_OCT_CLASSES_DEFAULT;
 }
 
 extern "C" {
@@ -723,10 +747,10 @@
     FT_CHECK(own.devAlloc(&ex->d_selCount, B * g.nlevels + FT_MAX_LEVELS));
     FT_CHECK(own.devAlloc(&ex->d_overflow, 1));
     FT_CHECK(own.devAlloc(&ex->d_ovSlot, B));
-    FT_CHECK(own.devAlloc(&ex->d_bigCount, 4 * FT_OCT_STREAMS));
-    FT_CHECK(own.pinAlloc(&ex->h_bigStat, FT_OCT_STREAMS));
-    FT_CHECK(own.pinAlloc(&ex->h_histStat, FT_OCT_STREAMS));
-    for (int k = 0; k < FT_OCT_STREAMS; k++) ex->h_bigStat[k] = ex->h_histStat[k] = 0;
+    FT_CHECK(own.devAlloc(&ex->d_bigCount, 4 * FT_PIPE_MAX));
+    FT_CHECK(own.pinAlloc(&ex->h_bigStat, FT_PIPE_MAX));
+    FT_CHECK(own.pinAlloc(&ex->h_histStat, FT_PIPE_MAX));
+    for (int k = 0; k < FT_PIPE_MAX; k++) ex->h_bigStat[k] = ex->h_histStat[k] = 0;
     FT_CHECK(own.devAlloc(&ex->d_bigList, (size_t)FT_OCT_STREAMS * B * g.nlevels));
     FT_CHECK(own.devAlloc(&ex->d_sortList, (size_t)FT_OCT_STREAMS * B * g.nlevels));
     FT_CHECK(own.pinAlloc(&ex->h_selCount, B * g.nlevels));
@@ -771,18 +795,14 @@
     {
         FtOctArgs &o = ex->octLayout;
         memset(&o, 0, sizeof o);
-        int maxQ = 0, need = 0;
+        int maxQ = 0, need[FT_MAX_LEVELS];
+        o.poolCap = octPoolNeeds(ex, need);
         for (int l = 0; l < nlevels; l++) {
             o.quota[l] = ex->quota[l];
             o.levelMax[l] = ex->levelMax[l];
             o.selOff[l] = ex->levelOff[l];
             maxQ = std::max(maxQ, ex->quota[l]);
-            const int minB = FT_EDGE_THRESHOLD - 3;
-            int nIni = (int)std::round(static_cast<float>(g.lv[l].maxBX - minB) / (g.lv[l].maxBY - minB));
-            if (nIni < 1) nIni = 1;
-            need = std::max(need, ex->quota[l] + 4 * nIni);
-        }
-        o.poolCap = need + 16;
+        }
         (void)maxQ;
         ex->deviceOctree = ex->tune.device_octree != 0 && o.poolCap < 30000 && ft_octree_smem_bytes(o.poolCap) <= 160 * 1024;
         o.histCap = o.sortCap = o.histGrid = o.histWanted = o.histFirst = 0;
@@ -803,9 +823,10 @@
             FT_CHECK(own.devAlloc(&ex->d_candCountDev, B * g.nlevels));
             if (ft_octree_smem_bytes(o.poolCap, true) < ft_octree_smem_bytes(o.poolCap, false))
                 FT_CHECK(own.devAlloc(&ex->d_octLow, B * g.nlevels * (size_t)FT_OCT_MAXN));
+            ft_octree_classes_of(g, ex->quota.data(), need, octClassesWanted(), ex->d_octLow != nullptr, -1, -1, &ex->octClasses);
             FT_HIP(hipMemset(ex->d_overflow, 0, sizeof(int)));
             FT_HIP(hipMemset(ex->d_ovSlot, 0, sizeof(int) * B));
-            FT_HIP(hipMemset(ex->d_bigCount, 0, 4 * FT_OCT_STREAMS * sizeof(int)));
+            FT_HIP(hipMemset(ex->d_bigCount, 0, 4 * FT_PIPE_MAX * sizeof(int)));
         }
     }
     ctx->liveObjects++;
@@ -893,6 +914,39 @@
     if (rc != FT_OK) return rc;
     ft_pyr_bands_of(ex.geom, bands, first_row, end_row);
     return FT_OK;
+}
+
+int ft_octree_class_plan(int width, int height, int nfeatures, float scale_factor, int nlevels, int classes, int *split, int *keys,
+                         int *pool, int *lds_bytes, int *compact) {
+    FT_REQUIRE(nlevels >= 1 && nlevels <= FT_MAX_LEVELS && scale_factor > 1.0f && nfeatures > 0 && (classes == 0 || classes == 1) &&
+                   split && keys && pool && lds_bytes && compact,
+               "bad parameters");
+    ft_extractor ex;
+    ex.nfeatures = nfeatures;
+    ex.scaleFactor = scale_factor;
+    ex.nlevels = nlevels;
+    ex.width = width;
+    ex.height = height;
+    std::vector<FtTap> taps;
+    int rc = buildGeometry(&ex, taps);
+    if (rc != FT_OK) return rc;
+    int need[FT_MAX_LEVELS];
+    const int poolCap = octPoolNeeds(&ex, need);
+    *compact = ft_octree_smem_bytes(poolCap, true) < ft_octree_smem_bytes(poolCap, false) ? 1 : 0;
+    FtOctClasses c;
+    ft_octree_classes_of(ex.geom, ex.quota.data(), need, classes, *compact != 0, -1, -1, &c);
+    *split = c.split;
+    for (int k = 0; k < 2; k++) {
+        keys[k] = c.keys[k];
+        pool[k] = c.pool[k];
+        lds_bytes[k] = c.smem[k];
+    }
+    return FT_OK;
+}
+
+int ft_octree_lds_bytes(int keys, int pool, int compact) {
+    FT_REQUIRE(keys >= 1 && keys <= 16384 && pool >= 1 && pool < 30000, "bad parameters");
+    return (int)ft_octree_class_smem_bytes(keys, pool, compact != 0);
 }
 
 int ft_extractor_destroy(ft_extractor *ex) {
@@ -989,7 +1043,7 @@
         FT_CHECK(ft_extract_prepare(ex, images, batch, on_device, width, height, stride));
         for (int s = 0, b0 = 0; b0 < batch; s++, b0 += sb) {
             const int nb = std::min(sb, batch - b0);
-            FT_CHECK(ft_extract_launch_a(ex, b0, nb, dev ? nullptr : ex->evA[s]));
+            FT_CHECK(ft_extract_launch_a(ex, s, b0, nb, dev ? nullptr : ex->evA[s]));
             if (dev) FT_CHECK(ft_extract_launch_octree(ex, s, b0, nb, ex->evA[s]));
         }
         for (int s = 0, b0 = 0; b0 < batch; s++, b0 += sb) {
diff --git a/fasttrack_amd/csrc/ft_host.h b/fasttrack_amd/csrc/ft_host.h
--- a/fasttrack_amd/csrc/ft_host.h
+++ b/fasttrack_amd/csrc/ft_host.h
@@ -196,6 +196,7 @@
     std::vector<int> levelOff;
     FtGeom geom{};
     FtPyrBands pyrBands{};
+    FtOctClasses octClasses{};
     hipStream_t stream = nullptr;
     hipStream_t streamB = nullptr;
     hipEvent_t evA[FT_PIPE_MAX] = {}, evB[FT_PIPE_MAX] = {};
@@ -318,7 +319,7 @@
 int ft_pipeline_depth(const ft_tuning &t, int batch, bool deviceOctree);
 int ft_extract_prepare(ft_extractor *ex, const uint8_t *const *images, int batch, int on_device, int width, int height,
                        int stride);
-int ft_extract_launch_a(ft_extractor *ex, int b0, int nb, hipEvent_t done);
+int ft_extract_launch_a(ft_extractor *ex, int sub, int b0, int nb, hipEvent_t done);
 int ft_extract_ensure_stage(ft_extractor *ex);
 int ft_extract_ensure_host_cand(ft_extractor *ex);
 void ft_extract_restage(ft_extractor *ex, const uint8_t *const *images, int batch, int width, int height, int stride);
diff --git a/fasttrack_amd/csrc/ft_internal.h b/fasttrack_amd/csrc/ft_internal.h
--- a/fasttrack_amd/csrc/ft_internal.h
+++ b/fasttrack_amd/csrc/ft_internal.h
@@ -171,11 +171,24 @@
                          const uint8_t *pyr, int iniTh, int minTh, int alignedLoads, int *cellCount,
                          uint32_t *stage, int ordered, const FtCellRec *cellTab);
 int ft_launch_compact(hipStream_t st, const FtGeom &g, int batch, const int *cellCount, const uint32_t *stage,
-                      uint32_t *cand, int *candCount);
+                      uint32_t *cand, int *candCount, int *octCounters);
 int ft_launch_orient_desc(hipStream_t st, const FtGeom &g, int batch, const uint8_t *const *l0, int l0pitch,
                           const uint8_t *pyr, int alignedLoads, const FtSelKp *sel, const int *selCount,
                           const FtOctArgs &layout, int *nSel, ft_keypoint *keys, uint8_t *desc);
-int ft_launch_octree(hipStream_t st, const FtGeom &g, int batch, const FtOctArgs &a);
+struct FtOctClasses {
+    int split;
+    int keys[2], pool[2];
+    int smem[2];
+};
+#define FT_OCT_MINKEYS 64
+#define FT_OCT_CLASSES_DEFAULT 0
+#define FT_OCT_CLASS_SPLIT 3
+#define FT_OCT_CLASS_FILL 6
+void ft_octree_classes_of(const FtGeom &g, const int *quota, const int *need, int classes, bool compact, int split, int fill,
+                          FtOctClasses *out);
+int ft_launch_octree(hipStream_t st, const FtGeom &g, int batch, const FtOctArgs &a, const FtOctClasses *cls = nullptr,
+                     bool countersZeroed = false);
+size_t ft_octree_class_smem_bytes(int keys, int poolCap, bool compact);
 int ft_launch_blur_level(hipStream_t st, const uint8_t *img, int pitch, int w, int h, uint8_t *dst, int dstPitch);
 size_t ft_octree_smem_bytes(int poolCap, bool compact = false);
 size_t ft_octree_hist_smem_bytes(int poolCap);
diff --git a/fasttrack_amd/csrc/kernels_extract.hip b/fasttrack_amd/csrc/kernels_extract.hip
--- a/fasttrack_amd/csrc/kernels_extract.hip
+++ b/fasttrack_amd/csrc/kernels_extract.hip
@@ -894,12 +894,13 @@
 }
 
 __global__ __launch_bounds__(256) void k_compact(FtGeom g, const int *cellCount, const uint32_t *stage,
-                                                 uint32_t *cand, int *candCount) {
+                                                 uint32_t *cand, int *candCount, int *octCounters) {
     extern __shared__ __attribute__((aligned(16))) uint8_t smem[];
     int *offs = (int *)smem;
     __shared__ int wsum[4];
     const int tid = threadIdx.x, lane = tid & 63, wave = tid >> 6;
     const int level = blockIdx.x, slot = blockIdx.y;
+    if (octCounters && level == 0 && slot == 0 && tid < 2) octCounters[tid] = 0;
     const FtLevelGeom &L = g.lv[level];
     const int nCells = L.nCols * L.nRows;
     const int *cnt = cellCount + (size_t)slot * g.totalCells + L.cellBase;
@@ -1534,13 +1535,13 @@
 }
 
 int ft_launch_compact(hipStream_t st, const FtGeom &g, int batch, const int *cellCount, const uint32_t *stage,
-                      uint32_t *cand, int *candCount) {
+                      uint32_t *cand, int *candCount, int *octCounters) {
     int maxCells = 0;
     for (int l = 0; l < g.nlevels; l++) maxCells = std::max(maxCells, g.lv[l].nCols * g.lv[l].nRows);
     dim3 grid2(g.nlevels, batch, 1), block(256, 1, 1);
     for (int rep = ft_debug_repeat("compact"); rep > 0; rep--)
     hipLaunchKernelGGL(k_compact, grid2, block, (size_t)(maxCells + 1) * sizeof(int), st, g, cellCount, stage, cand,
-                       candCount);
+                       candCount, octCounters);
     FT_HIP(hipGetLastError());
     return FT_OK;
 }
diff --git a/fasttrack_amd/csrc/kernels_octree.hip b/fasttrack_amd/csrc/kernels_octree.hip
--- a/fasttrack_amd/csrc/kernels_octree.hip
+++ b/fasttrack_amd/csrc/kernels_octree.hip
@@ -289,7 +289,7 @@
 
 template <bool HIST>
 __device__ __forceinline__ bool oct_level(const FtGeom &g, const FtOctArgs &a, const int slot, const int level, const int maxN,
-                                          uint8_t *smem, uint32_t *lowG = nullptr) {
+                                          const int cap, uint8_t *smem, uint32_t *lowG = nullptr) {
     const int tid = threadIdx.x;
     const int lane = tid & 63;
     const FtLevelGeom &L = g.lv[level];
@@ -345,7 +345,6 @@
         }
     }
     const uint32_t *cand = a.cand + (size_t)slot * g.candPerSlot + L.candBase;
-    const int cap = a.poolCap;
     const OctLds o = oct_lds_layout(cap, HIST ? oct_hist_key_bytes() : maxN * 8, HIST, lowG != nullptr);
     const bool compact = !HIST && o.low != 0;
     unsigned long long *keys = (unsigned long long *)(smem + o.keys);
@@ -801,11 +800,12 @@
     }
 }
 
-__global__ __launch_bounds__(OCT_THREADS) void k_octree(FtGeom g, FtOctArgs a) {
+__global__ __launch_bounds__(OCT_THREADS) void k_octree(FtGeom g, FtOctArgs a, int level0, int maxN, int cap) {
     extern __shared__ __attribute__((aligned(16))) uint8_t smem[];
     __builtin_amdgcn_s_setprio(3);
-    oct_level<false>(g, a, blockIdx.x, blockIdx.y, FT_OCT_MAXN, smem,
-                     a.low ? a.low + ((size_t)blockIdx.x * g.nlevels + blockIdx.y) * FT_OCT_MAXN : nullptr);
+    const int level = level0 + (int)blockIdx.y;
+    oct_level<false>(g, a, blockIdx.x, level, maxN, cap, smem,
+                     a.low ? a.low + ((size_t)blockIdx.x * g.nlevels + level) * FT_OCT_MAXN : nullptr);
 }
 
 __global__ __launch_bounds__(OCT_THREADS) void k_octree_hist(FtGeom g, FtOctArgs a) {
@@ -816,7 +816,7 @@
     for (int ei = (int)blockIdx.x; ei < cnt; ei += (int)gridDim.x) {
         const unsigned e = a.bigList[ei];
         const int slot = (int)(e & 0xffffu), level = (int)(e >> 16);
-        const bool done = oct_level<true>(g, a, slot, level, 0, smem);
+        const bool done = oct_level<true>(g, a, slot, level, 0, a.poolCap, smem);
         if (!done && threadIdx.x == 0) {
             const int n = a.candCount[slot * g.nlevels + level];
             bool ok = false;
@@ -845,11 +845,11 @@
     const int n = a.candCount[slot * g.nlevels + level];
     const int N = a.quota[level];
     bool done = false;
-    if (2 * n >= 3 * N || n > FT_OCT_MAXN) done = oct_level<true>(g, a, slot, level, 0, smem);
+    if (2 * n >= 3 * N || n > FT_OCT_MAXN) done = oct_level<true>(g, a, slot, level, 0, a.poolCap, smem);
     if (done) return;
     if (n <= FT_OCT_MAXN) {
         __syncthreads();
-        oct_level<false>(g, a, slot, level, FT_OCT_MAXN, smem, a.low ? a.low + ((size_t)slot * g.nlevels + level) * FT_OCT_MAXN : nullptr);
+        oct_level<false>(g, a, slot, level, FT_OCT_MAXN, a.poolCap, smem, a.low ? a.low + ((size_t)slot * g.nlevels + level) * FT_OCT_MAXN : nullptr);
         return;
     }
     if (threadIdx.x == 0) {
@@ -875,7 +875,7 @@
     const int cnt = min(a.bigCount[1], a.sortCap);
     if ((int)blockIdx.x >= cnt) return;
     const unsigned e = a.sortList[blockIdx.x];
-    oct_level<false>(g, a, (int)(e & 0xffffu), (int)(e >> 16), a.bigN, smem);
+    oct_level<false>(g, a, (int)(e & 0xffffu), (int)(e >> 16), a.bigN, a.poolCap, smem);
 }
 
 }
@@ -888,7 +888,42 @@
     return 0;
 }
 
-int ft_launch_octree(hipStream_t st, const FtGeom &g, int batch, const FtOctArgs &a) {
+size_t ft_octree_class_smem_bytes(int keys, int poolCap, bool compact) { return (size_t)oct_lds_layout(poolCap, keys * 8, false, compact).total; }
+
+void ft_octree_classes_of(const FtGeom &g, const int *quota, const int *need, int classes, bool compact, int split, int fill,
+                          FtOctClasses *out) {
+    int pool0 = 0;
+    for (int l = 0; l < g.nlevels; l++) pool0 = std::max(pool0, need[l]);
+    FtOctClasses c;
+    c.split = g.nlevels;
+    c.keys[0] = c.keys[1] = FT_OCT_MAXN;
+    c.pool[0] = c.pool[1] = pool0;
+    c.smem[0] = c.smem[1] = (int)ft_octree_class_smem_bytes(FT_OCT_MAXN, pool0, compact);
+    *out = c;
+    if (const char *e = ft_debug_env("FT_DEBUG_OCT_SPLIT")) split = atoi(e);
+    if (const char *e = ft_debug_env("FT_DEBUG_OCT_FILL")) fill = atoi(e);
+    if (split < 0) split = FT_OCT_CLASS_SPLIT;
+    if (fill < 1) fill = FT_OCT_CLASS_FILL;
+    if (!classes || split < 1 || split >= g.nlevels) return;
+    int maxQ = 0, maxCand = 0, pool1 = 0;
+    for (int l = split; l < g.nlevels; l++) {
+        maxQ = std::max(maxQ, quota[l]);
+        maxCand = std::max(maxCand, g.lv[l].candCap);
+        pool1 = std::max(pool1, need[l]);
+    }
+    const long long want = std::min<long long>((long long)fill * maxQ, maxCand);
+    int keys = FT_OCT_MINKEYS;
+    while (keys < want && keys < FT_OCT_MAXN) keys <<= 1;
+    const int smem1 = (int)ft_octree_class_smem_bytes(keys, pool1, compact);
+    if (smem1 >= c.smem[0]) return;
+    c.split = split;
+    c.keys[1] = keys;
+    c.pool[1] = pool1;
+    c.smem[1] = smem1;
+    *out = c;
+}
+
+int ft_launch_octree(hipStream_t st, const FtGeom &g, int batch, const FtOctArgs &a, const FtOctClasses *cls, bool countersZeroed) {
     const size_t smem = ft_octree_smem_bytes(a.poolCap, a.low != nullptr);
     if (ft_debug_env("FT_DEBUG_OCC")) fprintf(stderr, "[ft] k_octree: %zu B of LDS per workgroup (pool %d)\n", smem, a.poolCap);
     if (smem > 64 * 1024)
@@ -899,21 +934,31 @@
     const size_t smemBig = a.bigN ? (size_t)oct_lds_layout(a.poolCap, a.bigN * 8, false).total : 0;
     if (a.bigN && a.sortCap > 0)
         FT_HIP(hipFuncSetAttribute((const void *)k_octree_big, hipFuncAttributeMaxDynamicSharedMemorySize, (int)smemBig));
+    bool zeroed = countersZeroed;
     if (a.histFirst) {
         const size_t smemAll = std::max(ft_octree_hist_smem_bytes(a.poolCap), smem);
         if (smemAll > 64 * 1024)
             FT_HIP(hipFuncSetAttribute((const void *)k_octree_auto, hipFuncAttributeMaxDynamicSharedMemorySize, (int)smemAll));
         for (int rep = ft_debug_repeat("octree"); rep > 0; rep--) {
-            if (a.bigN) FT_HIP(hipMemsetAsync(a.bigCount, 0, 2 * sizeof(int), st));
+            if (a.bigN && !zeroed) FT_HIP(hipMemsetAsync(a.bigCount, 0, 2 * sizeof(int), st));
+            zeroed = false;
             hipLaunchKernelGGL(k_octree_auto, dim3(batch, g.nlevels), dim3(OCT_THREADS), smemAll, st, g, a);
             if (a.bigN && a.sortCap > 0) hipLaunchKernelGGL(k_octree_big, dim3(a.sortCap), dim3(OCT_THREADS), smemBig, st, g, a);
         }
         FT_HIP(hipGetLastError());
         return FT_OK;
     }
+    const bool two = cls && cls->split > 0 && cls->split < g.nlevels;
     for (int rep = ft_debug_repeat("octree"); rep > 0; rep--) {
-        if (a.bigN || a.histCap > 0 || a.histWanted) FT_HIP(hipMemsetAsync(a.bigCount, 0, 2 * sizeof(int), st));
-        hipLaunchKernelGGL(k_octree, dim3(batch, g.nlevels), dim3(OCT_THREADS), smem, st, g, a);
+        if ((a.bigN || a.histCap > 0 || a.histWanted) && !zeroed) FT_HIP(hipMemsetAsync(a.bigCount, 0, 2 * sizeof(int), st));
+        zeroed = false;
+        if (two) {
+            hipLaunchKernelGGL(k_octree, dim3(batch, g.nlevels - cls->split), dim3(OCT_THREADS), (size_t)cls->smem[1], st, g, a, cls->split,
+                               cls->keys[1], cls->pool[1]);
+            hipLaunchKernelGGL(k_octree, dim3(batch, cls->split), dim3(OCT_THREADS), smem, st, g, a, 0, FT_OCT_MAXN, a.poolCap);
+        } else {
+            hipLaunchKernelGGL(k_octree, dim3(batch, g.nlevels), dim3(OCT_THREADS), smem, st, g, a, 0, FT_OCT_MAXN, a.poolCap);
+        }
         if (a.histCap > 0) hipLaunchKernelGGL(k_octree_hist, dim3(std::min(a.histCap, std::max(a.histGrid, 1))), dim3(OCT_THREADS), smemHist, st, g, a);
         if (a.bigN && a.sortCap > 0) hipLaunchKernelGGL(k_octree_big, dim3(a.sortCap), dim3(OCT_THREADS), smemBig, st, g, a);
     }
diff --git a/fasttrack_amd/csrc/matcher.cpp b/fasttrack_amd/csrc/matcher.cpp
--- a/fasttrack_amd/csrc/matcher.cpp
+++ b/fasttrack_amd/csrc/matcher.cpp
@@ -280,7 +280,7 @@
         imgs.insert(imgs.end(), imagesR, imagesR + B);
         FT_CHECK(ft_extract_prepare(L, imgs.data(), 2 * B, on_device, width, height, stride));
         fe->ctx->addStat("stereo.device_octree_batches", 0);
-        FT_CHECK(ft_extract_launch_a(L, 0, 2 * B, nullptr));
+        FT_CHECK(ft_extract_launch_a(L, 0, 0, 2 * B, nullptr));
         FT_CHECK(ft_extract_launch_octree(L, 0, 0, 2 * B, L->evA[0]));
         hipStream_t st = L->streamB;
         FT_HIP(hipStreamWaitEvent(st, L->evA[0], 0));
@@ -316,10 +316,10 @@
     if (dev) fe->ctx->addStat("stereo.device_octree_batches", 0);
     for (int s = 0, b0 = 0; b0 < batch; s++, b0 += sb) {
         const int nb = std::min(sb, batch - b0);
-        rc = ft_extract_launch_a(L, b0, nb, dev ? nullptr : L->evA[s]);
+        rc = ft_extract_launch_a(L, s, b0, nb, dev ? nullptr : L->evA[s]);
         if (rc == FT_OK && dev) rc = ft_extract_launch_octree(L, s, b0, nb, L->evA[s]);
         if (rc != FT_OK) return rc;
-        rc = ft_extract_launch_a(R, b0, nb, dev ? nullptr : R->evA[s]);
+        rc = ft_extract_launch_a(R, s, b0, nb, dev ? nullptr : R->evA[s]);
         if (rc == FT_OK && dev) rc = ft_extract_launch_octree(R, s, b0, nb, R->evA[s]);
         if (rc != FT_OK) return rc;
     }
diff --git a/include/fasttrack_amd.h b/include/fasttrack_amd.h
--- a/include/fasttrack_amd.h
+++ b/include/fasttrack_amd.h
@@ -89,6 +89,9 @@
 FT_API int ft_level_geometry(int width, int height, int nfeatures, float scale_factor, int nlevels, int *level_w,
                              int *level_h, int *quota, int *n_cols, int *n_rows, int *w_cell, int *h_cell);
 FT_API int ft_pyramid_band_plan(int width, int height, float scale_factor, int nlevels, int bands, int *first_row, int *end_row);
+FT_API int ft_octree_class_plan(int width, int height, int nfeatures, float scale_factor, int nlevels, int classes, int *split,
+                                int *keys, int *pool, int *lds_bytes, int *compact);
+FT_API int ft_octree_lds_bytes(int keys, int pool, int compact);
 
 FT_API int ft_stereo_match(ft_extractor *exL, ft_extractor *exR, int slot, const ft_keypoint *keysL, int nL,
                            const ft_keypoint *keysR, int nR, const uint8_t *descL, const uint8_t *descR,
```

New measurement: 83410, median of 3. Within noise of the previous version (+0.1%).
